# BruceGeLi/TCE_RL

Measured on NVIDIA B200. Metric: TCE policy-update episodes/sec, higher is better.
Workload: dtype f32

## Files before the change

### include/tce_b200.h

```cpp
#ifndef TCE_B200_H
#define TCE_B200_H

#include <stddef.h>
#include <stdint.h>

#ifdef __cplusplus
extern "C" {
#endif

typedef enum {
  TCE_OK = 0,
  TCE_ERR_INVALID_ARGUMENT = -1,
  TCE_ERR_UNSUPPORTED_SHAPE = -2,
  TCE_ERR_CUDA = -3,
  TCE_ERR_WORKSPACE = -4
} tce_status;

int tce_version(void);
const char *tce_strerror(int status);
const char *tce_last_cuda_error(void);

typedef struct {
  int32_t num_dof;
  int32_t num_basis;
  int32_t num_basis_outside;
  int32_t pre_compute_length_factor;
  int32_t auto_scale_basis;
  int32_t relative_goal;
  int32_t relative_goal_scaled;
  int32_t reserved;
  double tau, delay, dt, alpha, alpha_phase, basis_bandwidth_factor, weights_scale, goal_scale;
} tce_mp_cfg;

typedef struct tce_tables tce_tables_t;

int tce_prodmp_tables_create(const tce_mp_cfg *cfg, void *stream, tce_tables_t **out);
void tce_prodmp_tables_destroy(tce_tables_t *tables);
int tce_prodmp_tables_num_pc(const tce_tables_t *tables);
int tce_prodmp_tables_export(const tce_tables_t *tables, double *y1, double *y2, double *dy1,
                             double *dy2, double *pos_basis, double *vel_basis, double *scale);

int tce_prodmp_traj_fwd(const tce_tables_t *tables, const float *params, const float *times,
                        const float *init_time, const float *init_pos, const float *init_vel,
                        float *traj, int64_t B, int64_t T, void *stream);
int tce_prodmp_traj_fwd_uniform(const tce_tables_t *tables, const float *params, const float *times_row,
                                const float *init_time, const float *init_pos, const float *init_vel,
                                float *rows_ws, float *traj, int64_t B, int64_t T, void *stream);
int tce_prodmp_traj_bwd(const tce_tables_t *tables, const float *grad_traj, const float *times,
                        const float *init_time, float *grad_params, float *grad_init_pos,
                        float *grad_init_vel, int64_t B, int64_t T, void *stream);

int tce_mvn_rsample(const float *mean, const float *L, int64_t ldb_L, const float *eps, uint64_t seed,
                    uint64_t offset, float *out, int64_t B, int n, void *stream);
int tce_chol_fwd(const float *A, float *L, int32_t *info, int64_t B, int n, void *stream);
int tce_chol_bwd(const float *L, const float *grad_L, float *grad_A, int64_t B, int n, void *stream);
int tce_policy_head_fwd(const float *vec, int64_t ldb_vec, float min_std, float *L, int64_t B, int n,
                        void *stream);
int tce_policy_head_bwd(const float *vec, int64_t ldb_vec, const float *grad_L, float *grad_vec,
                        int64_t B, int n, void *stream);
int tce_policy_head_diag_fwd(const float *vec, int64_t ldb_vec, float min_std, float *L, int64_t B, int n,
                             void *stream);
int tce_policy_head_diag_bwd(const float *vec, int64_t ldb_vec, const float *grad_L, float *grad_vec,
                             int64_t B, int n, void *stream);
int tce_gauss_stats(const float *mean, const float *L, int64_t ldb_L, const float *mean_o,
                    const float *L_o, int64_t ldb_Lo, double *out, int64_t B, int n, void *stream);
int tce_gauss_stats_bwd(const float *mean, const float *L, int64_t ldb_L, const float *mean_o,
                        const float *L_o, int64_t ldb_Lo, const double *grad_out, float *grad_mean,
                        float *grad_L, int64_t B, int n, void *stream);

int tce_gauss_maha(const float *mean, const float *mean_o, const float *L_o, int64_t ldb_Lo,
                   const double *grad_out, double *maha, float *grad_mean, int64_t B, int n, void *stream);
int tce_gauss_maha_bwd_full(const float *mean, const float *mean_o, const float *L_o, int64_t ldb_Lo,
                            const double *grad_out, float *grad_mean, float *grad_L, int64_t B, int n,
                            void *stream);
int tce_tri_inverse(const float *L, int64_t ldb, double *Linv, int64_t B, int n, void *stream);
int tce_gauss_maha_shared(const float *mean, const float *mean_o, const double *Linv, const double *grad_out,
                          double *maha, float *grad_mean, int64_t B, int n, void *stream);

int tce_proj_mean_fwd(const float *mean, const float *mean_o, const double *mean_part, double eps,
                      float *proj_mean, int64_t B, int n, void *stream);
int tce_proj_mean_bwd(const float *mean, const float *mean_o, const double *mean_part, double eps,
                      const float *grad_out, float *grad_mean, double *grad_mean_part, int64_t B, int n,
                      void *stream);
int tce_proj_entropy_fwd(const float *L, const double *beta, int64_t ldb_beta, int equality, float *out,
                         double *entropy, int64_t B, int n, void *stream);
int tce_proj_entropy_bwd(const float *L, const double *beta, int64_t ldb_beta, int equality,
                         const float *grad_out, float *grad_L, int64_t B, int n, void *stream);
int tce_proj_kl_diag_fwd(const float *s, int64_t ldb_s, int64_t inc_s, const float *s_old, int64_t ldb_so,
                         int64_t inc_so, double eps_cov, const double *beta, int64_t ldb_beta, int equality,
                         float *out, int64_t ldb_o, int64_t inc_o, double *state, int32_t *info, int64_t B, int n,
                         void *stream);
int tce_proj_kl_diag_bwd(const float *s, int64_t ldb_s, int64_t inc_s, const float *s_old, int64_t ldb_so,
                         int64_t inc_so, const double *state, const float *grad_out, int64_t ldb_g, int64_t inc_g,
                         float *grad_s, int64_t ldb_gs, int64_t inc_gs, int64_t B, int n, void *stream);
size_t tce_proj_kl_save_doubles(int64_t B, int n);
int tce_proj_kl_cov_fwd(const float *L, const float *L_o, double eps_cov, float *proj_L, double *save,
                        int32_t *info, int warm_start, int64_t B, int n, void *stream);
int tce_proj_kl_cov_bwd(const float *L, const float *proj_L, const float *grad_out, const double *save,
                        float *grad_L, int64_t B, int n, void *stream);
int tce_proj_kl_entropy_fwd(const float *L, const float *L_o, double eps_cov, const double *beta,
                            int64_t ldb_beta, int equality, float *proj_L, float *out_L, double *save,
                            int32_t *info, int warm_start, int64_t B, int n, void *stream);
int tce_proj_kl_entropy_bwd(const float *L, const float *proj_L, const float *grad_out, const double *save,
                            float *grad_L, int64_t B, int n, void *stream);
int tce_proj_kl_entropy_bwd_inv(const float *L, const float *proj_L, const float *grad_out, const double *save,
                                const double *out_inv, float *grad_L, int64_t B, int n, void *stream);
int tce_proj_kl_entropy_bwd_tr(const float *L, const float *proj_L, const float *grad_out, const double *save,
                               double tr_coeff, float *grad_L, int64_t B, int n, void *stream);
int tce_proj_kl_bwd_sigma(const float *L, const double *grad_sigma, const double *save, int fused_entropy,
                          double tr_coeff, float *grad_L, int64_t B, int n, void *stream);
int tce_proj_kl_entropy_fwd_sigma_vec(const float *vec, int64_t ldb_vec, float min_std, float *L_built,
                                      const float *L_o, double eps_cov, const double *beta, int64_t ldb_beta,
                                      int equality, float *proj_L, float *out_L, double *save, int32_t *info,
                                      int warm_start, int64_t B, int n, void *stream);
int tce_proj_kl_bwd_sigma_k_vec(const float *L, const float *vec, int64_t ldb_vec, const double *grad_sigma,
                                const double *save, int fused_entropy, double tr_coeff, float *grad_vec, int64_t B,
                                int n, void *stream);
int tce_proj_kl_bwd_prep(double *save, int64_t B, int n, void *stream);
int tce_proj_kl_bwd_sigma_k(const float *L, const double *grad_sigma, const double *save, int fused_entropy,
                            double tr_coeff, float *grad_L, int64_t B, int n, void *stream);
int tce_proj_kl_entropy_fwd_sigma(const float *L, const float *L_o, double eps_cov, const double *beta,
                                  int64_t ldb_beta, int equality, float *proj_L, float *out_L, double *save,
                                  int32_t *info, int warm_start, int64_t B, int n, void *stream);
int tce_proj_kl_entropy_fwd_chol(const double *save, float *proj_L, float *out_L, double *out_inv, int32_t *info,
                                 int64_t B, int n, void *stream);
int tce_proj_frob_cov_fwd(const float *L, const float *L_o, int64_t ldb_Lo, double eps_cov, float *proj_L,
                          double *save_sc, int32_t *info, int64_t B, int n, void *stream);
int tce_proj_frob_cov_bwd(const float *L, const float *L_o, int64_t ldb_Lo, double eps_cov,
                          const float *proj_L, const float *grad_out, const double *save_sc, float *grad_L,
                          int64_t B, int n, void *stream);
int tce_proj_w2_cov_fwd(const float *L, const float *L_o, int64_t ldb_Lo, double eps_cov, int scale_prec,
                        float *proj_L, double *save_sc, int64_t B, int n, void *stream);
int tce_proj_w2_cov_bwd(const float *L, const float *L_o, int64_t ldb_Lo, double eps_cov, int scale_prec,
                        const float *grad_out, float *grad_L, int64_t B, int n, void *stream);
int tce_cov_distance(int kind, const float *L, const float *L_o, int64_t ldb_Lo, int scale_prec,
                     const double *grad_val, double *val, float *grad_L, int64_t B, int n, void *stream);

size_t tce_seglik_work_bytes(const tce_tables_t *tables, int64_t B, int64_t P);
int tce_seglik_gram(const tce_tables_t *tables, const float *smp_traj, const float *mean, const float *L,
                    int64_t ldb_L, const float *times, const float *init_time, const float *init_pos,
                    const float *init_vel, const int64_t *pred_pairs, void *work, double *diag_max,
                    int64_t B, int64_t T, int64_t P, void *stream);
int tce_seglik_chol(const tce_tables_t *tables, const void *work, void *adj, const double *diag_max, double reg_rel,
                    const float *grad_logp, const float *logp_old, const float *advantage,
                    double grad_scale, double *loss_acc, float *logp, int32_t *info, int64_t B,
                    int64_t P, void *stream);
int tce_seglik_bwd(const tce_tables_t *tables, const void *work, const float *L, int64_t ldb_L,
                   const float *times, const float *init_time, const int64_t *pred_pairs,
                   const float *upstream, float *grad_mean, float *grad_L, int64_t B, int64_t T, int64_t P,
                   void *stream);
int tce_seglik_diag_max(const tce_tables_t *tables, const float *s, int64_t ldb_s, int64_t inc_s,
                        const float *times, const float *init_time, const int64_t *pred_pairs, double *diag_max,
                        int64_t B, int64_t T, int64_t P, void *stream);
int tce_seglik_diag_fwd(const tce_tables_t *tables, const float *smp_traj, const float *mean, const float *s,
                        int64_t ldb_s, int64_t inc_s, const float *times, const float *init_time,
                        const float *init_pos, const float *init_vel, const int64_t *pred_pairs,
                        const double *diag_max, double reg_rel, float *logp, int32_t *info, int64_t B, int64_t T,
                        int64_t P, void *stream);
int tce_seglik_diag_bwd(const tce_tables_t *tables, const float *smp_traj, const float *mean, const float *s,
                        int64_t ldb_s, int64_t inc_s, const float *times, const float *init_time,
                        const float *init_pos, const float *init_vel, const int64_t *pred_pairs,
                        const double *diag_max, double reg_rel, const float *grad_logp, float *grad_mean,
                        float *grad_s, int64_t ldb_gs, int64_t inc_gs, int64_t B, int64_t T, int64_t P,
                        void *stream);

int tce_seglik_fused_config(const tce_tables_t *tables, int64_t B, int64_t P, int chained, int32_t *episodes_per_iter,
                            int32_t *grid, int64_t *part_floats, int64_t *pre_doubles_per_episode);
int tce_seglik_prepass(const tce_tables_t *tables, const float *smp_traj, const float *mean, const float *L,
                       int64_t ldb_L, const double *Sigma0, const double *sigma_scale, const float *times,
                       const float *init_time, const float *init_pos, const float *init_vel,
                       const int64_t *pred_pairs, double *pre, double *diag_max, int chained, int64_t B, int64_t T,
                       int64_t P, void *stream);
int tce_seglik_fused(const tce_tables_t *tables, const double *pre, const float *L, int64_t ldb_L,
                     const double *Sigma0, const double *sigma_scale, const int64_t *pred_pairs,
                     const double *diag_max, double reg_rel, int grad_mode, const float *grad_logp,
                     const float *logp_old, const float *advantage, double grad_scale, double *loss_acc, float *logp,
                     int32_t *info, float *grad_mean, float *grad_L, float *dsigma_part, int chained, int64_t B,
                     int64_t P, void *stream);
int tce_seglik_dsigma_reduce(const tce_tables_t *tables, float *dsigma_part, int nparts, const float *L,
                             const float *upstream, float *grad_L, double *grad_sigma, void *stream);
size_t tce_seglik_uniform_ws_doubles(const tce_tables_t *tables, int64_t P);
int tce_seglik_uniform_parts(const tce_tables_t *tables, int64_t B, int64_t P, int32_t *nparts,
                             int64_t *apart_doubles);
int tce_seglik_uniform_prep(const tce_tables_t *tables, const float *L, const double *Sigma0,
                            const double *sigma_scale, const float *times, const float *init_time,
                            const int64_t *pred_pairs, double *ws, double *diag_max, double reg_rel, int what,
                            int64_t P, void *stream);
int tce_seglik_uniform_main(const tce_tables_t *tables, const double *ws, const float *smp_traj, const float *mean,
                            const float *init_pos, const float *init_vel, const int64_t *pred_pairs, int grad_mode,
                            const float *grad_logp, const float *logp_old, const float *advantage,
                            double grad_scale, double *loss_acc, float *logp, int32_t *info, float *grad_mean,
                            double *apart, int64_t B, int64_t T, int64_t P, void *stream);
int tce_seglik_uniform_finish(const tce_tables_t *tables, double *ws, const double *apart, int nparts,
                              const float *L, const float *upstream, float *grad_L, double *grad_sigma, int64_t P,
                              void *stream);

int tce_gae(const float *rewards, const float *values, const uint8_t *dones, const uint8_t *tl_dones,
            float gamma, float lam, int use_gae, float *adv, float *ret, int64_t B, int64_t T,
            void *stream);
int tce_segment_advantage_raw(int mode, const float *rewards, const float *values, const float *advantages,
                              const int64_t *pred_pairs, float gamma, float *seg, double *stats, int64_t B,
                              int64_t T, int64_t P, void *stream);
int tce_sum_stats(const float *x, double *stats, int64_t N, void *stream);
int tce_normalize_by_stats(float *x, const double *stats, int64_t N, void *stream);

int tce_grad_sumsq(const float *grad_flat, int64_t n, double *state, void *stream);
int tce_adam_step(int count, float *const *params, const int64_t *sizes, const float *grad_flat, float *m,
                  float *v, const double *state, double max_norm, double lr, double beta1, double beta2,
                  double eps, double weight_decay, void *stream);

int tce_p2p_allreduce_sumsq(int world, int rank, const void *const *peer_bufs, void *const *peer_pads, int64_t n,
                            float *avg_out, void *local2, double *state3, void *stream);
int tce_p2p_allreduce_sumsq_range(int world, int rank, const void *const *peer_bufs, void *const *peer_pads,
                                  int64_t offset, int64_t n, int phase, int bump_step, float *avg_out, void *local2,
                                  double *state3, void *stream);

size_t tce_p2p_push_xchg_bytes(int world, int64_t n_total);
int tce_p2p_push_allreduce_sumsq(int world, int rank, void *const *peer_xchg, const float *grad, int64_t n_total,
                                 int64_t offset, int64_t n, int phase, int bump_step, float *avg_out, void *local2,
                                 double *state3, void *stream);

int tce_epoch_mean_fwd(const float *mean, const float *mean_old, const double *Linv_old, double eps_mean,
                       float *proj_mean, double *maha_old, float *u_old, double *acc, int64_t B, int n,
                       void *stream);
int tce_epoch_tr_mean(const float *mean, const float *mean_old, const double *maha_old, const float *u_old,
                      const double *Linv_new, const double *kl_scalars, double eps_mean, double tr_coeff,
                      float *tr_grad, double *acc, int64_t B, int n, void *stream);
int tce_epoch_mean_combine(const float *g_proj_mean, const float *mean, const float *mean_old, const double *maha_old,
                           const float *u_old, const float *tr_grad, double eps_mean, float *grad_mean, int64_t B,
                           int n, void *stream);
int tce_epoch_metrics(const double *acc, const double *lik_stats, const double *kl_scalars, const double *adam_stats,
                      int64_t B, double tr_coeff, int with_cov, double ent_coef, double *out19, void *stream);

int tce_debug_kl_phase_cycles(long long *out32);
int tce_debug_seglik_phase_cycles(long long *out32);
int tce_bench_fma(int fp64, int iters, void *scratch, double *flops, void *stream);

#ifdef __cplusplus
}
#endif
#endif
```

### tce_rl_b200/_lib.py

```python
from __future__ import annotations

import ctypes as C
import os

HERE = os.path.dirname(os.path.abspath(__file__))
LIB_PATH = os.path.join(HERE, "libtce_b200.so")


class TceError(RuntimeError):
    pass


class MpCfg(C.Structure):
    _fields_ = [("num_dof", C.c_int32), ("num_basis", C.c_int32), ("num_basis_outside", C.c_int32),
                ("pre_compute_length_factor", C.c_int32), ("auto_scale_basis", C.c_int32),
                ("relative_goal", C.c_int32), ("relative_goal_scaled", C.c_int32), ("reserved", C.c_int32),
                ("tau", C.c_double), ("delay", C.c_double), ("dt", C.c_double), ("alpha", C.c_double),
                ("alpha_phase", C.c_double), ("basis_bandwidth_factor", C.c_double),
                ("weights_scale", C.c_double), ("goal_scale", C.c_double)]


_P, _I64, _I32, _U64, _F, _D = C.c_void_p, C.c_int64, C.c_int, C.c_uint64, C.c_float, C.c_double

SIGNATURES = {
    "tce_version": (C.c_int, []),
    "tce_strerror": (C.c_char_p, [C.c_int]),
    "tce_last_cuda_error": (C.c_char_p, []),
    "tce_prodmp_tables_create": (C.c_int, [C.POINTER(MpCfg), _P, C.POINTER(_P)]),
    "tce_prodmp_tables_destroy": (None, [_P]),
    "tce_prodmp_tables_num_pc": (C.c_int, [_P]),
    "tce_prodmp_tables_export": (C.c_int, [_P] * 8),
    "tce_prodmp_traj_fwd": (C.c_int, [_P] * 7 + [_I64, _I64, _P]),
    "tce_prodmp_traj_fwd_uniform": (C.c_int, [_P] * 8 + [_I64, _I64, _P]),
    "tce_prodmp_traj_bwd": (C.c_int, [_P] * 7 + [_I64, _I64, _P]),
    "tce_mvn_rsample": (C.c_int, [_P, _P, _I64, _P, _U64, _U64, _P, _I64, _I32, _P]),
    "tce_chol_fwd": (C.c_int, [_P, _P, _P, _I64, _I32, _P]),
    "tce_chol_bwd": (C.c_int, [_P, _P, _P, _I64, _I32, _P]),
    "tce_policy_head_fwd": (C.c_int, [_P, _I64, _F, _P, _I64, _I32, _P]),
    "tce_policy_head_bwd": (C.c_int, [_P, _I64, _P, _P, _I64, _I32, _P]),
    "tce_policy_head_diag_fwd": (C.c_int, [_P, _I64, _F, _P, _I64, _I32, _P]),
    "tce_policy_head_diag_bwd": (C.c_int, [_P, _I64, _P, _P, _I64, _I32, _P]),
    "tce_proj_kl_diag_fwd": (C.c_int, [_P, _I64, _I64, _P, _I64, _I64, _D, _P, _I64, _I32, _P, _I64, _I64, _P, _P, _I64,
                                       _I32, _P]),
    "tce_proj_kl_diag_bwd": (C.c_int, [_P, _I64, _I64, _P, _I64, _I64, _P, _P, _I64, _I64, _P, _I64, _I64, _I64, _I32,
                                       _P]),
    "tce_seglik_diag_max": (C.c_int, [_P, _P, _I64, _I64, _P, _P, _P, _P, _I64, _I64, _I64, _P]),
    "tce_seglik_diag_fwd": (C.c_int, [_P, _P, _P, _P, _I64, _I64, _P, _P, _P, _P, _P, _P, _D, _P, _P, _I64, _I64, _I64,
                                      _P]),
    "tce_seglik_diag_bwd": (C.c_int, [_P, _P, _P, _P, _I64, _I64, _P, _P, _P, _P, _P, _P, _D, _P, _P, _P, _I64, _I64,
                                      _I64, _I64, _I64, _P]),
    "tce_gauss_stats": (C.c_int, [_P, _P, _I64, _P, _P, _I64, _P, _I64, _I32, _P]),
    "tce_gauss_stats_bwd": (C.c_int, [_P, _P, _I64, _P, _P, _I64, _P, _P, _P, _I64, _I32, _P]),
    "tce_gauss_maha": (C.c_int, [_P, _P, _P, _I64, _P, _P, _P, _I64, _I32, _P]),
    "tce_gauss_maha_bwd_full": (C.c_int, [_P, _P, _P, _I64, _P, _P, _P, _I64, _I32, _P]),
    "tce_tri_inverse": (C.c_int, [_P, _I64, _P, _I64, _I32, _P]),
    "tce_gauss_maha_shared": (C.c_int, [_P, _P, _P, _P, _P, _P, _I64, _I32, _P]),
    "tce_proj_mean_fwd": (C.c_int, [_P, _P, _P, _D, _P, _I64, _I32, _P]),
    "tce_proj_mean_bwd": (C.c_int, [_P, _P, _P, _D, _P, _P, _P, _I64, _I32, _P]),
    "tce_proj_entropy_fwd": (C.c_int, [_P, _P, _I64, _I32, _P, _P, _I64, _I32, _P]),
    "tce_proj_entropy_bwd": (C.c_int, [_P, _P, _I64, _I32, _P, _P, _I64, _I32, _P]),
    "tce_proj_kl_save_doubles": (C.c_size_t, [_I64, _I32]),
    "tce_proj_kl_cov_fwd": (C.c_int, [_P, _P, _D, _P, _P, _P, _I32, _I64, _I32, _P]),
    "tce_proj_kl_cov_bwd": (C.c_int, [_P, _P, _P, _P, _P, _I64, _I32, _P]),
    "tce_proj_kl_entropy_fwd": (C.c_int, [_P, _P, _D, _P, _I64, _I32, _P, _P, _P, _P, _I32, _I64, _I32, _P]),
    "tce_proj_kl_entropy_bwd": (C.c_int, [_P, _P, _P, _P, _P, _I64, _I32, _P]),
    "tce_proj_kl_entropy_bwd_tr": (C.c_int, [_P, _P, _P, _P, _D, _P, _I64, _I32, _P]),
    "tce_proj_kl_bwd_sigma": (C.c_int, [_P, _P, _P, _I32, _D, _P, _I64, _I32, _P]),
    "tce_proj_kl_bwd_sigma_k": (C.c_int, [_P, _P, _P, _I32, _D, _P, _I64, _I32, _P]),
    "tce_proj_kl_bwd_prep": (C.c_int, [_P, _I64, _I32, _P]),
    "tce_proj_kl_entropy_fwd_sigma_vec": (C.c_int, [_P, _I64, _F, _P, _P, _D, _P, _I64, _I32, _P, _P, _P, _P, _I32, _I64,
                                                    _I32, _P]),
    "tce_proj_kl_bwd_sigma_k_vec": (C.c_int, [_P, _P, _I64, _P, _P, _I32, _D, _P, _I64, _I32, _P]),
    "tce_proj_kl_entropy_bwd_inv": (C.c_int, [_P, _P, _P, _P, _P, _P, _I64, _I32, _P]),
    "tce_proj_kl_entropy_fwd_sigma": (C.c_int, [_P, _P, _D, _P, _I64, _I32, _P, _P, _P, _P, _I32, _I64, _I32, _P]),
    "tce_proj_kl_entropy_fwd_chol": (C.c_int, [_P, _P, _P, _P, _P, _I64, _I32, _P]),
    "tce_grad_sumsq": (C.c_int, [_P, _I64, _P, _P]),
    "tce_adam_step": (C.c_int, [_I32, _P, _P, _P, _P, _P, _P, _D, _D, _D, _D, _D, _D, _P]),
    "tce_proj_frob_cov_fwd": (C.c_int, [_P, _P, _I64, _D, _P, _P, _P, _I64, _I32, _P]),
    "tce_proj_frob_cov_bwd": (C.c_int, [_P, _P, _I64, _D, _P, _P, _P, _P, _I64, _I32, _P]),
    "tce_proj_w2_cov_fwd": (C.c_int, [_P, _P, _I64, _D, _I32, _P, _P, _I64, _I32, _P]),
    "tce_proj_w2_cov_bwd": (C.c_int, [_P, _P, _I64, _D, _I32, _P, _P, _I64, _I32, _P]),
    "tce_cov_distance": (C.c_int, [_I32, _P, _P, _I64, _I32, _P, _P, _P, _I64, _I32, _P]),
    "tce_seglik_work_bytes": (C.c_size_t, [_P, _I64, _I64]),
    "tce_seglik_gram": (C.c_int, [_P, _P, _P, _P, _I64, _P, _P, _P, _P, _P, _P, _P, _I64, _I64, _I64, _P]),
    "tce_seglik_chol": (C.c_int, [_P, _P, _P, _P, _D, _P, _P, _P, _D, _P, _P, _P, _I64, _I64, _P]),
    "tce_seglik_bwd": (C.c_int, [_P, _P, _P, _I64, _P, _P, _P, _P, _P, _P, _I64, _I64, _I64, _P]),
    "tce_seglik_fused_config": (C.c_int, [_P, _I64, _I64, _I32, C.POINTER(C.c_int32), C.POINTER(C.c_int32),
                                          C.POINTER(C.c_int64), C.POINTER(C.c_int64)]),
    "tce_seglik_prepass": (C.c_int, [_P] * 4 + [_I64] + [_P] * 9 + [_I32, _I64, _I64, _I64, _P]),
    "tce_seglik_fused": (C.c_int, [_P, _P, _P, _I64, _P, _P, _P, _P, _D, _I32, _P, _P, _P, _D, _P, _P, _P, _P, _P, _P,
                                   _I32, _I64, _I64, _P]),
    "tce_seglik_dsigma_reduce": (C.c_int, [_P, _P, _I32, _P, _P, _P, _P, _P]),
    "tce_seglik_uniform_ws_doubles": (C.c_size_t, [_P, _I64]),
    "tce_seglik_uniform_parts": (C.c_int, [_P, _I64, _I64, C.POINTER(C.c_int32), C.POINTER(C.c_int64)]),
    "tce_seglik_uniform_prep": (C.c_int, [_P, _P, _P, _P, _P, _P, _P, _P, _P, _D, _I32, _I64, _P]),
    "tce_seglik_uniform_main": (C.c_int, [_P, _P, _P, _P, _P, _P, _P, _I32, _P, _P, _P, _D, _P, _P, _P, _P, _P, _I64,
                                          _I64, _I64, _P]),
    "tce_seglik_uniform_finish": (C.c_int, [_P, _P, _P, _I32, _P, _P, _P, _P, _I64, _P]),
    "tce_p2p_allreduce_sumsq": (C.c_int, [_I32, _I32, _P, _P, _I64, _P, _P, _P, _P]),
    "tce_p2p_allreduce_sumsq_range": (C.c_int, [_I32, _I32, _P, _P, _I64, _I64, _I32, _I32, _P, _P, _P, _P]),
    "tce_p2p_push_xchg_bytes": (C.c_size_t, [_I32, _I64]),
    "tce_p2p_push_allreduce_sumsq": (C.c_int, [_I32, _I32, _P, _P, _I64, _I64, _I64, _I32, _I32, _P, _P, _P, _P]),
    "tce_epoch_mean_fwd": (C.c_int, [_P, _P, _P, _D, _P, _P, _P, _P, _I64, _I32, _P]),
    "tce_epoch_tr_mean": (C.c_int, [_P, _P, _P, _P, _P, _P, _D, _D, _P, _P, _I64, _I32, _P]),
    "tce_epoch_mean_combine": (C.c_int, [_P, _P, _P, _P, _P, _P, _D, _P, _I64, _I32, _P]),
    "tce_epoch_metrics": (C.c_int, [_P, _P, _P, _P, _I64, _D, _I32, _D, _P, _P]),
    "tce_gae": (C.c_int, [_P, _P, _P, _P, _F, _F, _I32, _P, _P, _I64, _I64, _P]),
    "tce_segment_advantage_raw": (C.c_int, [_I32, _P, _P, _P, _P, _F, _P, _P, _I64, _I64, _I64, _P]),
    "tce_sum_stats": (C.c_int, [_P, _P, _I64, _P]),
    "tce_normalize_by_stats": (C.c_int, [_P, _P, _I64, _P]),
    "tce_debug_kl_phase_cycles": (C.c_int, [_P]),
    "tce_debug_seglik_phase_cycles": (C.c_int, [_P]),
    "tce_bench_fma": (C.c_int, [_I32, _I32, _P, C.POINTER(C.c_double), _P]),
}

_lib = None


def load() -> C.CDLL:
    global _lib
    if _lib is None:
        if not os.path.exists(LIB_PATH):
            raise TceError(f"{LIB_PATH} is missing: run `python -m tce_rl_b200._build` "
                           "(or __graft_entry__.build()); there is no CPU fallback")
        lib = C.CDLL(LIB_PATH)
        for name, (res, args) in SIGNATURES.items():
            fn = getattr(lib, name)
            fn.restype, fn.argtypes = res, args
        _lib = lib
    return _lib


def check(status: int, what: str = "") -> None:
    if status != 0:
        lib = load()
        msg = lib.tce_strerror(status).decode()
        if status == -3:
            msg += " -- " + lib.tce_last_cuda_error().decode()
        raise TceError(f"{what}: {msg} (status {status})")


LAUNCHES = 0
_NO_KERNEL = {"tce_seglik_fused_config", "tce_seglik_uniform_parts", "tce_prodmp_tables_export", "tce_prodmp_tables_create", "tce_debug_kl_phase_cycles", "tce_debug_seglik_phase_cycles"}


TIMING = None


def call(name: str, *args) -> None:
    global LAUNCHES
    if TIMING is not None and name not in _NO_KERNEL:
        import torch
        st = torch.cuda.ExternalStream(args[-1]) if args[-1] else torch.cuda.default_stream()
        a, b = torch.cuda.Event(enable_timing=True), torch.cuda.Event(enable_timing=True)
        a.record(st)
        check(getattr(load(), name)(*args), name)
        b.record(st)
        TIMING.append((name, a, b))
        LAUNCHES += 1
        return
    check(getattr(load(), name)(*args), name)
    if name not in _NO_KERNEL:
        LAUNCHES += 1
```

### tce_rl_b200/csrc/tce_seglik_fused.cu

```cuda
#include <math.h>

#include "tce_common.cuh"

namespace {

constexpr int FT = 256;
constexpr double LN_2PI = 1.8378770664093453;

__host__ __device__ constexpr int tri(int n) { return n * (n + 1) / 2; }
__device__ __forceinline__ int tri_idx(int r, int c) { return r * (r + 1) / 2 + c; }
__device__ __forceinline__ void tri_decode(int t, int &I, int &J) {
  int i = (int)((sqrtf(8.0f * (float)t + 1.0f) - 1.0f) * 0.5f);
  while (i * (i + 1) / 2 > t) --i;
  while ((i + 1) * (i + 2) / 2 <= t) ++i;
  I = i;
  J = t - i * (i + 1) / 2;
}

struct Links { int pf, ps, nxt, prv; };
__device__ __forceinline__ Links links(int chained, int q, int P) {
  Links l;
  if (chained) { l.pf = q < P ? q : -1; l.ps = q >= 1 ? q - 1 : -1; l.nxt = q + 1; l.prv = q - 1; }
  else if (q & 1) { l.pf = -1; l.ps = q >> 1; l.nxt = q; l.prv = q - 1; }
  else { l.pf = q >> 1; l.ps = -1; l.nxt = q + 1; l.prv = q; }
  return l;
}
__device__ __forceinline__ long long point_time_index(const int64_t *__restrict__ pairs, int chained, int q, int P) {
  if (!chained) return pairs[q];
  return q < P ? pairs[2 * q] : pairs[2 * P - 1];
}
__device__ __forceinline__ int point_of(int chained, int p, int k) { return chained ? p + k : 2 * p + k; }

__device__ int block_chained(const int64_t *__restrict__ pairs, int P) {
  int ok = 1;
  for (int pp = threadIdx.x; pp + 1 < P; pp += blockDim.x) ok &= (pairs[2 * pp + 1] == pairs[2 * pp + 2]);
  return __syncthreads_and(ok) != 0;
}

template <int K1>
__device__ __forceinline__ void init_row_entry(const TabDev &tb, double t_init, int j, double *init_row) {
  int i0; double w;
  time_to_index(tb, t_init, i0, w);
  if (j < K1) {
    init_row[5 + j] = lerp_t(tb.pos[(size_t)i0 * K1 + j], tb.pos[(size_t)(i0 + 1) * K1 + j], w);
    init_row[5 + K1 + j] = lerp_t(tb.vel[(size_t)i0 * K1 + j], tb.vel[(size_t)(i0 + 1) * K1 + j], w);
  } else {
    const double a = lerp_t(tb.y1[i0], tb.y1[i0 + 1], w), b = lerp_t(tb.y2[i0], tb.y2[i0 + 1], w);
    const double c = lerp_t(tb.dy1[i0], tb.dy1[i0 + 1], w), d = lerp_t(tb.dy2[i0], tb.dy2[i0 + 1], w);
    init_row[0] = a; init_row[1] = b; init_row[2] = c; init_row[3] = d;
    init_row[4] = 1.0 / (a * d - b * c);
  }
}
template <int K1>
__device__ __forceinline__ void basis_entry(const TabDev &tb, const double *init_row, double t, int j, double *h_row,
                                            double *xi_row) {
  int i0; double w;
  time_to_index(tb, t, i0, w);
  const double y1 = lerp_t(tb.y1[i0], tb.y1[i0 + 1], w), y2 = lerp_t(tb.y2[i0], tb.y2[i0 + 1], w);
  const double idet = init_row[4];
  const double xi1 = (init_row[3] * y1 - init_row[2] * y2) * idet, xi2 = (init_row[0] * y2 - init_row[1] * y1) * idet;
  if (j < K1) {
    const double pj = lerp_t(tb.pos[(size_t)i0 * K1 + j], tb.pos[(size_t)(i0 + 1) * K1 + j], w);
    h_row[j] = (pj - xi1 * init_row[5 + j] - xi2 * init_row[5 + K1 + j]) * tb.scale[j];
  } else {
    xi_row[0] = xi1;
    xi_row[1] = xi2;
  }
}

template <int N>
__device__ __forceinline__ double seg_factor(double (&c)[tri(N)], double (&z)[N], double reg, int &bad) {
#define CE(r, q) c[(r) * ((r) + 1) / 2 + (q)]
  bad = 0;
  double half_logdet = 0.0, maha = 0.0;
#pragma unroll
  for (int j = 0; j < N; ++j) {
    double dj = CE(j, j) + reg;
#pragma unroll
    for (int k = 0; k < j; ++k) dj = fma(-CE(j, k), CE(j, k), dj);
    if (!(dj > 0.0) && bad == 0) bad = j + 1;
    double inv = (double)rsqrtf((float)dj);
    inv = inv * fma(-0.5 * dj, inv * inv, 1.5);
    inv = inv * fma(-0.5 * dj, inv * inv, 1.5);
    CE(j, j) = inv;
    half_logdet += 0.5 * log(dj);
#pragma unroll
    for (int i = j + 1; i < N; ++i) {
      double v = CE(i, j);
#pragma unroll
      for (int k = 0; k < j; ++k) v = fma(-CE(i, k), CE(j, k), v);
      CE(i, j) = v * inv;
    }
    double zj = z[j];
#pragma unroll
    for (int k = 0; k < j; ++k) zj = fma(-CE(j, k), z[k], zj);
    zj *= inv;
    z[j] = zj;
    maha = fma(zj, zj, maha);
  }
  return -0.5 * ((double)N * LN_2PI + maha) - half_logdet;
}
template <int N>
__device__ __forceinline__ void seg_adjoint(double (&c)[tri(N)], double (&z)[N], double g) {
#pragma unroll
  for (int i = N - 1; i >= 0; --i) {
    double v = z[i];
#pragma unroll
    for (int k = i + 1; k < N; ++k) v = fma(-CE(k, i), z[k], v);
    z[i] = v * CE(i, i);
  }
#pragma unroll
  for (int j = 0; j < N; ++j) {
#pragma unroll
    for (int i = j + 1; i < N; ++i) {
      double v = 0.0;
#pragma unroll
      for (int k = j; k < i; ++k) v = fma(CE(i, k), CE(k, j), v);
      CE(i, j) = -v * CE(i, i);
    }
  }
#pragma unroll
  for (int i = 0; i < N; ++i) {
#pragma unroll
    for (int j = 0; j <= i; ++j) {
      double v = 0.0;
#pragma unroll
      for (int k = i; k < N; ++k) v = fma(CE(k, i), CE(k, j), v);
      CE(i, j) = 0.5 * g * (z[i] * z[j] - v);
    }
  }
#pragma unroll
  for (int i = 0; i < N; ++i) z[i] *= g;
#undef CE
}

struct SegIO {
  const float *grad_logp, *logp_old, *advantage;
  float *logp;
  int32_t *info;
  double grad_scale, reg;
  int grad_mode;
};
template <int N>
__device__ __noinline__ void segment_thread(double *Ccol, double *Rcol, int S, long long gid, const SegIO &io,
                                            double &loss_part, double &ratio_part) {
  constexpr int NT = tri(N);
  double c[NT];
#define CE(r, q) c[(r) * ((r) + 1) / 2 + (q)]
#define ZS(i) Rcol[(size_t)(i) * S]
#pragma unroll
  for (int t = 0; t < NT; ++t) c[t] = Ccol[(size_t)t * S];
  int bad = 0;
  double half_logdet = 0.0, maha = 0.0;
#pragma unroll
  for (int j = 0; j < N; ++j) {
    double dj = CE(j, j) + io.reg;
#pragma unroll
    for (int k = 0; k < j; ++k) dj = fma(-CE(j, k), CE(j, k), dj);
    if (!(dj > 0.0) && bad == 0) bad = j + 1;
    double inv = (double)rsqrtf((float)dj);
    inv = inv * fma(-0.5 * dj, inv * inv, 1.5);
    inv = inv * fma(-0.5 * dj, inv * inv, 1.5);
    CE(j, j) = inv;
    half_logdet += 0.5 * log(dj);
#pragma unroll
    for (int i = j + 1; i < N; ++i) {
      double v = CE(i, j);
#pragma unroll
      for (int k = 0; k < j; ++k) v = fma(-CE(i, k), CE(j, k), v);
      CE(i, j) = v * inv;
    }
    double zj = ZS(j);
#pragma unroll
    for (int k = 0; k < j; ++k) zj = fma(-CE(j, k), ZS(k), zj);
    zj *= inv;
    ZS(j) = zj;
    maha = fma(zj, zj, maha);
  }
  const double lp = -0.5 * ((double)N * LN_2PI + maha) - half_logdet;
  if (io.logp) io.logp[gid] = (float)lp;
  if (io.info) io.info[gid] = bad;
  if (io.grad_mode == 0) return;
  double g;
  if (io.grad_mode == 2) {
    const double ratio = exp(lp - (double)io.logp_old[gid]);
    g = -ratio * (double)io.advantage[gid] * io.grad_scale;
    loss_part += g;
    ratio_part += ratio * io.grad_scale;
  } else {
    g = (double)io.grad_logp[gid];
  }
#pragma unroll
  for (int i = N - 1; i >= 0; --i) {
    double v = ZS(i);
#pragma unroll
    for (int k = i + 1; k < N; ++k) v = fma(-CE(k, i), ZS(k), v);
    ZS(i) = v * CE(i, i);
  }
#pragma unroll
  for (int j = 0; j < N; ++j) {
#pragma unroll
    for (int i = j + 1; i < N; ++i) {
      double v = 0.0;
#pragma unroll
      for (int k = j; k < i; ++k) v = fma(CE(i, k), CE(k, j), v);
      CE(i, j) = -v * CE(i, i);
    }
  }
  const double hg = 0.5 * g;
#pragma unroll
  for (int i = 0; i < N; ++i) {
    const double ai = ZS(i);
#pragma unroll
    for (int j = 0; j <= i; ++j) {
      double v = 0.0;
#pragma unroll
      for (int k = i; k < N; ++k) v = fma(CE(k, i), CE(k, j), v);
      Ccol[(size_t)(i * (i + 1) / 2 + j) * S] = hg * (ai * ZS(j) - v);
    }
  }
#pragma unroll
  for (int i = 0; i < N; ++i) ZS(i) = g * ZS(i);
#undef CE
#undef ZS
}

template <int K1>
__device__ __noinline__ void dsigma_block_store(bool own, const double *G, int S, const double *hm_e, int bd, int bdd,
                                                int chained, int nq, int P, float *dst, int ld, float *dst_t) {
  double acc[K1 * K1];
  if (own) {
#pragma unroll
    for (int t = 0; t < K1 * K1; ++t) acc[t] = 0.0;
    const int r0 = 2 * bd, q0 = 2 * bdd;
    const double *g00 = G + (size_t)tri_idx(r0, q0) * S, *g10 = G + (size_t)tri_idx(r0 + 1, q0) * S;
    const double *g11 = G + (size_t)tri_idx(r0 + 1, q0 + 1) * S;
    const double *g01 = (bd != bdd) ? G + (size_t)tri_idx(r0, q0 + 1) * S : g10;
    for (int q = 0; q < nq; ++q) {
      const Links lk = links(chained, q, P);
      const double *hq = hm_e + q * K1;
      double cs = 0.0, cn = 0.0, cp = 0.0;
      if (lk.pf >= 0) { cs += g00[lk.pf]; cn = g10[lk.pf]; }
      if (lk.ps >= 0) { cs += g11[lk.ps]; cp = g01[lk.ps]; }
      const double *hn = hm_e + (lk.pf >= 0 ? lk.nxt : q) * K1, *hp = hm_e + (lk.ps >= 0 ? lk.prv : q) * K1;
      double h[K1], w[K1];
#pragma unroll
      for (int j = 0; j < K1; ++j) h[j] = hq[j];
#pragma unroll
      for (int i = 0; i < K1; ++i) w[i] = fma(cs, h[i], fma(cn, hn[i], cp * hp[i]));
#pragma unroll
      for (int i = 0; i < K1; ++i)
#pragma unroll
        for (int j = 0; j < K1; ++j) acc[i * K1 + j] = fma(w[i], h[j], acc[i * K1 + j]);
    }
  }
  __syncthreads();
  if (own) {
    if (ld == 0) {
#pragma unroll
      for (int t = 0; t < K1 * K1; ++t) dst[t] = (float)acc[t];
    } else {
#pragma unroll
      for (int i = 0; i < K1; ++i)
#pragma unroll
        for (int j = 0; j < K1; ++j) {
          const float v = (float)acc[i * K1 + j];
          dst[i * ld + j] = v;
          if (dst_t) dst_t[j * ld + i] = v;
        }
    }
  }
}

__host__ __device__ inline size_t pre_doubles(int nq, int K1, int N, int P) { return (size_t)nq * K1 + (size_t)N * P; }

template <int D, int K1>
struct FusedLayout {
  static constexpr int Dp = D * K1, N = 2 * D, NT = tri(N), NB = tri(D);
  static constexpr int KP = (K1 + 1) & ~1;
  static constexpr int NR4 = (Dp + 3) & ~3, LD = NR4 + 1;
  static constexpr int IR = (5 + 2 * K1 + 1) & ~1;
  static constexpr int LCNT = (NR4 * NR4 + FT - 1) / FT;
  size_t sblk, dsacc, cs, rs, hm, total;
  int E, S, SP, nq;
  __host__ __device__ FusedLayout(int E_, int P, int chained) {
    E = E_; S = E * P; SP = S | 1; nq = chained ? P + 1 : 2 * P;
    size_t o = 0;
    auto take = [&](size_t bytes) { size_t at = o; o += (bytes + 15) & ~(size_t)15; return at; };
    const size_t sb = sizeof(double) * NB * K1 * KP, ls = sizeof(float) * NR4 * LD;
    sblk = take(sb > ls ? sb : ls);
    dsacc = take(sizeof(float) * NB * K1 * K1);
    const size_t c1 = sizeof(double) * NT * SP, c2 = sizeof(float) * (size_t)E * NR4 * LD;
    const size_t c3 = sizeof(float) * (size_t)E * NB * K1 * K1, c12 = c1 > c2 ? c1 : c2;
    cs = take(c12 > c3 ? c12 : c3);
    rs = take(sizeof(double) * N * SP);
    hm = take(sizeof(double) * (size_t)E * nq * K1);
    total = o;
  }
};

template <int K1, int KP>
__device__ __forceinline__ double *sblk_at(double *Sblk, int blk) { return Sblk + (size_t)blk * K1 * KP; }

template <int K1, int KP>
__device__ __forceinline__ void sblk_store(double *Sblk, int i, int j, double v) {
  const int d = i / K1, dd = j / K1, ii = i - d * K1, jj = j - dd * K1;
  double *blk = sblk_at<K1, KP>(Sblk, tri_idx(d, dd));
  blk[ii * KP + jj] = v;
  if (d == dd) blk[jj * KP + ii] = v;
}

__device__ __forceinline__ void stage_lower(const float *__restrict__ L, float *Ls, int n, int NR, int LD) {
  for (int e0 = threadIdx.x; e0 < NR * NR; e0 += 4 * FT) {
    float v[4];
#pragma unroll
    for (int u = 0; u < 4; ++u) {
      const int e = e0 + u * FT, i = e / NR, c = e - i * NR;
      v[u] = (e < NR * NR && i < n && c <= i) ? L[(size_t)i * n + c] : 0.0f;
    }
#pragma unroll
    for (int u = 0; u < 4; ++u) {
      const int e = e0 + u * FT, i = e / NR, c = e - i * NR;
      if (e < NR * NR) Ls[i * LD + c] = v[u];
    }
  }
}

template <int D, int K1>
__device__ __forceinline__ void sigma_from_factor(const float *Ls, double *Sblk) {
  using FL = FusedLayout<D, K1>;
  constexpr int NT4 = FL::NR4 / 4, LD = FL::LD, Dp = FL::Dp;
  static_assert(tri(NT4) <= FT, "one tile per thread");
  float c[4][4];
  int I = 0, J = 0;
  const bool act = threadIdx.x < tri(NT4);
  if (act) {
    tri_decode(threadIdx.x, I, J);
    const float *a = Ls + (4 * I) * LD, *bq = Ls + (4 * J) * LD;
#pragma unroll
    for (int x = 0; x < 4; ++x)
#pragma unroll
      for (int y = 0; y < 4; ++y) c[x][y] = 0.f;
    const int kmax = 4 * J + 3;
    for (int k = 0; k <= kmax; ++k) {
      float av[4], bv[4];
#pragma unroll
      for (int x = 0; x < 4; ++x) { av[x] = a[x * LD + k]; bv[x] = bq[x * LD + k]; }
#pragma unroll
      for (int x = 0; x < 4; ++x)
#pragma unroll
        for (int y = 0; y < 4; ++y) c[x][y] = fmaf(av[x], bv[y], c[x][y]);
    }
  }
  __syncthreads();
  if (act) {
#pragma unroll
    for (int x = 0; x < 4; ++x)
#pragma unroll
      for (int y = 0; y < 4; ++y) {
        const int i = 4 * I + x, j = 4 * J + y;
        if (i < Dp && j <= i) sblk_store<K1, FL::KP>(Sblk, i, j, (double)c[x][y]);
      }
  }
  __syncthreads();
}

template <int D, int K1>
__device__ __forceinline__ double gram_item(const double *__restrict__ Sb, const double *__restrict__ hm_e, int q,
                                            const Links &lk, int d, int dd, double *CS, int S, int slot0) {
  constexpr int KP = FusedLayout<D, K1>::KP;
  double h[K1], v[K1];
  const double *hq = hm_e + q * K1;
#pragma unroll
  for (int j = 0; j < K1; ++j) h[j] = hq[j];
#pragma unroll
  for (int i = 0; i < K1; ++i) {
    const double *row = Sb + i * KP;
    double a0 = 0.0, a1 = 0.0;
#pragma unroll
    for (int j = 0; j + 1 < K1; j += 2) {
      const double2 s = *reinterpret_cast<const double2 *>(row + j);
      a0 = fma(s.x, h[j], a0);
      a1 = fma(s.y, h[j + 1], a1);
    }
    if (K1 & 1) a0 = fma(row[K1 - 1], h[K1 - 1], a0);
    v[i] = a0 + a1;
  }
  double kuu = 0.0;
#pragma unroll
  for (int i = 0; i < K1; ++i) kuu = fma(h[i], v[i], kuu);
  const int r0 = 2 * d, q0 = 2 * dd;
  if (lk.pf >= 0) {
    const double *hn = hm_e + lk.nxt * K1;
    double kup = 0.0;
#pragma unroll
    for (int i = 0; i < K1; ++i) kup = fma(hn[i], v[i], kup);
    CS[(size_t)tri_idx(r0, q0) * S + slot0 + lk.pf] = kuu;
    CS[(size_t)tri_idx(r0 + 1, q0) * S + slot0 + lk.pf] = kup;
  }
  if (lk.ps >= 0) {
    CS[(size_t)tri_idx(r0 + 1, q0 + 1) * S + slot0 + lk.ps] = kuu;
    if (d != dd) {
      const double *hp = hm_e + lk.prv * K1;
      double kum = 0.0;
#pragma unroll
      for (int i = 0; i < K1; ++i) kum = fma(hp[i], v[i], kum);
      CS[(size_t)tri_idx(r0, q0 + 1) * S + slot0 + lk.ps] = kum;
    }
  }
  return kuu;
}

template <int NR4, int CNT>
__device__ __forceinline__ void prefetch_lower(const float *__restrict__ L, int n, float (&v)[CNT]) {
#pragma unroll
  for (int u = 0; u < CNT; ++u) {
    const int e = threadIdx.x + u * FT, i = e / NR4, c = e - i * NR4;
    v[u] = (e < NR4 * NR4 && i < n && c <= i) ? L[(size_t)i * n + c] : 0.0f;
  }
}
template <int NR4, int CNT>
__device__ __forceinline__ void commit_lower(const float (&v)[CNT], float *Ls, int LD) {
#pragma unroll
  for (int u = 0; u < CNT; ++u) {
    const int e = threadIdx.x + u * FT, i = e / NR4, c = e - i * NR4;
    if (e < NR4 * NR4) Ls[i * LD + c] = v[u];
  }
}

constexpr int PT = 128;
template <int D, int K1, bool SIGMA_IN>
__global__ void __launch_bounds__(PT)
seglik_prepass_kernel(TabDev tb, const float *__restrict__ smp_traj, const float *__restrict__ mean,
                      const float *__restrict__ L, long long ldb_L, const double *__restrict__ Sigma0,
                      const double *__restrict__ sigma_scale, const float *__restrict__ times,
                      const float *__restrict__ init_time, const float *__restrict__ init_pos,
                      const float *__restrict__ init_vel, const int64_t *__restrict__ pairs,
                      double *__restrict__ pre, double *__restrict__ diag_max, long long B, int T, int P,
                      int chained) {
  using FL = FusedLayout<D, K1>;
  constexpr int Dp = FL::Dp, N = FL::N, IR = FL::IR;
  extern __shared__ __align__(16) unsigned char smem_raw[];
  double *Sd = reinterpret_cast<double *>(smem_raw);
  double *hm = Sd + D * K1 * K1;
  double *xi = hm + (size_t)2 * P * K1;
  double *init_row = xi + (size_t)4 * P;
  float *Lsm = reinterpret_cast<float *>(init_row + IR);
  __shared__ double s_max[PT / 32];
  if (chained && !block_chained(pairs, P)) return;
  const int nq = chained ? P + 1 : 2 * P;
  const size_t pstride = pre_doubles(nq, K1, N, P);
  const bool shared_cov = SIGMA_IN || ldb_L == 0;
  const double tau = tb.tau;
  double my_max = 0.0;
  auto load_diag_blocks = [&](long long b) {
    if (SIGMA_IN) {
      const double sc = sigma_scale ? *sigma_scale : 1.0;
      for (int e = threadIdx.x; e < D * K1 * K1; e += PT) {
        const int d = e / (K1 * K1), r = e - d * K1 * K1, i = r / K1, j = r - i * K1;
        Sd[e] = sc * Sigma0[(size_t)(d * K1 + i) * Dp + d * K1 + j];
      }
    } else {
      const float *Lb = L + b * ldb_L;
      for (int e0 = threadIdx.x; e0 < Dp * Dp; e0 += 8 * PT) {
        float v[8];
#pragma unroll
        for (int u = 0; u < 8; ++u) v[u] = (e0 + u * PT < Dp * Dp) ? Lb[e0 + u * PT] : 0.f;
#pragma unroll
        for (int u = 0; u < 8; ++u) {
          const int e = e0 + u * PT;
          if (e < Dp * Dp) Lsm[(e / Dp) * (Dp + 1) + (e % Dp)] = v[u];
        }
      }
      __syncthreads();
      for (int e = threadIdx.x; e < D * K1 * K1; e += PT) {
        const int d = e / (K1 * K1), r = e - d * K1 * K1, i = r / K1, j = r - i * K1;
        const float *a = Lsm + (d * K1 + i) * (Dp + 1), *bq = Lsm + (d * K1 + j) * (Dp + 1);
        const int kmax = d * K1 + (i < j ? i : j);
        float a0 = 0.f, a1 = 0.f, a2 = 0.f, a3 = 0.f;
        int k = 0;
        for (; k + 3 <= kmax; k += 4) {
          a0 = fmaf(a[k], bq[k], a0); a1 = fmaf(a[k + 1], bq[k + 1], a1);
          a2 = fmaf(a[k + 2], bq[k + 2], a2); a3 = fmaf(a[k + 3], bq[k + 3], a3);
        }
        for (; k <= kmax; ++k) a0 = fmaf(a[k], bq[k], a0);
        Sd[e] = (double)((a0 + a1) + (a2 + a3));
      }
    }
  };
  if (shared_cov) load_diag_blocks(0);
  for (long long b = blockIdx.x; b < B; b += gridDim.x) {
    __syncthreads();
    if (!shared_cov) load_diag_blocks(b);
    if (threadIdx.x <= K1) init_row_entry<K1>(tb, (double)init_time[b], threadIdx.x, init_row);
    __syncthreads();
    for (int it = threadIdx.x; it < nq * (K1 + 1); it += PT) {
      const int q = it / (K1 + 1), j = it - q * (K1 + 1);
      basis_entry<K1>(tb, init_row, (double)times[b * T + point_time_index(pairs, chained, q, P)], j, hm + q * K1,
                      xi + 2 * q);
    }
    __syncthreads();
    double *pb = pre + (size_t)b * pstride;
    for (int it = threadIdx.x; it < nq * K1; it += PT) pb[it] = hm[it];
    double *rb = pb + (size_t)nq * K1;
    for (int it = threadIdx.x; it < P * N; it += PT) {
      const int d = it / (2 * P), pk = it - d * 2 * P, p = pk >> 1, k = pk & 1;
      const int q = point_of(chained, p, k);
      const double *hq = hm + q * K1;
      const double y0 = (double)init_pos[b * D + d], v0 = (double)init_vel[b * D + d] * tau;
      double mu = xi[2 * q] * y0 + xi[2 * q + 1] * v0;
      const float *th = mean + b * Dp + d * K1;
#pragma unroll
      for (int j = 0; j < K1; ++j) mu = fma(hq[j], (double)th[j], mu);
      if (tb.relative_goal) {
        const double shift = tb.relative_goal_scaled ? y0 : y0 / tb.scale[K1 - 1];
        mu = fma(hq[K1 - 1], shift, mu);
      }
      const double x = (double)smp_traj[(b * T + pairs[2 * p + k]) * (2 * D) + d];
      rb[(size_t)(2 * d + k) * P + p] = x - mu;
    }
    for (int it = threadIdx.x; it < D * nq; it += PT) {
      const int d = it / nq, q = it - d * nq;
      const double *S = Sd + d * K1 * K1, *h = hm + q * K1;
      double acc = 0.0;
#pragma unroll
      for (int i = 0; i < K1; ++i) {
        double v = 0.0;
#pragma unroll
        for (int j = 0; j < K1; ++j) v = fma(S[i * K1 + j], h[j], v);
        acc = fma(h[i], v, acc);
      }
      my_max = fmax(my_max, acc);
    }
  }
  my_max = warp_max(my_max);
  if ((threadIdx.x & 31) == 0) s_max[threadIdx.x >> 5] = my_max;
  __syncthreads();
  if (threadIdx.x == 0) {
    double m = 0.0;
    for (int w = 0; w < PT / 32; ++w) m = fmax(m, s_max[w]);
    atomic_max_pos_double(diag_max, m);
  }
}

template <int D, int K1, bool SIGMA_IN>
__global__ void __launch_bounds__(FT, 1)
seglik_fused_kernel(const double *__restrict__ pre, const float *__restrict__ L, long long ldb_L,
                    const double *__restrict__ Sigma0, const double *__restrict__ sigma_scale,
                    const int64_t *__restrict__ pairs, const double *__restrict__ diag_max, double reg_rel,
                    int grad_mode, const float *__restrict__ grad_logp, const float *__restrict__ logp_old,
                    const float *__restrict__ advantage, double grad_scale, double *__restrict__ loss_acc,
                    float *__restrict__ logp, int32_t *__restrict__ info, float *__restrict__ grad_mean,
                    float *__restrict__ grad_L, float *__restrict__ dsigma_part, long long B, int P, int E,
                    int chained) {
  using FL = FusedLayout<D, K1>;
  constexpr int Dp = FL::Dp, N = FL::N, NT = FL::NT, NB = FL::NB, KP = FL::KP, NR4 = FL::NR4, LD = FL::LD;
  constexpr int LCNT = FL::LCNT;
  extern __shared__ __align__(16) unsigned char smem_raw[];
  if (chained && !block_chained(pairs, P)) {
    if (blockIdx.x == 0 && threadIdx.x == 0 && info) info[0] = -7;
    return;
  }
  const FL lay(E, P, chained);
  const int S = lay.SP, nq = lay.nq;
  double *Sblk = reinterpret_cast<double *>(smem_raw + lay.sblk);
  float *Ls = reinterpret_cast<float *>(smem_raw + lay.sblk);
  float *dsacc = reinterpret_cast<float *>(smem_raw + lay.dsacc);
  double *CS = reinterpret_cast<double *>(smem_raw + lay.cs);
  float *dSb = reinterpret_cast<float *>(smem_raw + lay.cs);
  double *RS = reinterpret_cast<double *>(smem_raw + lay.rs);
  double *hm = reinterpret_cast<double *>(smem_raw + lay.hm);
  __shared__ double s_red[2 * (FT / 32)];

  const bool shared_cov = SIGMA_IN || ldb_L == 0;
  const bool want_grad = grad_mode != 0;
  const int warp = threadIdx.x >> 5, lane = threadIdx.x & 31;
  const double reg = reg_rel * (*diag_max);
  const size_t pstride = pre_doubles(nq, K1, N, P);
  double loss_part = 0.0, ratio_part = 0.0;
  if (blockIdx.x == 0 && threadIdx.x == 0 && dsigma_part && want_grad)
    *reinterpret_cast<unsigned int *>(dsigma_part + ((size_t)gridDim.x + 1) * NB * K1 * K1) = 0u;

  if (shared_cov) {
    if (SIGMA_IN) {
      const double sc = sigma_scale ? *sigma_scale : 1.0;
      for (int e0 = threadIdx.x; e0 < Dp * Dp; e0 += 4 * FT) {
        double v[4];
#pragma unroll
        for (int u = 0; u < 4; ++u) v[u] = (e0 + u * FT < Dp * Dp) ? Sigma0[e0 + u * FT] : 0.0;
#pragma unroll
        for (int u = 0; u < 4; ++u) {
          const int e = e0 + u * FT, i = e / Dp, j = e - i * Dp;
          if (e < Dp * Dp && j <= i) sblk_store<K1, KP>(Sblk, i, j, sc * v[u]);
        }
      }
      __syncthreads();
    } else {
      float lr[LCNT];
      prefetch_lower<NR4, LCNT>(L, Dp, lr);
      commit_lower<NR4, LCNT>(lr, Ls, LD);
      __syncthreads();
      sigma_from_factor<D, K1>(Ls, Sblk);
    }
    if (want_grad && dsigma_part)
      for (int e = threadIdx.x; e < NB * K1 * K1; e += FT) dsacc[e] = 0.f;
  }

  const long long n_groups = (B + E - 1) / E;
  for (long long grp = blockIdx.x; grp < n_groups; grp += gridDim.x) {
    const long long b0 = grp * E;
    const int Ec = (int)((B - b0) < E ? (B - b0) : E);
    __syncthreads();
    {
      const double *pg = pre + (size_t)b0 * pstride;
      const int total = Ec * (int)pstride, hme = nq * K1;
      for (int it0 = threadIdx.x; it0 < total; it0 += 6 * FT) {
        double v[6];
#pragma unroll
        for (int u = 0; u < 6; ++u) v[u] = (it0 + u * FT < total) ? pg[it0 + u * FT] : 0.0;
#pragma unroll
        for (int u = 0; u < 6; ++u) {
          const int it = it0 + u * FT;
          if (it < total) {
            const int e = it / (int)pstride, r = it - e * (int)pstride;
            if (r < hme) hm[(size_t)e * hme + r] = v[u];
            else { const int rr = r - hme, i = rr / P, p = rr - i * P; RS[(size_t)i * S + e * P + p] = v[u]; }
          }
        }
      }
    }
    __syncthreads();
    if (shared_cov) {
      const int items = Ec * nq, chunks = (items + 31) >> 5;
      for (int wt = warp; wt < NB * chunks; wt += FT / 32) {
        const int blk = wt / chunks, item = (wt - blk * chunks) * 32 + lane;
        if (item < items) {
          int d, dd;
          tri_decode(blk, d, dd);
          const int e = item / nq, q = item - e * nq;
          gram_item<D, K1>(sblk_at<K1, KP>(Sblk, blk), hm + (size_t)e * nq * K1, q, links(chained, q, P), d, dd, CS, S,
                           e * P);
        }
      }
    } else {
      float lr[LCNT];
      prefetch_lower<NR4, LCNT>(L + b0 * ldb_L, Dp, lr);
      for (int e = 0; e < Ec; ++e) {
        __syncthreads();
        commit_lower<NR4, LCNT>(lr, Ls, LD);
        if (e + 1 < Ec) prefetch_lower<NR4, LCNT>(L + (b0 + e + 1) * ldb_L, Dp, lr);
        __syncthreads();
        sigma_from_factor<D, K1>(Ls, Sblk);
        const int chunks = (nq + 31) >> 5;
        for (int wt = warp; wt < NB * chunks; wt += FT / 32) {
          const int blk = wt / chunks, q = (wt - blk * chunks) * 32 + lane;
          if (q < nq) {
            int d, dd;
            tri_decode(blk, d, dd);
            gram_item<D, K1>(sblk_at<K1, KP>(Sblk, blk), hm + (size_t)e * nq * K1, q, links(chained, q, P), d, dd, CS,
                             S, e * P);
          }
        }
      }
    }
    __syncthreads();
    if ((int)threadIdx.x < Ec * P) {
      const int slot = threadIdx.x, e = slot / P, p = slot - e * P;
      SegIO io{grad_logp, logp_old, advantage, logp, info, grad_scale, reg, grad_mode};
      segment_thread<N>(CS + slot, RS + slot, S, (b0 + e) * P + p, io, loss_part, ratio_part);
    }
    if (!want_grad) continue;
    __syncthreads();
    if (grad_mean) {
      for (int it = threadIdx.x; it < Ec * Dp; it += FT) {
        const int e = it / Dp, o = it - e * Dp, d = o / K1, j = o - d * K1;
        const double *hm_e = hm + (size_t)e * nq * K1;
        const double *a0 = RS + (size_t)(2 * d) * S + e * P, *a1 = RS + (size_t)(2 * d + 1) * S + e * P;
        double acc0 = 0.0, acc1 = 0.0;
        for (int p = 0; p < P; ++p) {
          acc0 = fma(hm_e[point_of(chained, p, 0) * K1 + j], a0[p], acc0);
          acc1 = fma(hm_e[point_of(chained, p, 1) * K1 + j], a1[p], acc1);
        }
        grad_mean[(b0 + e) * Dp + o] = (float)(acc0 + acc1);
      }
    }
    if (!grad_L && !dsigma_part) continue;
    const bool own = (int)threadIdx.x < Ec * NB;
    int be = 0, bblk = 0, bd = 0, bdd = 0;
    if (own) {
      be = threadIdx.x / NB; bblk = threadIdx.x - be * NB;
      tri_decode(bblk, bd, bdd);
    }
    if (shared_cov) {
      dsigma_block_store<K1>(own, CS + be * P, S, hm + (size_t)be * nq * K1, bd, bdd, chained, nq, P,
                             dSb + ((size_t)be * NB + bblk) * (K1 * K1), 0, nullptr);
      __syncthreads();
      for (int e2 = threadIdx.x; e2 < NB * K1 * K1; e2 += FT) {
        float s = dsacc[e2];
        for (int e = 0; e < Ec; ++e) s += dSb[(size_t)e * NB * K1 * K1 + e2];
        dsacc[e2] = s;
      }
    } else {
      float *M0 = dSb + (size_t)be * NR4 * LD;
      dsigma_block_store<K1>(own, CS + be * P, S, hm + (size_t)be * nq * K1, bd, bdd, chained, nq, P,
                             M0 + (bd * K1) * LD + bdd * K1, LD, bd != bdd ? M0 + (bdd * K1) * LD + bd * K1 : nullptr);
      if (NR4 > Dp) {
        for (int it = threadIdx.x; it < Ec * (NR4 - Dp) * NR4; it += FT) {
          const int e = it / ((NR4 - Dp) * NR4), r = it - e * (NR4 - Dp) * NR4, a = Dp + r / NR4, c = r - (r / NR4) * NR4;
          float *M = dSb + (size_t)e * NR4 * LD;
          M[a * LD + c] = 0.f;
          M[c * LD + a] = 0.f;
        }
      }
      float lr[LCNT];
      prefetch_lower<NR4, LCNT>(L + b0 * ldb_L, Dp, lr);
      for (int e = 0; e < Ec; ++e) {
        __syncthreads();
        commit_lower<NR4, LCNT>(lr, Ls, LD);
        if (e + 1 < Ec) prefetch_lower<NR4, LCNT>(L + (b0 + e + 1) * ldb_L, Dp, lr);
        __syncthreads();
        const float *M = dSb + (size_t)e * NR4 * LD;
        float *gL = grad_L + (size_t)(b0 + e) * Dp * Dp;
        constexpr int NT4 = NR4 / 4;
        if (threadIdx.x < tri(NT4)) {
          int I, J;
          tri_decode(threadIdx.x, I, J);
          const float *mrow = M + (4 * I) * LD;
          float c4[4][4];
#pragma unroll
          for (int x = 0; x < 4; ++x)
#pragma unroll
            for (int y = 0; y < 4; ++y) c4[x][y] = 0.f;
          for (int k = NR4 - 1; k >= 4 * J; --k) {
            float mv[4], lv[4];
#pragma unroll
            for (int x = 0; x < 4; ++x) { mv[x] = mrow[x * LD + k]; lv[x] = Ls[k * LD + 4 * J + x]; }
#pragma unroll
            for (int x = 0; x < 4; ++x)
#pragma unroll
              for (int y = 0; y < 4; ++y) c4[x][y] = fmaf(mv[x], lv[y], c4[x][y]);
          }
#pragma unroll
          for (int x = 0; x < 4; ++x)
#pragma unroll
            for (int y = 0; y < 4; ++y) {
              const int i = 4 * I + x, j = 4 * J + y;
              if (i < Dp && j < Dp) gL[(size_t)i * Dp + j] = j <= i ? 2.f * c4[x][y] : 0.f;
            }
        } else {
          for (int t = threadIdx.x - tri(NT4); t < NT4 * NT4; t += FT - tri(NT4)) {
            const int I = t / NT4, J = t - I * NT4;
            if (J > I)
              for (int x = 0; x < 4; ++x)
                for (int y = 0; y < 4; ++y) {
                  const int i = 4 * I + x, j = 4 * J + y;
                  if (i < Dp && j < Dp) gL[(size_t)i * Dp + j] = 0.f;
                }
          }
        }
      }
    }
  }
  __syncthreads();
  if (shared_cov && want_grad && dsigma_part) {
    float *out = dsigma_part + (size_t)blockIdx.x * NB * K1 * K1;
    for (int e = threadIdx.x; e < NB * K1 * K1; e += FT) out[e] = dsacc[e];
  }
  if (grad_mode == 2 && loss_acc) {
    loss_part = warp_sum(loss_part);
    ratio_part = warp_sum(ratio_part);
    if (lane == 0) { s_red[2 * warp] = loss_part; s_red[2 * warp + 1] = ratio_part; }
    __syncthreads();
    if (threadIdx.x == 0) {
      double a = 0.0, r = 0.0;
      for (int w = 0; w < FT / 32; ++w) { a += s_red[2 * w]; r += s_red[2 * w + 1]; }
      if (r != 0.0) { atomicAdd(loss_acc, a); atomicAdd(loss_acc + 1, r); }
    }
  }
}

template <int D, int K1>
__device__ __forceinline__ void dl_from_dsigma(const float *M, const float *Ls, float *__restrict__ grad_L) {
  using FL = FusedLayout<D, K1>;
  constexpr int Dp = FL::Dp, NR4 = FL::NR4, LD = FL::LD, NT2 = NR4 / 2;
  for (int t = threadIdx.x; t < tri(NT2); t += blockDim.x) {
    int I, J;
    tri_decode(t, I, J);
    const float *m0 = M + (2 * I) * LD, *m1 = m0 + LD;
    float c00 = 0.f, c01 = 0.f, c10 = 0.f, c11 = 0.f;
    for (int k = 2 * J; k < NR4; ++k) {
      const float a0 = m0[k], a1 = m1[k], l0 = Ls[k * LD + 2 * J], l1 = Ls[k * LD + 2 * J + 1];
      c00 = fmaf(a0, l0, c00); c01 = fmaf(a0, l1, c01);
      c10 = fmaf(a1, l0, c10); c11 = fmaf(a1, l1, c11);
    }
    const int i0 = 2 * I, j0 = 2 * J;
    if (i0 < Dp && j0 < Dp) grad_L[(size_t)i0 * Dp + j0] = 2.f * c00;
    if (i0 < Dp && j0 + 1 < Dp) grad_L[(size_t)i0 * Dp + j0 + 1] = j0 + 1 <= i0 ? 2.f * c01 : 0.f;
    if (i0 + 1 < Dp && j0 < Dp) grad_L[(size_t)(i0 + 1) * Dp + j0] = 2.f * c10;
    if (i0 + 1 < Dp && j0 + 1 < Dp) grad_L[(size_t)(i0 + 1) * Dp + j0 + 1] = 2.f * c11;
  }
  for (int e = threadIdx.x; e < Dp * Dp; e += blockDim.x) {
    const int i = e / Dp, j = e - i * Dp;
    if (j / 2 > i / 2) grad_L[e] = 0.f;
  }
}

template <int D, int K1>
__device__ __forceinline__ void unpack_blocks(const float *blocks, float scale, float *M) {
  using FL = FusedLayout<D, K1>;
  constexpr int NB = FL::NB, LD = FL::LD, NE = NB * K1 * K1;
  for (int e = threadIdx.x; e < NE; e += blockDim.x) {
    const float v = scale * __ldcg(blocks + e);
    const int blk = e / (K1 * K1), r = e - blk * K1 * K1, i = r / K1, j = r - i * K1;
    int d, dd;
    tri_decode(blk, d, dd);
    M[(d * K1 + i) * LD + dd * K1 + j] = v;
    if (d != dd) M[(dd * K1 + j) * LD + d * K1 + i] = v;
  }
}

constexpr int RT = 256;
template <int D, int K1>
__global__ void __launch_bounds__(RT)
dsigma_reduce_kernel(float *part, int nparts, const float *__restrict__ L, const float *__restrict__ upstream,
                     float *__restrict__ grad_L, double *__restrict__ grad_sigma) {
  using FL = FusedLayout<D, K1>;
  constexpr int Dp = FL::Dp, NB = FL::NB, NR4 = FL::NR4, LD = FL::LD, NE = NB * K1 * K1;
  extern __shared__ __align__(16) unsigned char smem_raw[];
  float *M = reinterpret_cast<float *>(smem_raw);
  float *Ls = M + NR4 * LD;
  __shared__ float s_part[8][33];
  __shared__ int s_last;
  float *dsum = part + (size_t)nparts * NE;
  unsigned int *ticket = reinterpret_cast<unsigned int *>(dsum + NE);
  const int el = threadIdx.x & 31, sl = threadIdx.x >> 5, e = blockIdx.x * 32 + el;
  float a[4] = {0.f, 0.f, 0.f, 0.f};
  if (e < NE) {
    int k = sl;
    for (; k + 24 < nparts; k += 32) {
#pragma unroll
      for (int u = 0; u < 4; ++u) a[u] += part[(size_t)(k + 8 * u) * NE + e];
    }
    for (; k < nparts; k += 8) a[0] += part[(size_t)k * NE + e];
  }
  s_part[sl][el] = (a[0] + a[1]) + (a[2] + a[3]);
  __syncthreads();
  if (threadIdx.x < 32 && e < NE) {
    float t = 0.f;
#pragma unroll
    for (int u = 0; u < 8; ++u) t += s_part[u][el];
    dsum[e] = t;
  }
  __threadfence();
  __syncthreads();
  if (threadIdx.x == 0) s_last = (atomicAdd(ticket, 1u) == gridDim.x - 1);
  __syncthreads();
  if (!s_last) return;
  __threadfence();
  const float up = upstream ? *upstream : 1.0f;
  for (int t = threadIdx.x; t < NR4 * LD; t += RT) M[t] = 0.f;
  for (int e0 = threadIdx.x; e0 < NR4 * NR4; e0 += RT) {
    const int i = e0 / NR4, c = e0 - i * NR4;
    Ls[i * LD + c] = (L && i < Dp && c <= i) ? L[(size_t)i * Dp + c] : 0.f;
  }
  __syncthreads();
  unpack_blocks<D, K1>(dsum, up, M);
  __syncthreads();
  if (grad_sigma)
    for (int t = threadIdx.x; t < Dp * Dp; t += RT) grad_sigma[t] = (double)M[(t / Dp) * LD + (t % Dp)];
  if (grad_L) dl_from_dsigma<D, K1>(M, Ls, grad_L);
}

template <int D, int K1>
struct UniLayout {
  static constexpr int N = 2 * D, NT = tri(N);
  size_t hm, xi, xinv, cinv, gbuf, hld, flags, total;
  __host__ __device__ UniLayout(int P) {
    size_t o = 0;
    auto take = [&](size_t n) { size_t at = o; o += (n + 1) & ~(size_t)1; return at; };
    hm = take((size_t)2 * P * K1); xi = take((size_t)4 * P); xinv = take((size_t)P * NT);
    cinv = take((size_t)P * NT); gbuf = take((size_t)P * NT); hld = take(P); flags = take(4); total = o;
  }
};

constexpr int UT = 1024;
template <int D, int K1, bool SIGMA_IN>
__global__ void __launch_bounds__(UT)
uniform_prep_kernel(TabDev tb, const float *__restrict__ L, const double *__restrict__ Sigma0,
                    const double *__restrict__ sigma_scale, const float *__restrict__ times,
                    const float *__restrict__ init_time, const int64_t *__restrict__ pairs, double *ws,
                    double *diag_max, double reg_rel, int P, int what) {
  using FL = FusedLayout<D, K1>;
  using UL = UniLayout<D, K1>;
  constexpr int Dp = FL::Dp, N = FL::N, NT = FL::NT, NB = FL::NB, KP = FL::KP, NR4 = FL::NR4, LD = FL::LD, IR = FL::IR;
  extern __shared__ __align__(16) unsigned char smem_raw[];
  const UL ul(P);
  double *Sblk = reinterpret_cast<double *>(smem_raw);
  float *Ls = reinterpret_cast<float *>(smem_raw);
  const size_t sb = sizeof(double) * NB * K1 * KP, ls = sizeof(float) * NR4 * LD;
  double *irow = reinterpret_cast<double *>(smem_raw + (((sb > ls ? sb : ls) + 15) & ~(size_t)15));
  double *hm = irow + IR;
  __shared__ double s_max[UT / 32];
  const int warp = threadIdx.x >> 5, lane = threadIdx.x & 31;
  const int chained = block_chained(pairs, P);
  const int nq = chained ? P + 1 : 2 * P;
  double *g_c = ws + ul.xinv;
  if (what & 1) {
    if (threadIdx.x <= K1) init_row_entry<K1>(tb, (double)init_time[0], threadIdx.x, irow);
    if (SIGMA_IN) {
      const double sc = sigma_scale ? *sigma_scale : 1.0;
      for (int e0 = threadIdx.x; e0 < Dp * Dp; e0 += 4 * UT) {
        double v[4];
#pragma unroll
        for (int u = 0; u < 4; ++u) v[u] = (e0 + u * UT < Dp * Dp) ? Sigma0[e0 + u * UT] : 0.0;
#pragma unroll
        for (int u = 0; u < 4; ++u) {
          const int e = e0 + u * UT, i = e / Dp, j = e - i * Dp;
          if (e < Dp * Dp && j <= i) sblk_store<K1, KP>(Sblk, i, j, sc * v[u]);
        }
      }
      __syncthreads();
    } else {
      for (int e0 = threadIdx.x; e0 < NR4 * NR4; e0 += 4 * UT) {
        float v[4];
#pragma unroll
        for (int u = 0; u < 4; ++u) {
          const int e = e0 + u * UT, i = e / NR4, c = e - i * NR4;
          v[u] = (e < NR4 * NR4 && i < Dp && c <= i) ? L[(size_t)i * Dp + c] : 0.f;
        }
#pragma unroll
        for (int u = 0; u < 4; ++u) {
          const int e = e0 + u * UT, i = e / NR4, c = e - i * NR4;
          if (e < NR4 * NR4) Ls[i * LD + c] = v[u];
        }
      }
      __syncthreads();
      float vals[(Dp * (Dp + 1) / 2 + UT - 1) / UT];
      int cnt = 0;
      for (int t = threadIdx.x; t < tri(Dp); t += UT, ++cnt) {
        int i, j;
        tri_decode(t, i, j);
        const float *a = Ls + i * LD, *bq = Ls + j * LD;
        float a0 = 0.f, a1 = 0.f;
        int k = 0;
        for (; k + 1 <= j; k += 2) { a0 = fmaf(a[k], bq[k], a0); a1 = fmaf(a[k + 1], bq[k + 1], a1); }
        if (k <= j) a0 = fmaf(a[k], bq[k], a0);
        vals[cnt] = a0 + a1;
      }
      __syncthreads();
      cnt = 0;
      for (int t = threadIdx.x; t < tri(Dp); t += UT, ++cnt) {
        int i, j;
        tri_decode(t, i, j);
        sblk_store<K1, KP>(Sblk, i, j, (double)vals[cnt]);
      }
      __syncthreads();
    }
    for (int it = threadIdx.x; it < nq * (K1 + 1); it += UT) {
      const int q = it / (K1 + 1), j = it - q * (K1 + 1);
      double xr[2];
      basis_entry<K1>(tb, irow, (double)times[point_time_index(pairs, chained, q, P)], j, hm + (size_t)q * K1, xr);
      if (j < K1) ws[ul.hm + (size_t)q * K1 + j] = hm[(size_t)q * K1 + j];
      else { ws[ul.xi + 2 * q] = xr[0]; ws[ul.xi + 2 * q + 1] = xr[1]; }
    }
    __syncthreads();
    double my_max = 0.0;
    for (int it = threadIdx.x; it < NB * nq; it += UT) {
      const int blk = it / nq, q = it - blk * nq;
      int d, dd;
      tri_decode(blk, d, dd);
      const Links lk = links(chained, q, P);
      double h[K1], v[K1];
      const double *Sb = sblk_at<K1, KP>(Sblk, blk), *hq = hm + (size_t)q * K1;
#pragma unroll
      for (int j = 0; j < K1; ++j) h[j] = hq[j];
#pragma unroll
      for (int i = 0; i < K1; ++i) {
        double a0 = 0.0, a1 = 0.0;
#pragma unroll
        for (int j = 0; j + 1 < K1; j += 2) { a0 = fma(Sb[i * KP + j], h[j], a0); a1 = fma(Sb[i * KP + j + 1], h[j + 1], a1); }
        if (K1 & 1) a0 = fma(Sb[i * KP + K1 - 1], h[K1 - 1], a0);
        v[i] = a0 + a1;
      }
      double kuu = 0.0;
#pragma unroll
      for (int i = 0; i < K1; ++i) kuu = fma(h[i], v[i], kuu);
      const int r0 = 2 * d, q0 = 2 * dd;
      if (lk.pf >= 0) {
        const double *hn = hm + (size_t)lk.nxt * K1;
        double kup = 0.0;
#pragma unroll
        for (int i = 0; i < K1; ++i) kup = fma(hn[i], v[i], kup);
        g_c[(size_t)lk.pf * NT + tri_idx(r0, q0)] = kuu;
        g_c[(size_t)lk.pf * NT + tri_idx(r0 + 1, q0)] = kup;
      }
      if (lk.ps >= 0) {
        g_c[(size_t)lk.ps * NT + tri_idx(r0 + 1, q0 + 1)] = kuu;
        if (d != dd) {
          const double *hp = hm + (size_t)lk.prv * K1;
          double kum = 0.0;
#pragma unroll
          for (int i = 0; i < K1; ++i) kum = fma(hp[i], v[i], kum);
          g_c[(size_t)lk.ps * NT + tri_idx(r0, q0 + 1)] = kum;
        }
      }
      if (d == dd) my_max = fmax(my_max, kuu);
    }
    my_max = warp_max(my_max);
    if (lane == 0) s_max[warp] = my_max;
    __syncthreads();
    if (threadIdx.x == 0) {
      double m = 0.0;
      for (int w = 0; w < UT / 32; ++w) m = fmax(m, s_max[w]);
      atomic_max_pos_double(diag_max, m);
      ws[ul.flags] = (double)chained;
      ws[ul.flags + 1] = (double)nq;
      *reinterpret_cast<unsigned int *>(ws + ul.flags + 2) = 0u;
    }
  }
}

template <int D, int K1>
__global__ void __launch_bounds__(32)
uniform_factor_kernel(double *ws, const double *__restrict__ diag_max, double reg_rel, int P) {
  using UL = UniLayout<D, K1>;
  constexpr int N = 2 * D, NT = tri(N);
  static_assert(N <= 32, "lane = row");
  const UL ul(P);
  __shared__ double A[NT], X[NT], dinv[N];
  const int p = blockIdx.x, lane = threadIdx.x;
  const double reg = reg_rel * (*diag_max);
  double *g_x = ws + ul.xinv + (size_t)p * NT;
  for (int t = lane; t < NT; t += 32) A[t] = g_x[t];
  __syncwarp();
  double hld = 0.0;
  const int i = lane;
  for (int j = 0; j < N; ++j) {
    double s = 0.0;
    if (i >= j && i < N) {
      s = A[tri_idx(i, j)] + (i == j ? reg : 0.0);
      const double *ri = A + tri_idx(i, 0), *rj = A + tri_idx(j, 0);
      double s1 = 0.0;
      int k = 0;
      for (; k + 1 < j; k += 2) { s = fma(-ri[k], rj[k], s); s1 = fma(-ri[k + 1], rj[k + 1], s1); }
      if (k < j) s = fma(-ri[k], rj[k], s);
      s += s1;
    }
    const double d = __shfl_sync(0xffffffffu, s, j);
    double inv = (double)rsqrtf((float)d);
    inv = inv * fma(-0.5 * d, inv * inv, 1.5);
    inv = inv * fma(-0.5 * d, inv * inv, 1.5);
    hld += 0.5 * log(d);
    __syncwarp();
    if (i == j) { A[tri_idx(j, j)] = d * inv; dinv[j] = inv; }
    else if (i > j && i < N) A[tri_idx(i, j)] = s * inv;
    __syncwarp();
  }
  if (lane < N) {
    const int j = lane;
    double x[N];
#pragma unroll
    for (int r = 0; r < N; ++r) {
      double v = (r == j) ? 1.0 : 0.0;
#pragma unroll
      for (int k = 0; k < r; ++k) v = fma(-A[r * (r + 1) / 2 + k], (k >= j) ? x[k] : 0.0, v);
      x[r] = (r >= j) ? v * dinv[r] : 0.0;
    }
#pragma unroll
    for (int r = 0; r < N; ++r)
      if (r >= j) X[tri_idx(r, j)] = x[r];
  }
  __syncwarp();
  for (int t = lane; t < NT; t += 32) {
    int r, c;
    tri_decode(t, r, c);
    double v = 0.0;
    for (int k = r; k < N; ++k) v = fma(X[tri_idx(k, r)], X[tri_idx(k, c)], v);
    ws[ul.cinv + (size_t)p * NT + t] = v;
    g_x[t] = X[t];
  }
  if (lane == 0) ws[ul.hld + p] = hld;
}

constexpr int UM_THREADS = 256;
template <int D, int K1, int EP>
struct UniMainSmem {
  static constexpr int UM_EP = EP;
  static constexpr int Dp = D * K1, N = 2 * D, NT = tri(N), AL = UM_EP + 1, MS = Dp | 1;
  size_t X, h, xi, hld, al, g, mean, r, y0, pidx, total;
  int RS;
  __host__ __device__ UniMainSmem(int P) {
    size_t o = 0;
    auto take = [&](size_t bytes) { size_t at = o; o += (bytes + 15) & ~(size_t)15; return at; };
    RS = (2 * P * D) | 1;
    X = take(sizeof(double) * P * NT); h = take(sizeof(double) * 2 * P * K1); xi = take(sizeof(double) * 4 * P);
    hld = take(sizeof(double) * P); al = take(sizeof(double) * (size_t)P * N * AL);
    g = take(sizeof(double) * (size_t)P * AL); r = take(sizeof(double) * (size_t)UM_EP * RS);
    mean = take(sizeof(float) * UM_EP * MS); y0 = take(sizeof(float) * 2 * UM_EP * D);
    pidx = take(sizeof(int) * 2 * P);
    total = o;
  }
};
template <int D, int K1, int UM_EP>
__global__ void __launch_bounds__(UM_THREADS, 1)
uniform_main_kernel(TabDev tb, const double *__restrict__ ws, const float *__restrict__ smp_traj,
                    const float *__restrict__ mean, const float *__restrict__ init_pos,
                    const float *__restrict__ init_vel, const int64_t *__restrict__ pairs, int grad_mode,
                    const float *__restrict__ grad_logp, const float *__restrict__ logp_old,
                    const float *__restrict__ advantage, double grad_scale, double *__restrict__ loss_acc,
                    float *__restrict__ logp, int32_t *__restrict__ info, float *__restrict__ grad_mean,
                    double *__restrict__ apart, long long B, int T, int P) {
  using UL = UniLayout<D, K1>;
  using SM = UniMainSmem<D, K1, UM_EP>;
  constexpr int Dp = D * K1, N = 2 * D, NT = tri(N), AL = SM::AL, MS = SM::MS;
  const UL ul(P);
  const SM sm(P);
  extern __shared__ __align__(16) unsigned char smem_raw[];
  double *sX = reinterpret_cast<double *>(smem_raw + sm.X);
  double *sh = reinterpret_cast<double *>(smem_raw + sm.h);
  double *sxi = reinterpret_cast<double *>(smem_raw + sm.xi);
  double *shld = reinterpret_cast<double *>(smem_raw + sm.hld);
  double *sal = reinterpret_cast<double *>(smem_raw + sm.al);
  double *sg = reinterpret_cast<double *>(smem_raw + sm.g);
  double *sr = reinterpret_cast<double *>(smem_raw + sm.r);
  float *smean = reinterpret_cast<float *>(smem_raw + sm.mean);
  float *sy0 = reinterpret_cast<float *>(smem_raw + sm.y0);
  int *spidx = reinterpret_cast<int *>(smem_raw + sm.pidx);
  __shared__ double s_red[2 * (UM_THREADS / 32)];
  const int chained = (int)ws[ul.flags], nq = (int)ws[ul.flags + 1];
  const int warp = threadIdx.x >> 5, lane = threadIdx.x & 31, nwarps = UM_THREADS / 32;
  const int RS = sm.RS;
  const bool want_grad = grad_mode != 0;
  const double tau = tb.tau;
  for (int t = threadIdx.x; t < P * NT; t += UM_THREADS) sX[t] = ws[ul.xinv + t];
  for (int t = threadIdx.x; t < nq * K1; t += UM_THREADS) sh[t] = ws[ul.hm + t];
  for (int t = threadIdx.x; t < 2 * nq; t += UM_THREADS) sxi[t] = ws[ul.xi + t];
  for (int t = threadIdx.x; t < P; t += UM_THREADS) shld[t] = ws[ul.hld + t];
  for (int t = threadIdx.x; t < nq; t += UM_THREADS) spidx[t] = (int)point_time_index(pairs, chained, t, P);
  constexpr int MAXACC = 12;
  const int NE = P * (NT + 1);
  double racc[MAXACC];
#pragma unroll
  for (int u = 0; u < MAXACC; ++u) racc[u] = 0.0;
  double loss_part = 0.0, ratio_part = 0.0;
  const long long n_chunks = (B + UM_EP - 1) / UM_EP;
  for (long long ch = blockIdx.x; ch < n_chunks; ch += gridDim.x) {
    const long long bbase = ch * UM_EP;
    const int nb = (int)((B - bbase) < UM_EP ? (B - bbase) : UM_EP);
    __syncthreads();
    for (int t = threadIdx.x; t < nb * Dp; t += UM_THREADS) smean[(t / Dp) * MS + (t % Dp)] = mean[bbase * Dp + t];
    for (int t = threadIdx.x; t < nb * D; t += UM_THREADS) {
      sy0[t] = init_pos[bbase * D + t];
      sy0[UM_EP * D + t] = init_vel[bbase * D + t];
    }
    for (int t0 = threadIdx.x; t0 < nb * nq * D; t0 += 8 * UM_THREADS) {
      float v[8];
#pragma unroll
      for (int u = 0; u < 8; ++u) {
        const int t = t0 + u * UM_THREADS;
        if (t < nb * nq * D) {
          const int l = t / (nq * D), r = t - l * nq * D, q = r / D, d = r - q * D;
          v[u] = smp_traj[((bbase + l) * T + spidx[q]) * (2 * D) + d];
        }
      }
#pragma unroll
      for (int u = 0; u < 8; ++u) {
        const int t = t0 + u * UM_THREADS;
        if (t < nb * nq * D) { const int l = t / (nq * D); sr[(size_t)l * RS + (t - l * nq * D)] = (double)v[u]; }
      }
    }
    __syncthreads();
    for (int t = threadIdx.x; t < nb * nq * D; t += UM_THREADS) {
      const int l = t / (nq * D), r = t - l * nq * D, q = r / D, d = r - q * D;
      const double y0 = (double)sy0[l * D + d], v0 = (double)sy0[UM_EP * D + l * D + d] * tau;
      const double *hq = sh + (size_t)q * K1;
      const float *th = smean + l * MS + d * K1;
      double mu = sxi[2 * q] * y0 + sxi[2 * q + 1] * v0;
#pragma unroll
      for (int j = 0; j < K1; ++j) mu = fma(hq[j], (double)th[j], mu);
      if (tb.relative_goal) {
        const double shift = tb.relative_goal_scaled ? y0 : y0 / tb.scale[K1 - 1];
        mu = fma(hq[K1 - 1], shift, mu);
      }
      sr[(size_t)l * RS + r] -= mu;
    }
    __syncthreads();
    constexpr int PPW = 32 / UM_EP;
    const int el = lane % UM_EP;
    const long long b = bbase + el;
    for (int p = warp * PPW + lane / UM_EP; p < P; p += nwarps * PPW) {
      double g = 0.0, al[N];
#pragma unroll
      for (int i = 0; i < N; ++i) al[i] = 0.0;
      if (el < nb) {
        const double *X = sX + (size_t)p * NT;
        const double *r0 = sr + (size_t)el * RS + point_of(chained, p, 0) * D;
        const double *r1 = sr + (size_t)el * RS + point_of(chained, p, 1) * D;
        double r[N], z[N];
#pragma unroll
        for (int d = 0; d < D; ++d) { r[2 * d] = r0[d]; r[2 * d + 1] = r1[d]; }
        double maha = 0.0;
#pragma unroll
        for (int i = 0; i < N; ++i) {
          double v = 0.0;
#pragma unroll
          for (int j = 0; j <= i; ++j) v = fma(X[i * (i + 1) / 2 + j], r[j], v);
          z[i] = v;
          maha = fma(v, v, maha);
        }
        const double lp = -0.5 * ((double)N * LN_2PI + maha) - shld[p];
        const long long gid = b * P + p;
        if (logp) logp[gid] = (float)lp;
        if (info) info[gid] = 0;
        if (want_grad) {
          if (grad_mode == 2) {
            const double ratio = exp(lp - (double)logp_old[gid]);
            g = -ratio * (double)advantage[gid] * grad_scale;
            loss_part += g;
            ratio_part += ratio * grad_scale;
          } else {
            g = (double)grad_logp[gid];
          }
#pragma unroll
          for (int j = 0; j < N; ++j) {
            double v = 0.0;
#pragma unroll
            for (int i = j; i < N; ++i) v = fma(X[i * (i + 1) / 2 + j], z[i], v);
            al[j] = v;
          }
        }
      }
      if (want_grad) {
#pragma unroll
        for (int j = 0; j < N; ++j) sal[((size_t)p * N + j) * AL + el] = al[j];
        sg[(size_t)p * AL + el] = g;
      }
    }
    if (!want_grad) continue;
    __syncthreads();
    if (grad_mean) {
      for (int it = threadIdx.x; it < UM_EP * Dp; it += UM_THREADS) {
        const int o = it / UM_EP, l = it - o * UM_EP, d = o / K1, j = o - d * K1;
        if (l >= nb) continue;
        double acc0 = 0.0, acc1 = 0.0;
        for (int p = 0; p < P; ++p) {
          const double gg = sg[(size_t)p * AL + l];
          acc0 = fma(gg * sh[(size_t)point_of(chained, p, 0) * K1 + j], sal[((size_t)p * N + 2 * d) * AL + l], acc0);
          acc1 = fma(gg * sh[(size_t)point_of(chained, p, 1) * K1 + j], sal[((size_t)p * N + 2 * d + 1) * AL + l], acc1);
        }
        grad_mean[(bbase + l) * Dp + o] = (float)(acc0 + acc1);
      }
    }
    if (apart) {
      constexpr int nb_even = UM_EP;
#pragma unroll
      for (int u = 0; u < MAXACC; ++u) {
        const int e = threadIdx.x + u * UM_THREADS;
        if (e < NE) {
          const int p = e / (NT + 1), t = e - p * (NT + 1);
          const double *gp = sg + (size_t)p * AL;
          double a0 = 0.0, a1 = 0.0;
          if (t < NT) {
            int i, j;
            tri_decode(t, i, j);
            const double *ai = sal + ((size_t)p * N + i) * AL, *aj = sal + ((size_t)p * N + j) * AL;
#pragma unroll 4
            for (int l = 0; l < nb_even; l += 2) {
              a0 = fma(gp[l] * ai[l], aj[l], a0);
              a1 = fma(gp[l + 1] * ai[l + 1], aj[l + 1], a1);
            }
          } else {
            for (int l = 0; l < nb_even; ++l) a0 += gp[l];
          }
          racc[u] += a0 + a1;
        }
      }
    }
  }
  if (want_grad && apart) {
#pragma unroll
    for (int u = 0; u < MAXACC; ++u) {
      const int e = threadIdx.x + u * UM_THREADS;
      if (e < NE) apart[(size_t)blockIdx.x * NE + e] = racc[u];
    }
  }
  if (grad_mode == 2 && loss_acc) {
    loss_part = warp_sum(loss_part);
    ratio_part = warp_sum(ratio_part);
    if (lane == 0) { s_red[2 * warp] = loss_part; s_red[2 * warp + 1] = ratio_part; }
    __syncthreads();
    if (threadIdx.x == 0) {
      double a = 0.0, rr = 0.0;
      for (int w = 0; w < nwarps; ++w) { a += s_red[2 * w]; rr += s_red[2 * w + 1]; }
      if (rr != 0.0) { atomicAdd(loss_acc, a); atomicAdd(loss_acc + 1, rr); }
    }
  }
}

template <int D, int K1>
__global__ void __launch_bounds__(UT)
uniform_finish_kernel(double *ws, const double *__restrict__ apart, int nparts, const float *__restrict__ L,
                      const float *__restrict__ upstream, float *__restrict__ grad_L, double *__restrict__ grad_sigma,
                      int P) {
  using FL = FusedLayout<D, K1>;
  using UL = UniLayout<D, K1>;
  constexpr int Dp = FL::Dp, NT = FL::NT, NB = FL::NB, NR4 = FL::NR4, LD = FL::LD;
  static_assert(NT + 1 <= 128, "128 entry slots");
  const UL ul(P);
  extern __shared__ __align__(16) unsigned char smem_raw[];
  float *M = reinterpret_cast<float *>(smem_raw);
  float *Ls = M + NR4 * LD;
  double *G = reinterpret_cast<double *>(Ls + NR4 * LD + (NR4 * LD & 1));
  double *hm = G + (size_t)P * NT;
  __shared__ double s_part[8][129];
  __shared__ int s_last;
  const int NE = P * (NT + 1);
  const int p = blockIdx.x, t = threadIdx.x & 127, sl = threadIdx.x >> 7;
  unsigned int *ticket = reinterpret_cast<unsigned int *>(ws + ul.flags + 2);
  float lreg[(NR4 * NR4 + UT - 1) / UT];
#pragma unroll
  for (int u = 0; u < (NR4 * NR4 + UT - 1) / UT; ++u) {
    const int e = threadIdx.x + u * UT, i = e / NR4, c = e - i * NR4;
    lreg[u] = (L && e < NR4 * NR4 && i < Dp && c <= i) ? L[(size_t)i * Dp + c] : 0.f;
  }
  double a[4] = {0.0, 0.0, 0.0, 0.0};
  if (t <= NT) {
    const double *src = apart + (size_t)p * (NT + 1) + t;
    int k = sl;
    for (; k + 24 < nparts; k += 32) {
#pragma unroll
      for (int u = 0; u < 4; ++u) a[u] += src[(size_t)(k + 8 * u) * NE];
    }
    for (; k < nparts; k += 8) a[0] += src[(size_t)k * NE];
  }
  s_part[sl][t] = (a[0] + a[1]) + (a[2] + a[3]);
  __syncthreads();
  if (threadIdx.x <= NT) {
    double v = 0.0;
#pragma unroll
    for (int u = 0; u < 8; ++u) v += s_part[u][threadIdx.x];
    s_part[0][threadIdx.x] = v;
  }
  __syncthreads();
  if (threadIdx.x < NT)
    ws[ul.gbuf + (size_t)p * NT + threadIdx.x] =
        0.5 * (s_part[0][threadIdx.x] - s_part[0][NT] * ws[ul.cinv + (size_t)p * NT + threadIdx.x]);
  __threadfence();
  __syncthreads();
  if (threadIdx.x == 0) s_last = (atomicAdd(ticket, 1u) == gridDim.x - 1);
  __syncthreads();
  if (!s_last) return;
  __threadfence();
  const int chained = (int)ws[ul.flags], nq = (int)ws[ul.flags + 1];
  const float up = upstream ? *upstream : 1.0f;
  for (int e = threadIdx.x; e < P * NT; e += UT) G[e] = __ldcg(ws + ul.gbuf + e);
  for (int e = threadIdx.x; e < nq * K1; e += UT) hm[e] = ws[ul.hm + e];
  for (int e = threadIdx.x; e < NR4 * LD; e += UT) M[e] = 0.f;
#pragma unroll
  for (int u = 0; u < (NR4 * NR4 + UT - 1) / UT; ++u) {
    const int e = threadIdx.x + u * UT, i = e / NR4, c = e - i * NR4;
    if (e < NR4 * NR4) Ls[i * LD + c] = lreg[u];
  }
  __syncthreads();
  for (int task = threadIdx.x; task < NB * K1; task += UT) {
    const int blk = task / K1, i = task - blk * K1;
    int d, dd;
    tri_decode(blk, d, dd);
    const int r0 = 2 * d, q0 = 2 * dd;
    const int e00 = tri_idx(r0, q0), e10 = tri_idx(r0 + 1, q0), e11 = tri_idx(r0 + 1, q0 + 1);
    const int e01 = (d != dd) ? tri_idx(r0, q0 + 1) : e10;
    double acc[K1];
#pragma unroll
    for (int j = 0; j < K1; ++j) acc[j] = 0.0;
    for (int q = 0; q < nq; ++q) {
      const Links lk = links(chained, q, P);
      double w = 0.0;
      const double hqi = hm[(size_t)q * K1 + i];
      if (lk.pf >= 0) {
        const double *Gp = G + (size_t)lk.pf * NT;
        w += Gp[e00] * hqi + Gp[e10] * hm[(size_t)lk.nxt * K1 + i];
      }
      if (lk.ps >= 0) {
        const double *Gp = G + (size_t)lk.ps * NT;
        w += Gp[e11] * hqi + Gp[e01] * hm[(size_t)lk.prv * K1 + i];
      }
#pragma unroll
      for (int j = 0; j < K1; ++j) acc[j] = fma(w, hm[(size_t)q * K1 + j], acc[j]);
    }
#pragma unroll
    for (int j = 0; j < K1; ++j) {
      const float v = up * (float)acc[j];
      M[(d * K1 + i) * LD + dd * K1 + j] = v;
      if (d != dd) M[(dd * K1 + j) * LD + d * K1 + i] = v;
    }
  }
  __syncthreads();
  if (grad_sigma)
    for (int e = threadIdx.x; e < Dp * Dp; e += UT) grad_sigma[e] = (double)M[(e / Dp) * LD + (e % Dp)];
  if (grad_L) dl_from_dsigma<D, K1>(M, Ls, grad_L);
}

}

#define TCE_FOR_SHAPES(X) X(7, 9) X(4, 9) X(7, 4) X(3, 4) X(2, 3)

namespace {
constexpr size_t SMEM_LIMIT = 227 * 1024;

template <int D, int K1>
int fused_pick_E(int P, int chained) {
  int E = FT / P;
  if (E > FT / tri(D)) E = FT / tri(D);
  while (E > 1 && FusedLayout<D, K1>(E, P, chained).total > SMEM_LIMIT) --E;
  if (E < 1 || FusedLayout<D, K1>(E, P, chained).total > SMEM_LIMIT) return 0;
  return E;
}

int sm_count() {
  static int n = 0;
  if (!n) {
    int dev = 0;
    cudaGetDevice(&dev);
    cudaDeviceGetAttribute(&n, cudaDevAttrMultiProcessorCount, dev);
    if (n <= 0) n = 148;
  }
  return n;
}
}

extern "C" int tce_seglik_fused_config(const tce_tables_t *t, int64_t B, int64_t P, int chained, int32_t *E_out,
                                       int32_t *grid_out, int64_t *part_floats, int64_t *pre_doubles_per_episode) {
  if (!t || B < 0 || P < 1) return TCE_ERR_INVALID_ARGUMENT;
#define X(Dv, Kv)                                                                              \
  if (t->D == Dv && t->K1 == Kv) {                                                             \
    if (P > FT) return TCE_ERR_UNSUPPORTED_SHAPE;                                              \
    const int E = fused_pick_E<Dv, Kv>((int)P, chained);                                       \
    if (!E) return TCE_ERR_UNSUPPORTED_SHAPE;                                                  \
    const int64_t groups = (B + E - 1) / E;                                                    \
    int grid = (int)(groups < sm_count() ? groups : sm_count());                               \
    if (grid < 1) grid = 1;                                                                    \
    if (E_out) *E_out = E;                                                                     \
    if (grid_out) *grid_out = grid;                                                            \
                               \
    if (part_floats) *part_floats = ((int64_t)grid + 1) * tri(Dv) * Kv * Kv + 4;               \
    if (pre_doubles_per_episode)                                                               \
      *pre_doubles_per_episode = (int64_t)pre_doubles(chained ? (int)P + 1 : 2 * (int)P, Kv, 2 * Dv, (int)P); \
    return TCE_OK;                                                                             \
  }
  TCE_FOR_SHAPES(X)
#undef X
  return TCE_ERR_UNSUPPORTED_SHAPE;
}

template <bool SIGMA_IN>
static int prepass_launch(const tce_tables_t *t, const float *smp_traj, const float *mean, const float *L,
                          int64_t ldb_L, const double *Sigma0, const double *sigma_scale, const float *times,
                          const float *init_time, const float *init_pos, const float *init_vel,
                          const int64_t *pred_pairs, double *pre, double *diag_max, int chained, int64_t B, int64_t T,
                          int64_t P, void *stream) {
  if (B == 0) return TCE_OK;
  if (!t || !smp_traj || !mean || (SIGMA_IN ? !Sigma0 : !L) || !times || !init_time || !init_pos || !init_vel ||
      !pred_pairs || !pre || !diag_max || B < 0 || T < 1 || P < 1)
    return TCE_ERR_INVALID_ARGUMENT;
  cudaStream_t st = (cudaStream_t)stream;
#define X(Dv, Kv)                                                                                                  \
  if (t->D == Dv && t->K1 == Kv) {                                                                                 \
    using FL = FusedLayout<Dv, Kv>;                                                                                \
    const size_t smem = sizeof(double) * ((size_t)Dv * Kv * Kv + 2 * P * Kv + 4 * P + FL::IR) + 32 +               \
                        (SIGMA_IN ? 0 : sizeof(float) * FL::Dp * (FL::Dp + 1));                                    \
    if (smem > SMEM_LIMIT) return TCE_ERR_UNSUPPORTED_SHAPE;                                                       \
    auto kern = seglik_prepass_kernel<Dv, Kv, SIGMA_IN>;                                                           \
    TCE_CUDA(cudaFuncSetAttribute(kern, cudaFuncAttributeMaxDynamicSharedMemorySize, (int)smem), "prepass smem");  \
    int64_t grid = B;                                                                                              \
    const int64_t cap = (int64_t)sm_count() * 16;                                                                  \
    if (grid > cap) grid = cap;                                                                                    \
    kern<<<(unsigned)grid, PT, smem, st>>>(tab_dev(t), smp_traj, mean, L, ldb_L, Sigma0, sigma_scale, times,       \
                                           init_time, init_pos, init_vel, pred_pairs, pre, diag_max, (long long)B, \
                                           (int)T, (int)P, chained);                                               \
    TCE_CHECK_LAUNCH("seglik_prepass_kernel");                                                                     \
    return TCE_OK;                                                                                                 \
  }
  TCE_FOR_SHAPES(X)
#undef X
  return TCE_ERR_UNSUPPORTED_SHAPE;
}

extern "C" int tce_seglik_prepass(const tce_tables_t *t, const float *smp_traj, const float *mean, const float *L,
                                  int64_t ldb_L, const double *Sigma0, const double *sigma_scale, const float *times,
                                  const float *init_time, const float *init_pos, const float *init_vel,
                                  const int64_t *pred_pairs, double *pre, double *diag_max, int chained, int64_t B,
                                  int64_t T, int64_t P, void *stream) {
  if (Sigma0)
    return prepass_launch<true>(t, smp_traj, mean, nullptr, 0, Sigma0, sigma_scale, times, init_time, init_pos,
                                init_vel, pred_pairs, pre, diag_max, chained, B, T, P, stream);
  return prepass_launch<false>(t, smp_traj, mean, L, ldb_L, nullptr, nullptr, times, init_time, init_pos, init_vel,
                               pred_pairs, pre, diag_max, chained, B, T, P, stream);
}

template <bool SIGMA_IN>
static int fused_launch(const tce_tables_t *t, const double *pre, const float *L, int64_t ldb_L, const double *Sigma0,
                        const double *sigma_scale, const int64_t *pred_pairs, const double *diag_max, double reg_rel,
                        int grad_mode, const float *grad_logp, const float *logp_old, const float *advantage,
                        double grad_scale, double *loss_acc, float *logp, int32_t *info, float *grad_mean,
                        float *grad_L, float *dsigma_part, int chained, int64_t B, int64_t P, void *stream) {
  if (B == 0) return TCE_OK;
  if (!t || !pre || (SIGMA_IN ? !Sigma0 : !L) || !pred_pairs || !diag_max || B < 0 || P < 1 || grad_mode < 0 ||
      grad_mode > 2)
    return TCE_ERR_INVALID_ARGUMENT;
  if (grad_mode == 1 && !grad_logp) return TCE_ERR_INVALID_ARGUMENT;
  if (grad_mode == 2 && (!logp_old || !advantage)) return TCE_ERR_INVALID_ARGUMENT;
  const bool shared_cov = SIGMA_IN || ldb_L == 0;
  if (grad_mode && !shared_cov && dsigma_part) return TCE_ERR_INVALID_ARGUMENT;
  if (grad_mode && shared_cov && grad_L) return TCE_ERR_INVALID_ARGUMENT;
  cudaStream_t st = (cudaStream_t)stream;
  int32_t E = 0, grid = 0;
  int rc = tce_seglik_fused_config(t, B, P, chained, &E, &grid, nullptr, nullptr);
  if (rc != TCE_OK) return rc;
#define X(Dv, Kv)                                                                                                  \
  if (t->D == Dv && t->K1 == Kv) {                                                                                 \
    const size_t smem = FusedLayout<Dv, Kv>(E, (int)P, chained).total;                                             \
    auto kern = seglik_fused_kernel<Dv, Kv, SIGMA_IN>;                                                             \
    TCE_CUDA(cudaFuncSetAttribute(kern, cudaFuncAttributeMaxDynamicSharedMemorySize, (int)smem), "fused smem");    \
    kern<<<(unsigned)grid, FT, smem, st>>>(pre, L, ldb_L, Sigma0, sigma_scale, pred_pairs, diag_max, reg_rel,      \
                                           grad_mode, grad_logp, logp_old, advantage, grad_scale, loss_acc, logp,  \
                                           info, grad_mean, grad_L, dsigma_part, (long long)B, (int)P, (int)E,     \
                                           chained);                                                               \
    TCE_CHECK_LAUNCH("seglik_fused_kernel");                                                                       \
    return TCE_OK;                                                                                                 \
  }
  TCE_FOR_SHAPES(X)
#undef X
  return TCE_ERR_UNSUPPORTED_SHAPE;
}

extern "C" int tce_seglik_fused(const tce_tables_t *t, const double *pre, const float *L, int64_t ldb_L,
                                const double *Sigma0, const double *sigma_scale, const int64_t *pred_pairs,
                                const double *diag_max, double reg_rel, int grad_mode, const float *grad_logp,
                                const float *logp_old, const float *advantage, double grad_scale, double *loss_acc,
                                float *logp, int32_t *info, float *grad_mean, float *grad_L, float *dsigma_part,
                                int chained, int64_t B, int64_t P, void *stream) {
  if (Sigma0)
    return fused_launch<true>(t, pre, nullptr, 0, Sigma0, sigma_scale, pred_pairs, diag_max, reg_rel, grad_mode,
                              grad_logp, logp_old, advantage, grad_scale, loss_acc, logp, info, grad_mean, grad_L,
                              dsigma_part, chained, B, P, stream);
  return fused_launch<false>(t, pre, L, ldb_L, nullptr, nullptr, pred_pairs, diag_max, reg_rel, grad_mode, grad_logp,
                             logp_old, advantage, grad_scale, loss_acc, logp, info, grad_mean, grad_L, dsigma_part,
                             chained, B, P, stream);
}

extern "C" int tce_seglik_dsigma_reduce(const tce_tables_t *t, float *dsigma_part, int nparts, const float *L,
                                        const float *upstream, float *grad_L, double *grad_sigma, void *stream) {
  if (!t || !dsigma_part || nparts < 1 || (!grad_L && !grad_sigma) || (grad_L && !L)) return TCE_ERR_INVALID_ARGUMENT;
#define X(Dv, Kv)                                                                                               \
  if (t->D == Dv && t->K1 == Kv) {                                                                              \
    using FL = FusedLayout<Dv, Kv>;                                                                             \
    const size_t smem = sizeof(float) * 2 * FL::NR4 * FL::LD + 16;                                              \
    auto kern = dsigma_reduce_kernel<Dv, Kv>;                                                                   \
    TCE_CUDA(cudaFuncSetAttribute(kern, cudaFuncAttributeMaxDynamicSharedMemorySize, (int)smem), "reduce smem"); \
    const int NE = FL::NB * Kv * Kv;                                                                            \
    kern<<<(NE + 31) / 32, RT, smem, (cudaStream_t)stream>>>(dsigma_part, nparts, L, upstream, grad_L, grad_sigma); \
    TCE_CHECK_LAUNCH("dsigma_reduce_kernel");                                                                   \
    return TCE_OK;                                                                                              \
  }
  TCE_FOR_SHAPES(X)
#undef X
  return TCE_ERR_UNSUPPORTED_SHAPE;
}

extern "C" size_t tce_seglik_uniform_ws_doubles(const tce_tables_t *t, int64_t P) {
  if (!t || P < 1) return 0;
#define X(Dv, Kv) if (t->D == Dv && t->K1 == Kv) return UniLayout<Dv, Kv>((int)P).total;
  TCE_FOR_SHAPES(X)
#undef X
  return 0;
}

static int uniform_ep(int64_t B) { return B <= 8 * (int64_t)sm_count() ? 8 : 32; }
static int uniform_grid(int64_t B) {
  const int ep = uniform_ep(B);
  const int64_t chunks = (B + ep - 1) / ep;
  const int64_t cap = (int64_t)sm_count();
  return (int)(chunks < cap ? (chunks < 1 ? 1 : chunks) : cap);
}

extern "C" int tce_seglik_uniform_parts(const tce_tables_t *t, int64_t B, int64_t P, int32_t *nparts,
                                        int64_t *apart_doubles) {
  if (!t || P < 1 || B < 0) return TCE_ERR_INVALID_ARGUMENT;
  const int g = uniform_grid(B);
  const int64_t N = 2 * (int64_t)t->D, NT = N * (N + 1) / 2;
  if (P * (NT + 1) > 12 * UM_THREADS) return TCE_ERR_UNSUPPORTED_SHAPE;
  if (nparts) *nparts = g;
  if (apart_doubles) *apart_doubles = (int64_t)g * P * (NT + 1);
  return TCE_OK;
}

extern "C" int tce_seglik_uniform_prep(const tce_tables_t *t, const float *L, const double *Sigma0,
                                       const double *sigma_scale, const float *times, const float *init_time,
                                       const int64_t *pred_pairs, double *ws, double *diag_max, double reg_rel,
                                       int what, int64_t P, void *stream) {
  if (!t || (!L && !Sigma0) || !times || !init_time || !pred_pairs || !ws || !diag_max || P < 1 || !(what & 3))
    return TCE_ERR_INVALID_ARGUMENT;
  cudaStream_t st = (cudaStream_t)stream;
#define X(Dv, Kv)                                                                                                   \
  if (t->D == Dv && t->K1 == Kv) {                                                                                  \
    using FL = FusedLayout<Dv, Kv>;                                                                                 \
    const size_t sb = sizeof(double) * FL::NB * Kv * FL::KP, ls = sizeof(float) * FL::NR4 * FL::LD;                 \
    const size_t smem = (((sb > ls ? sb : ls) + 15) & ~(size_t)15) + sizeof(double) * (FL::IR + 2 * P * Kv) + 16;   \
    if (smem > SMEM_LIMIT) return TCE_ERR_UNSUPPORTED_SHAPE;                                                        \
    if ((what & 1) && Sigma0) {                                                                                     \
      auto kern = uniform_prep_kernel<Dv, Kv, true>;                                                                \
      TCE_CUDA(cudaFuncSetAttribute(kern, cudaFuncAttributeMaxDynamicSharedMemorySize, (int)smem), "uprep smem");   \
      kern<<<1, UT, smem, st>>>(tab_dev(t), nullptr, Sigma0, sigma_scale, times, init_time, pred_pairs, ws,         \
                                diag_max, reg_rel, (int)P, what);                                                   \
    } else if (what & 1) {                                                                                          \
      auto kern = uniform_prep_kernel<Dv, Kv, false>;                                                               \
      TCE_CUDA(cudaFuncSetAttribute(kern, cudaFuncAttributeMaxDynamicSharedMemorySize, (int)smem), "uprep smem");   \
      kern<<<1, UT, smem, st>>>(tab_dev(t), L, nullptr, nullptr, times, init_time, pred_pairs, ws, diag_max,        \
                                reg_rel, (int)P, what);                                                             \
    }                                                                                                               \
    if (what & 1) TCE_CHECK_LAUNCH("uniform_prep_kernel");                                                          \
    if (what & 2) uniform_factor_kernel<Dv, Kv><<<(unsigned)P, 32, 0, st>>>(ws, diag_max, reg_rel, (int)P);         \
    TCE_CHECK_LAUNCH("uniform_factor_kernel");                                                                      \
    return TCE_OK;                                                                                                  \
  }
  TCE_FOR_SHAPES(X)
#undef X
  return TCE_ERR_UNSUPPORTED_SHAPE;
}

extern "C" int tce_seglik_uniform_main(const tce_tables_t *t, const double *ws, const float *smp_traj,
                                       const float *mean, const float *init_pos, const float *init_vel,
                                       const int64_t *pred_pairs, int grad_mode, const float *grad_logp,
                                       const float *logp_old, const float *advantage, double grad_scale,
                                       double *loss_acc, float *logp, int32_t *info, float *grad_mean, double *apart,
                                       int64_t B, int64_t T, int64_t P, void *stream) {
  if (B == 0) return TCE_OK;
  if (!t || !ws || !smp_traj || !mean || !init_pos || !init_vel || !pred_pairs || B < 0 || T < 1 || P < 1 ||
      grad_mode < 0 || grad_mode > 2)
    return TCE_ERR_INVALID_ARGUMENT;
  if (grad_mode == 1 && !grad_logp) return TCE_ERR_INVALID_ARGUMENT;
  if (grad_mode == 2 && (!logp_old || !advantage)) return TCE_ERR_INVALID_ARGUMENT;
  const unsigned grid = (unsigned)uniform_grid(B);
#define X(Dv, Kv)                                                                                                  \
  if (t->D == Dv && t->K1 == Kv) {                                                                                 \
    constexpr int N = 2 * Dv, NT = N * (N + 1) / 2;                                                                \
    if (P * (NT + 1) > 12 * UM_THREADS) return TCE_ERR_UNSUPPORTED_SHAPE;                                          \
    if (uniform_ep(B) == 8) {                                                                                      \
      const size_t smem = UniMainSmem<Dv, Kv, 8>((int)P).total;                                                    \
      if (smem > SMEM_LIMIT) return TCE_ERR_UNSUPPORTED_SHAPE;                                                     \
      auto kern = uniform_main_kernel<Dv, Kv, 8>;                                                                  \
      TCE_CUDA(cudaFuncSetAttribute(kern, cudaFuncAttributeMaxDynamicSharedMemorySize, (int)smem), "umain smem");  \
      kern<<<grid, UM_THREADS, smem, (cudaStream_t)stream>>>(                                                      \
          tab_dev(t), ws, smp_traj, mean, init_pos, init_vel, pred_pairs, grad_mode, grad_logp, logp_old,          \
          advantage, grad_scale, loss_acc, logp, info, grad_mean, apart, (long long)B, (int)T, (int)P);            \
    } else {                                                                                                       \
      const size_t smem = UniMainSmem<Dv, Kv, 32>((int)P).total;                                                   \
      if (smem > SMEM_LIMIT) return TCE_ERR_UNSUPPORTED_SHAPE;                                                     \
      auto kern = uniform_main_kernel<Dv, Kv, 32>;                                                                 \
      TCE_CUDA(cudaFuncSetAttribute(kern, cudaFuncAttributeMaxDynamicSharedMemorySize, (int)smem), "umain smem");  \
      kern<<<grid, UM_THREADS, smem, (cudaStream_t)stream>>>(                                                      \
          tab_dev(t), ws, smp_traj, mean, init_pos, init_vel, pred_pairs, grad_mode, grad_logp, logp_old,          \
          advantage, grad_scale, loss_acc, logp, info, grad_mean, apart, (long long)B, (int)T, (int)P);            \
    }                                                                                                              \
    TCE_CHECK_LAUNCH("uniform_main_kernel");                                                                       \
    return TCE_OK;                                                                                                 \
  }
  TCE_FOR_SHAPES(X)
#undef X
  return TCE_ERR_UNSUPPORTED_SHAPE;
}

extern "C" int tce_seglik_uniform_finish(const tce_tables_t *t, double *ws, const double *apart, int nparts,
                                         const float *L, const float *upstream, float *grad_L, double *grad_sigma,
                                         int64_t P, void *stream) {
  if (!t || !ws || !apart || nparts < 1 || (!grad_L && !grad_sigma) || (grad_L && !L) || P < 1)
    return TCE_ERR_INVALID_ARGUMENT;
#define X(Dv, Kv)                                                                                          \
  if (t->D == Dv && t->K1 == Kv) {                                                                         \
    using FL = FusedLayout<Dv, Kv>;                                                                        \
    const size_t smem = sizeof(float) * (2 * FL::NR4 * FL::LD + 2) +                                       \
                        sizeof(double) * ((size_t)P * FL::NT + 2 * P * Kv) + 16;                           \
    if (smem > SMEM_LIMIT) return TCE_ERR_UNSUPPORTED_SHAPE;                                               \
    auto kern = uniform_finish_kernel<Dv, Kv>;                                                             \
    TCE_CUDA(cudaFuncSetAttribute(kern, cudaFuncAttributeMaxDynamicSharedMemorySize, (int)smem), "ufin smem"); \
    kern<<<(unsigned)P, UT, smem, (cudaStream_t)stream>>>(ws, apart, nparts, L, upstream, grad_L, grad_sigma, \
                                                          (int)P);                                         \
    TCE_CHECK_LAUNCH("uniform_finish_kernel");                                                             \
    return TCE_OK;                                                                                         \
  }
  TCE_FOR_SHAPES(X)
#undef X
  return TCE_ERR_UNSUPPORTED_SHAPE;
}
```

### tce_rl_b200/ops_seglik.py

```python
from __future__ import annotations

import ctypes as C
import warnings
import weakref
from typing import Optional, Tuple

import torch

from . import _lib
from ._lib import TceError

Tensor = torch.Tensor

_REG_GROUP = None
_GLOBAL_UNIFORM = False


def set_regulariser_group(group) -> None:
    global _REG_GROUP, _GLOBAL_UNIFORM
    _REG_GROUP = group
    _GLOBAL_UNIFORM = False


def sync_uniform(init_time: Tensor, times: Tensor) -> bool:
    global _GLOBAL_UNIFORM
    _GLOBAL_UNIFORM = False
    if _REG_GROUP is None:
        return False
    import torch.distributed as dist
    group = None if _REG_GROUP is True else _REG_GROUP
    local = times.shape[0] > 0 and times_uniform(init_time, times)
    if times.shape[0] > 0:
        row, t0 = times[0].double(), init_time[0].double().reshape(1)
        sig = torch.cat([t0, row.sum().reshape(1), (row * torch.arange(1, row.numel() + 1, device=row.device)).sum()
                         .reshape(1), torch.full((1,), float(local), device=row.device, dtype=torch.float64)])
    else:
        sig = None
    big = 1e300
    lo = sig.clone() if sig is not None else torch.full((4,), big, device=times.device, dtype=torch.float64)
    hi = sig.clone() if sig is not None else torch.full((4,), -big, device=times.device, dtype=torch.float64)
    dist.all_reduce(lo, op=dist.ReduceOp.MIN, group=group)
    dist.all_reduce(hi, op=dist.ReduceOp.MAX, group=group)
    _GLOBAL_UNIFORM = bool(torch.equal(lo, hi) and lo[3].item() == 1.0)
    return _GLOBAL_UNIFORM


def _reduce_diag_max(diag_max: Tensor) -> None:
    if _REG_GROUP is not None:
        import torch.distributed as dist
        dist.all_reduce(diag_max, op=dist.ReduceOp.MAX, group=None if _REG_GROUP is True else _REG_GROUP)


def _stream() -> int:
    return torch.cuda.current_stream().cuda_stream


def _p(t: Optional[Tensor]) -> Optional[int]:
    return None if t is None else t.data_ptr()


def _chk(t: Tensor, dtype=torch.float32, name="tensor") -> Tensor:
    if not t.is_cuda:
        raise TceError(f"{name} must be a CUDA tensor (tce_rl_b200 has no CPU path)")
    if t.dtype != dtype:
        raise TceError(f"{name} must be {dtype}, got {t.dtype}")
    return t.contiguous()


class _IdCache:

    def __init__(self):
        self._d = {}

    def get(self, t: Tensor):
        ent = self._d.get(id(t))
        return ent[1] if ent is not None and ent[0]() is t else None

    def put(self, t: Tensor, value) -> None:
        key = id(t)
        self._d[key] = (weakref.ref(t, lambda _r, k=key, d=self._d: d.pop(k, None)), value)


_PAIR_FACTS = _IdCache()
_TIME_FACTS = _IdCache()


def pairs_chained(pred_pairs: Tensor) -> bool:
    key = _PAIR_FACTS.get(pred_pairs)
    if key is not None and key[0] == pred_pairs._version:
        return key[1]
    if pred_pairs.is_cuda and torch.cuda.is_current_stream_capturing():
        return False
    pp = pred_pairs.detach().cpu()
    res = bool(pp.shape[0] >= 1 and (pp.shape[0] == 1 or bool((pp[:-1, 1] == pp[1:, 0]).all())))
    _PAIR_FACTS.put(pred_pairs, (pred_pairs._version, res))
    return res


_WARNED_CAPTURE = False


def times_uniform(init_time: Tensor, times: Tensor) -> bool:
    sig = (times._version, init_time.data_ptr(), init_time._version)
    key = _TIME_FACTS.get(times)
    if key is not None and key[0] == sig:
        return key[1]
    if times.is_cuda and torch.cuda.is_current_stream_capturing():
        global _WARNED_CAPTURE
        if not _WARNED_CAPTURE:
            _WARNED_CAPTURE = True
            warnings.warn("tce_rl_b200: time grid of a dataset first seen during CUDA-graph capture -- the capture cannot "
                          "read the device, so the general-grid likelihood is recorded (slower than the common-grid "
                          "path); run one eager epoch on these tensors first or call ops_seglik.declare_uniform")
        return False
    res = bool(times.shape[0] >= 1 and bool(((times == times[:1]).all() & (init_time == init_time[:1]).all()).item()))
    _TIME_FACTS.put(times, (sig, res))
    return res


def declare_uniform(init_time: Tensor, times: Tensor, value: bool) -> None:
    _TIME_FACTS.put(times, ((times._version, init_time.data_ptr(), init_time._version), bool(value)))


def shared_factor(L: Tensor, batch: int) -> Optional[Tensor]:
    n = L.shape[-1]
    if L.dim() == 2:
        return L.reshape(1, n, n)
    if L.dim() != 3:
        return None
    if L.shape[0] == 1:
        return L if L.is_contiguous() else L.contiguous()
    if L.stride(0) == 0 and L.stride(1) == n and L.stride(2) == 1:
        first = getattr(L, "_tce_first", None)
        if first is not None:
            return first
        base = L._base
        if base is not None and base.numel() == n * n and base.shape[-2:] == (n, n) and base.is_contiguous() \
                and base.data_ptr() == L.data_ptr():
            return base.reshape(1, n, n)
        return L[:1]
    return None


def fused_config(tables: int, B: int, P: int, chained: bool) -> dict:
    lib = _lib.load()
    E, grid, part, pre = C.c_int32(), C.c_int32(), C.c_int64(), C.c_int64()
    _lib.check(lib.tce_seglik_fused_config(tables, max(B, 1), P, int(chained), C.byref(E), C.byref(grid),
                                           C.byref(part), C.byref(pre)), "tce_seglik_fused_config")
    nparts, apart = C.c_int32(), C.c_int64()
    rc = lib.tce_seglik_uniform_parts(tables, max(B, 1), P, C.byref(nparts), C.byref(apart))
    return {"E": E.value, "grid": grid.value, "part_floats": part.value, "pre_doubles": pre.value,
            "ws_doubles": lib.tce_seglik_uniform_ws_doubles(tables, P),
            "uni_parts": nparts.value if rc == 0 else 0, "apart_doubles": apart.value if rc == 0 else 0}


@torch.library.custom_op("tce::seglik", mutates_args=())
def seglik(smp_traj: Tensor, mean: Tensor, L: Optional[Tensor], sigma: Optional[Tensor],
           sigma_scale: Optional[Tensor], times: Tensor, init_time: Tensor, init_pos: Tensor, init_vel: Tensor,
           pred_pairs: Tensor, tables: int, reg_rel: float, grad_mode: int, grad_logp: Optional[Tensor],
           logp_old: Optional[Tensor], advantage: Optional[Tensor], chained: bool, uniform: bool,
           want_grad_L: bool, want_grad_sigma: bool = False) -> Tuple[Tensor, Tensor, Tensor, Tensor, Tensor, Tensor]:
    smp_traj, mean, times = _chk(smp_traj, name="smp_traj"), _chk(mean, name="mean"), _chk(times, name="times")
    init_time, init_pos, init_vel = _chk(init_time), _chk(init_pos), _chk(init_vel)
    pairs = _chk(pred_pairs, torch.int64, "pred_pairs")
    B, T = times.shape
    P, Dp = pairs.shape[0], mean.shape[-1]
    dev = mean.device
    if L is None and sigma is None:
        raise TceError("either L or sigma is required")
    if L is not None:
        L = _chk(L, name="L")
        if L.dim() != 3 or L.shape[0] not in (1, B):
            raise TceError("L must be [B, n, n] or [1, n, n]")
    shared = sigma is not None or L.shape[0] == 1
    ldb = 0 if shared else Dp * Dp
    if sigma is not None:
        if sigma.dtype != torch.float64 or not sigma.is_cuda or not sigma.is_contiguous() or sigma.numel() != Dp * Dp:
            raise TceError("sigma must be a contiguous CUDA float64 [Dp, Dp] tensor")
    if uniform and not shared:
        raise TceError("the uniform path needs a shared covariance")
    logp = torch.empty(B, P, device=dev, dtype=torch.float32)
    info = torch.empty(B, P, device=dev, dtype=torch.int32)
    acc = torch.zeros(3, device=dev, dtype=torch.float64)
    diag_max, stats = acc[:1], acc[1:]
    want = grad_mode != 0
    g_mean = torch.empty(B, Dp, device=dev, dtype=torch.float32) if want else mean.new_empty(0)
    need_L = want and want_grad_L
    need_S = want and want_grad_sigma
    if need_S and not shared:
        raise TceError("grad_sigma exists for a shared covariance only")
    g_L = mean.new_empty(0)
    g_S = mean.new_empty(0, dtype=torch.float64)
    if B == 0:
        if need_L:
            g_L = torch.zeros(1 if shared else 0, Dp, Dp, device=dev, dtype=torch.float32)
        if need_S:
            g_S = torch.zeros(Dp, Dp, device=dev, dtype=torch.float64)
        return logp, info, acc, g_mean, g_L, g_S
    if need_L and shared and L is None:
        raise TceError("grad_L of a shared covariance needs its factor L")
    st = _stream()
    cfg = fused_config(tables, B, P, chained)
    scale = 1.0 / (B * P)
    if uniform and cfg["uni_parts"] == 0:
        uniform = False
    if uniform:
        ws = torch.empty(cfg["ws_doubles"], device=dev, dtype=torch.float64)
        Lp = None if sigma is not None else _p(L)
        if _REG_GROUP is None or (_GLOBAL_UNIFORM and shared):
            _lib.call("tce_seglik_uniform_prep", tables, Lp, _p(sigma), _p(sigma_scale), _p(times), _p(init_time),
                      _p(pairs), _p(ws), _p(diag_max), float(reg_rel), 3, P, st)
        else:
            _lib.call("tce_seglik_uniform_prep", tables, Lp, _p(sigma), _p(sigma_scale), _p(times), _p(init_time),
                      _p(pairs), _p(ws), _p(diag_max), float(reg_rel), 1, P, st)
            _reduce_diag_max(diag_max)
            _lib.call("tce_seglik_uniform_prep", tables, Lp, _p(sigma), _p(sigma_scale), _p(times), _p(init_time),
                      _p(pairs), _p(ws), _p(diag_max), float(reg_rel), 2, P, st)
        apart = torch.empty(cfg["apart_doubles"], device=dev, dtype=torch.float64) if (need_L or need_S) else None
        _lib.call("tce_seglik_uniform_main", tables, _p(ws), _p(smp_traj), _p(mean), _p(init_pos), _p(init_vel),
                  _p(pairs), int(grad_mode), _p(grad_logp), _p(logp_old), _p(advantage), scale, _p(stats), _p(logp),
                  _p(info), _p(g_mean) if want else None, _p(apart), B, T, P, st)
        if need_L or need_S:
            if need_L:
                g_L = torch.empty(1, Dp, Dp, device=dev, dtype=torch.float32)
            if need_S:
                g_S = torch.empty(Dp, Dp, device=dev, dtype=torch.float64)
            _lib.call("tce_seglik_uniform_finish", tables, _p(ws), _p(apart), cfg["uni_parts"],
                      _p(L) if need_L else None, None, _p(g_L) if need_L else None, _p(g_S) if need_S else None, P, st)
        return logp, info, acc, g_mean, g_L, g_S
    pre = torch.empty(B * cfg["pre_doubles"], device=dev, dtype=torch.float64)
    _lib.call("tce_seglik_prepass", tables, _p(smp_traj), _p(mean), None if sigma is not None else _p(L), ldb,
              _p(sigma), _p(sigma_scale), _p(times), _p(init_time), _p(init_pos), _p(init_vel), _p(pairs), _p(pre),
              _p(diag_max), int(chained), B, T, P, st)
    _reduce_diag_max(diag_max)
    part = None
    if need_L or need_S:
        if shared:
            part = torch.empty(cfg["part_floats"], device=dev, dtype=torch.float32)
        else:
            g_L = torch.empty(B, Dp, Dp, device=dev, dtype=torch.float32)
    _lib.call("tce_seglik_fused", tables, _p(pre), None if sigma is not None else _p(L), ldb, _p(sigma),
              _p(sigma_scale), _p(pairs), _p(diag_max), float(reg_rel), int(grad_mode), _p(grad_logp), _p(logp_old),
              _p(advantage), scale, _p(stats), _p(logp), _p(info), _p(g_mean) if want else None,
              _p(g_L) if (need_L and not shared) else None, _p(part), int(chained), B, P, st)
    if (need_L or need_S) and shared:
        if need_L:
            g_L = torch.empty(1, Dp, Dp, device=dev, dtype=torch.float32)
        if need_S:
            g_S = torch.empty(Dp, Dp, device=dev, dtype=torch.float64)
        _lib.call("tce_seglik_dsigma_reduce", tables, _p(part), cfg["grid"], _p(L) if need_L else None, None,
                  _p(g_L) if need_L else None, _p(g_S) if need_S else None, st)
    return logp, info, acc, g_mean, g_L, g_S


@seglik.register_fake
def _(smp_traj, mean, L, sigma, sigma_scale, times, init_time, init_pos, init_vel, pred_pairs, tables, reg_rel,
      grad_mode, grad_logp, logp_old, advantage, chained, uniform, want_grad_L, want_grad_sigma=False):
    B, P, Dp = times.shape[0], pred_pairs.shape[0], mean.shape[-1]
    shared = sigma is not None or L.shape[0] == 1
    want = grad_mode != 0
    return (mean.new_empty(B, P), mean.new_empty(B, P, dtype=torch.int32), mean.new_empty(3, dtype=torch.float64),
            mean.new_empty(B, Dp) if want else mean.new_empty(0),
            mean.new_empty(1 if shared else B, Dp, Dp) if (want and want_grad_L) else mean.new_empty(0),
            mean.new_empty(Dp, Dp, dtype=torch.float64) if (want and want_grad_sigma) else
            mean.new_empty(0, dtype=torch.float64))


def _resolve(L: Tensor, B: int, sigma):
    first = shared_factor(L, B)
    if first is not None:
        return first, True
    if sigma is not None:
        raise TceError("sigma describes ONE covariance: pass the shared factor with it")
    return L, False


class _SegLogProb(torch.autograd.Function):

    @staticmethod
    def forward(ctx, smp_traj, mean, L, times, init_time, init_pos, init_vel, pred_pairs, tables, reg_rel, chained,
                uniform, sigma, sigma_scale):
        logp, info, acc, _, _, _ = seglik(smp_traj, mean, L, sigma, sigma_scale, times, init_time, init_pos, init_vel,
                                          pred_pairs, tables, reg_rel, 0, None, None, None, chained, uniform, False)
        diag_max = acc[:1]
        ctx.save_for_backward(smp_traj, mean, L, times, init_time, init_pos, init_vel, pred_pairs)
        ctx.sig = (sigma, sigma_scale)
        ctx.args = (tables, reg_rel, chained, uniform)
        ctx.mark_non_differentiable(info, diag_max)
        ctx.set_materialize_grads(False)
        return logp, info, diag_max

    @staticmethod
    def backward(ctx, g_logp, g_info, g_diag):
        if g_logp is None:
            return (None,) * 14
        smp_traj, mean, L, times, init_time, init_pos, init_vel, pred_pairs = ctx.saved_tensors
        tables, reg_rel, chained, uniform = ctx.args
        need_S = ctx.sig[0] is not None and ctx.needs_input_grad[12]
        need_L = ctx.needs_input_grad[2] and not need_S
        _, _, _, g_mean, g_L, g_S = seglik(smp_traj, mean, L, ctx.sig[0], ctx.sig[1], times, init_time, init_pos,
                                           init_vel, pred_pairs, tables, reg_rel, 1, g_logp.contiguous(), None, None,
                                           chained, uniform, need_L, need_S)
        return (None, g_mean if ctx.needs_input_grad[1] else None, g_L if need_L else None) + (None,) * 9 + (
            g_S.view_as(ctx.sig[0]) if need_S else None, None)


_UNIT = {}


def unit_seed(device, dtype) -> Tensor:
    key = (str(device), dtype)
    if key not in _UNIT:
        _UNIT[key] = torch.ones((), device=device, dtype=dtype)
    return _UNIT[key]


class _SegSurrogate(torch.autograd.Function):

    @staticmethod
    def forward(ctx, smp_traj, mean, L, times, init_time, init_pos, init_vel, pred_pairs, logp_old, advantage, tables,
                reg_rel, chained, uniform, sigma, sigma_scale):
        need_S = sigma is not None and bool(ctx.needs_input_grad[14])
        need_L = bool(ctx.needs_input_grad[2]) and not need_S
        logp, info, acc, g_mean, g_L, g_S = seglik(smp_traj, mean, L, sigma, sigma_scale, times, init_time, init_pos,
                                                   init_vel, pred_pairs, tables, reg_rel, 2, None, logp_old, advantage,
                                                   chained, uniform, need_L, need_S)
        s32 = acc[1:].to(torch.float32)
        ctx.save_for_backward(g_mean, g_L, g_S.view_as(sigma) if need_S else g_S)
        ctx.need_L, ctx.need_S = need_L, need_S
        ctx.mark_non_differentiable(logp, info)
        ctx.set_materialize_grads(False)
        return s32[0], s32[1], logp, info

    @staticmethod
    def backward(ctx, g_loss, g_ratio, g_logp, g_info):
        if g_loss is None:
            return (None,) * 16
        g_mean, g_L, g_S = ctx.saved_tensors
        if g_loss is not unit_seed(g_loss.device, g_loss.dtype):
            g_mean = g_mean * g_loss
            g_L = g_L * g_loss if ctx.need_L else g_L
            g_S = g_S * g_loss if ctx.need_S else g_S
        return (None, g_mean if ctx.needs_input_grad[1] else None, g_L if ctx.need_L else None) + (None,) * 11 + (
            g_S if ctx.need_S else None, None)


def _facts(pred_pairs, init_time, times, shared, uniform):
    chained = pairs_chained(pred_pairs)
    if uniform is None:
        uniform = shared and times_uniform(init_time, times)
    return chained, bool(uniform and shared)


PER_EPISODE_STAGED = True


def seg_logprob(smp_traj, mean, L, times, init_time, init_pos, init_vel, pred_pairs, tables, reg_rel: float = 1e-4,
                return_info: bool = False, uniform: Optional[bool] = None, sigma=None):
    Lr, shared = _resolve(L, times.shape[0], sigma)
    if not shared and PER_EPISODE_STAGED and times.shape[0] > 0:
        from . import ops
        return ops.seg_logprob_staged(smp_traj, mean, L, times, init_time, init_pos, init_vel, pred_pairs, tables,
                                      reg_rel, return_info)
    chained, uni = _facts(pred_pairs, init_time, times, shared, uniform)
    logp, info, diag_max = _SegLogProb.apply(smp_traj, mean, Lr, times, init_time, init_pos, init_vel, pred_pairs,
                                             tables.handle, float(reg_rel), chained, uni,
                                             None if sigma is None else sigma[0], None if sigma is None else sigma[1])
    return (logp, info, diag_max) if return_info else logp


def diag_strides(L: Tensor, name: str = "L") -> Tuple[int, int]:
    if not L.is_cuda or L.dtype != torch.float32 or L.dim() != 3 or L.shape[-1] != L.shape[-2]:
        raise TceError(f"{name} must be a CUDA float32 [B, n, n] tensor")
    return (0 if L.shape[0] == 1 else L.stride(0)), L.stride(1) + L.stride(2)


def _dense_diag_grad(L: Tensor) -> Tuple[Tensor, int, int]:
    n = L.shape[-1]
    return torch.zeros(L.shape[0], n, n, device=L.device, dtype=torch.float32), n * n, n + 1


@torch.library.custom_op("tce::seglik_diag_fwd", mutates_args=())
def seglik_diag_fwd(smp_traj: Tensor, mean: Tensor, L: Tensor, times: Tensor, init_time: Tensor, init_pos: Tensor,
                    init_vel: Tensor, pred_pairs: Tensor, tables: int, reg_rel: float) -> Tuple[Tensor, Tensor, Tensor]:
    smp_traj, mean, times = _chk(smp_traj, name="smp_traj"), _chk(mean, name="mean"), _chk(times, name="times")
    init_time, init_pos, init_vel = _chk(init_time), _chk(init_pos), _chk(init_vel)
    pairs = _chk(pred_pairs, torch.int64, "pred_pairs")
    ldb, inc = diag_strides(L)
    B, T = times.shape
    P = pairs.shape[0]
    dev = mean.device
    diag_max = torch.zeros(1, device=dev, dtype=torch.float64)
    logp = torch.empty(B, P, device=dev, dtype=torch.float32)
    info = torch.empty(B, P, device=dev, dtype=torch.int32)
    if B == 0:
        return logp, diag_max, info
    st = _stream()
    _lib.call("tce_seglik_diag_max", tables, _p(L), ldb, inc, _p(times), _p(init_time), _p(pairs), _p(diag_max), B, T,
              P, st)
    _reduce_diag_max(diag_max)
    _lib.call("tce_seglik_diag_fwd", tables, _p(smp_traj), _p(mean), _p(L), ldb, inc, _p(times), _p(init_time),
              _p(init_pos), _p(init_vel), _p(pairs), _p(diag_max), float(reg_rel), _p(logp), _p(info), B, T, P, st)
    return logp, diag_max, info


@seglik_diag_fwd.register_fake
def _(smp_traj, mean, L, times, init_time, init_pos, init_vel, pred_pairs, tables, reg_rel):
    B, P = times.shape[0], pred_pairs.shape[0]
    return mean.new_empty(B, P), mean.new_empty(1, dtype=torch.float64), mean.new_empty(B, P, dtype=torch.int32)


@torch.library.custom_op("tce::seglik_diag_bwd", mutates_args=())
def seglik_diag_bwd(grad_logp: Tensor, smp_traj: Tensor, mean: Tensor, L: Tensor, times: Tensor, init_time: Tensor,
                    init_pos: Tensor, init_vel: Tensor, pred_pairs: Tensor, diag_max: Tensor, tables: int,
                    reg_rel: float) -> Tuple[Tensor, Tensor]:
    grad_logp = _chk(grad_logp, name="grad_logp")
    smp_traj, mean, times = _chk(smp_traj), _chk(mean), _chk(times)
    init_time, init_pos, init_vel = _chk(init_time), _chk(init_pos), _chk(init_vel)
    pairs = _chk(pred_pairs, torch.int64, "pred_pairs")
    ldb, inc = diag_strides(L)
    B, T = times.shape
    g_mean = torch.empty(B, mean.shape[-1], device=mean.device, dtype=torch.float32)
    g_L, ldb_g, inc_g = _dense_diag_grad(L)
    if B == 0:
        return g_mean, g_L
    _lib.call("tce_seglik_diag_bwd", tables, _p(smp_traj), _p(mean), _p(L), ldb, inc, _p(times), _p(init_time),
              _p(init_pos), _p(init_vel), _p(pairs), _p(diag_max), float(reg_rel), _p(grad_logp), _p(g_mean), _p(g_L),
              ldb_g, inc_g, B, T, pairs.shape[0], _stream())
    return g_mean, g_L


@seglik_diag_bwd.register_fake
def _(grad_logp, smp_traj, mean, L, times, init_time, init_pos, init_vel, pred_pairs, diag_max, tables, reg_rel):
    return mean.new_empty(mean.shape), L.new_empty(L.shape)


def _seglik_diag_setup(ctx, inputs, output):
    ctx.save_for_backward(*inputs[:8], output[1])
    ctx.tables, ctx.reg_rel = inputs[8], inputs[9]
    ctx.set_materialize_grads(False)


def _seglik_diag_backward(ctx, g_logp, g_diag, g_info):
    if g_logp is None:
        return (None,) * 10
    smp_traj, mean, L, times, init_time, init_pos, init_vel, pred_pairs, diag_max = ctx.saved_tensors
    g_mean, g_L = seglik_diag_bwd(g_logp.contiguous(), smp_traj, mean, L, times, init_time, init_pos, init_vel,
                                  pred_pairs, diag_max, ctx.tables, ctx.reg_rel)
    return (None, g_mean if ctx.needs_input_grad[1] else None, g_L if ctx.needs_input_grad[2] else None) + (None,) * 7


seglik_diag_fwd.register_autograd(_seglik_diag_backward, setup_context=_seglik_diag_setup)


def seg_logprob_diag(smp_traj, mean, L, times, init_time, init_pos, init_vel, pred_pairs, tables, reg_rel: float = 1e-4,
                     return_info: bool = False):
    logp, diag_max, info = seglik_diag_fwd(smp_traj, mean, L, times, init_time, init_pos, init_vel, pred_pairs,
                                           tables.handle, float(reg_rel))
    return (logp, info, diag_max) if return_info else logp


def seg_surrogate(smp_traj, mean, L, times, init_time, init_pos, init_vel, pred_pairs, logp_old, advantage, tables,
                  reg_rel: float = 1e-4, uniform: Optional[bool] = None, sigma=None):
    if sigma is None:
        sigma = getattr(L, "_tce_sigma", None)
        if sigma is not None:
            sigma = sigma[:2]
    Lr, shared = _resolve(L, times.shape[0], sigma)
    if not shared:
        sigma = None
        if PER_EPISODE_STAGED and times.shape[0] > 0:
            from . import ops
            return ops.seg_surrogate_staged(smp_traj, mean, L, times, init_time, init_pos, init_vel, pred_pairs,
                                            _chk(logp_old, name="logp_old"), _chk(advantage, name="advantage"),
                                            tables, reg_rel)
    chained, uni = _facts(pred_pairs, init_time, times, shared, uniform)
    loss, ratio, logp, _ = _SegSurrogate.apply(smp_traj, mean, Lr, times, init_time, init_pos, init_vel, pred_pairs,
                                               _chk(logp_old, name="logp_old"), _chk(advantage, name="advantage"),
                                               tables.handle, float(reg_rel), chained, uni,
                                               None if sigma is None else sigma[0],
                                               None if sigma is None else sigma[1])
    return loss, ratio.detach(), logp
```

Baseline: 5.055 million.

## Fuse uniform seglik prep, factor and finish kernels into fewer launches

The separate prep, per-pair factor and finish kernels of the uniform segment-likelihood path are merged. One factor kernel now has each block build its own covariance block and Cholesky factor in shared memory, replacing the global scratch buffer and the extra 32-thread launch. The finish reduction moves into the main kernel's tail using ticket counters, and the host-side zeros allocation becomes an in-kernel reset. This removes kernel launches and global round-trips per policy update, at the cost of redundant per-block basis and covariance setup and a last-block-done reduction pattern.

```diff
diff --git a/include/tce_b200.h b/include/tce_b200.h
--- a/include/tce_b200.h
+++ b/include/tce_b200.h
@@ -182,18 +182,16 @@
 size_t tce_seglik_uniform_ws_doubles(const tce_tables_t *tables, int64_t P);
 int tce_seglik_uniform_parts(const tce_tables_t *tables, int64_t B, int64_t P, int32_t *nparts,
                              int64_t *apart_doubles);
-int tce_seglik_uniform_prep(const tce_tables_t *tables, const float *L, const double *Sigma0,
-                            const double *sigma_scale, const float *times, const float *init_time,
-                            const int64_t *pred_pairs, double *ws, double *diag_max, double reg_rel, int what,
-                            int64_t P, void *stream);
-int tce_seglik_uniform_main(const tce_tables_t *tables, const double *ws, const float *smp_traj, const float *mean,
+int tce_seglik_uniform_factor(const tce_tables_t *tables, const float *L, const double *Sigma0,
+                              const double *sigma_scale, const float *times, const float *init_time,
+                              const int64_t *pred_pairs, double *ws, double *acc, double reg_rel, int what, int64_t P,
+                              void *stream);
+int tce_seglik_uniform_main(const tce_tables_t *tables, double *ws, const float *smp_traj, const float *mean,
                             const float *init_pos, const float *init_vel, const int64_t *pred_pairs, int grad_mode,
                             const float *grad_logp, const float *logp_old, const float *advantage,
                             double grad_scale, double *loss_acc, float *logp, int32_t *info, float *grad_mean,
-                            double *apart, int64_t B, int64_t T, int64_t P, void *stream);
-int tce_seglik_uniform_finish(const tce_tables_t *tables, double *ws, const double *apart, int nparts,
-                              const float *L, const float *upstream, float *grad_L, double *grad_sigma, int64_t P,
-                              void *stream);
+                            double *apart, const float *L, const float *upstream, float *grad_L, double *grad_sigma,
+                            int64_t B, int64_t T, int64_t P, void *stream);
 
 int tce_gae(const float *rewards, const float *values, const uint8_t *dones, const uint8_t *tl_dones,
             float gamma, float lam, int use_gae, float *adv, float *ret, int64_t B, int64_t T,
diff --git a/tce_rl_b200/_lib.py b/tce_rl_b200/_lib.py
--- a/tce_rl_b200/_lib.py
+++ b/tce_rl_b200/_lib.py
@@ -93,10 +93,9 @@
     "tce_seglik_dsigma_reduce": (C.c_int, [_P, _P, _I32, _P, _P, _P, _P, _P]),
     "tce_seglik_uniform_ws_doubles": (C.c_size_t, [_P, _I64]),
     "tce_seglik_uniform_parts": (C.c_int, [_P, _I64, _I64, C.POINTER(C.c_int32), C.POINTER(C.c_int64)]),
-    "tce_seglik_uniform_prep": (C.c_int, [_P, _P, _P, _P, _P, _P, _P, _P, _P, _D, _I32, _I64, _P]),
-    "tce_seglik_uniform_main": (C.c_int, [_P, _P, _P, _P, _P, _P, _P, _I32, _P, _P, _P, _D, _P, _P, _P, _P, _P, _I64,
-                                          _I64, _I64, _P]),
-    "tce_seglik_uniform_finish": (C.c_int, [_P, _P, _P, _I32, _P, _P, _P, _P, _I64, _P]),
+    "tce_seglik_uniform_factor": (C.c_int, [_P, _P, _P, _P, _P, _P, _P, _P, _P, _D, _I32, _I64, _P]),
+    "tce_seglik_uniform_main": (C.c_int, [_P, _P, _P, _P, _P, _P, _P, _I32, _P, _P, _P, _D, _P, _P, _P, _P, _P, _P,
+                                          _P, _P, _P, _I64, _I64, _I64, _P]),
     "tce_p2p_allreduce_sumsq": (C.c_int, [_I32, _I32, _P, _P, _I64, _P, _P, _P, _P]),
     "tce_p2p_allreduce_sumsq_range": (C.c_int, [_I32, _I32, _P, _P, _I64, _I64, _I32, _I32, _P, _P, _P, _P]),
     "tce_p2p_push_xchg_bytes": (C.c_size_t, [_I32, _I64]),
diff --git a/tce_rl_b200/csrc/tce_seglik_fused.cu b/tce_rl_b200/csrc/tce_seglik_fused.cu
--- a/tce_rl_b200/csrc/tce_seglik_fused.cu
+++ b/tce_rl_b200/csrc/tce_seglik_fused.cu
@@ -871,28 +871,52 @@
   if (grad_L) dl_from_dsigma<D, K1>(M, Ls, grad_L);
 }
 
+constexpr int UNI_GROUP = 8;
+constexpr int UNI_TICKETS = 64;
 template <int D, int K1>
 struct UniLayout {
   static constexpr int N = 2 * D, NT = tri(N);
-  size_t hm, xi, xinv, cinv, gbuf, hld, flags, total;
+  size_t hm, xi, xinv, cinv, hld, flags, tickets, total;
   __host__ __device__ UniLayout(int P) {
     size_t o = 0;
     auto take = [&](size_t n) { size_t at = o; o += (n + 1) & ~(size_t)1; return at; };
     hm = take((size_t)2 * P * K1); xi = take((size_t)4 * P); xinv = take((size_t)P * NT);
-    cinv = take((size_t)P * NT); gbuf = take((size_t)P * NT); hld = take(P); flags = take(4); total = o;
+    cinv = take((size_t)P * NT); hld = take(P); flags = take(2); tickets = take(UNI_TICKETS / 2); total = o;
   }
 };
 
-constexpr int UT = 1024;
+template <int K1, int KP>
+__device__ __forceinline__ void block_times_h(const double *Sb, const double *hq, double (&h)[K1], double (&v)[K1]) {
+#pragma unroll
+  for (int j = 0; j < K1; ++j) h[j] = hq[j];
+#pragma unroll
+  for (int i = 0; i < K1; ++i) {
+    double a0 = 0.0, a1 = 0.0;
+#pragma unroll
+    for (int j = 0; j + 1 < K1; j += 2) { a0 = fma(Sb[i * KP + j], h[j], a0); a1 = fma(Sb[i * KP + j + 1], h[j + 1], a1); }
+    if (K1 & 1) a0 = fma(Sb[i * KP + K1 - 1], h[K1 - 1], a0);
+    v[i] = a0 + a1;
+  }
+}
+template <int K1>
+__device__ __forceinline__ double dot_k(const double *a, const double (&v)[K1]) {
+  double s = 0.0;
+#pragma unroll
+  for (int i = 0; i < K1; ++i) s = fma(a[i], v[i], s);
+  return s;
+}
+
+constexpr int UF = 256;
 template <int D, int K1, bool SIGMA_IN>
-__global__ void __launch_bounds__(UT)
-uniform_prep_kernel(TabDev tb, const float *__restrict__ L, const double *__restrict__ Sigma0,
-                    const double *__restrict__ sigma_scale, const float *__restrict__ times,
-                    const float *__restrict__ init_time, const int64_t *__restrict__ pairs, double *ws,
-                    double *diag_max, double reg_rel, int P, int what) {
+__global__ void __launch_bounds__(UF)
+uniform_factor_kernel(TabDev tb, const float *__restrict__ L, const double *__restrict__ Sigma0,
+                      const double *__restrict__ sigma_scale, const float *__restrict__ times,
+                      const float *__restrict__ init_time, const int64_t *__restrict__ pairs, double *ws, double *acc,
+                      double reg_rel, int P, int what) {
   using FL = FusedLayout<D, K1>;
   using UL = UniLayout<D, K1>;
   constexpr int Dp = FL::Dp, N = FL::N, NT = FL::NT, NB = FL::NB, KP = FL::KP, NR4 = FL::NR4, LD = FL::LD, IR = FL::IR;
+  static_assert(N <= 32, "lane = row");
   extern __shared__ __align__(16) unsigned char smem_raw[];
   const UL ul(P);
   double *Sblk = reinterpret_cast<double *>(smem_raw);
@@ -900,194 +924,184 @@
   const size_t sb = sizeof(double) * NB * K1 * KP, ls = sizeof(float) * NR4 * LD;
   double *irow = reinterpret_cast<double *>(smem_raw + (((sb > ls ? sb : ls) + 15) & ~(size_t)15));
   double *hm = irow + IR;
-  __shared__ double s_max[UT / 32];
+  double *xis = hm + (size_t)2 * P * K1;
+  __shared__ double s_max[UF / 32], Cp[NT], Sf[NT], Xs[NT], dinv[N], s_hld;
   const int warp = threadIdx.x >> 5, lane = threadIdx.x & 31;
+  const int p = blockIdx.x;
   const int chained = block_chained(pairs, P);
   const int nq = chained ? P + 1 : 2 * P;
-  double *g_c = ws + ul.xinv;
+  if (threadIdx.x <= K1) init_row_entry<K1>(tb, (double)init_time[0], threadIdx.x, irow);
+  if (SIGMA_IN) {
+    const double sc = sigma_scale ? *sigma_scale : 1.0;
+    for (int e0 = threadIdx.x; e0 < Dp * Dp; e0 += 4 * UF) {
+      double v[4];
+#pragma unroll
+      for (int u = 0; u < 4; ++u) v[u] = (e0 + u * UF < Dp * Dp) ? Sigma0[e0 + u * UF] : 0.0;
+#pragma unroll
+      for (int u = 0; u < 4; ++u) {
+        const int e = e0 + u * UF, i = e / Dp, j = e - i * Dp;
+        if (e < Dp * Dp && j <= i) sblk_store<K1, KP>(Sblk, i, j, sc * v[u]);
+      }
+    }
+    __syncthreads();
+  } else {
+    for (int e0 = threadIdx.x; e0 < NR4 * NR4; e0 += 4 * UF) {
+      float v[4];
+#pragma unroll
+      for (int u = 0; u < 4; ++u) {
+        const int e = e0 + u * UF, i = e / NR4, c = e - i * NR4;
+        v[u] = (e < NR4 * NR4 && i < Dp && c <= i) ? L[(size_t)i * Dp + c] : 0.f;
+      }
+#pragma unroll
+      for (int u = 0; u < 4; ++u) {
+        const int e = e0 + u * UF, i = e / NR4, c = e - i * NR4;
+        if (e < NR4 * NR4) Ls[i * LD + c] = v[u];
+      }
+    }
+    __syncthreads();
+    float vals[(Dp * (Dp + 1) / 2 + UF - 1) / UF];
+    int cnt = 0;
+    for (int t = threadIdx.x; t < tri(Dp); t += UF, ++cnt) {
+      int i, j;
+      tri_decode(t, i, j);
+      const float *a = Ls + i * LD, *bq = Ls + j * LD;
+      float a0 = 0.f, a1 = 0.f;
+      int k = 0;
+      for (; k + 1 <= j; k += 2) { a0 = fmaf(a[k], bq[k], a0); a1 = fmaf(a[k + 1], bq[k + 1], a1); }
+      if (k <= j) a0 = fmaf(a[k], bq[k], a0);
+      vals[cnt] = a0 + a1;
+    }
+    __syncthreads();
+    cnt = 0;
+    for (int t = threadIdx.x; t < tri(Dp); t += UF, ++cnt) {
+      int i, j;
+      tri_decode(t, i, j);
+      sblk_store<K1, KP>(Sblk, i, j, (double)vals[cnt]);
+    }
+    __syncthreads();
+  }
+  for (int it = threadIdx.x; it < nq * (K1 + 1); it += UF) {
+    const int q = it / (K1 + 1), j = it - q * (K1 + 1);
+    basis_entry<K1>(tb, irow, (double)times[point_time_index(pairs, chained, q, P)], j, hm + (size_t)q * K1,
+                    xis + 2 * q);
+  }
+  __syncthreads();
+  if (p == 0 && (what & 2)) {
+    for (int t = threadIdx.x; t < nq * K1; t += UF) ws[ul.hm + t] = hm[t];
+    for (int t = threadIdx.x; t < 2 * nq; t += UF) ws[ul.xi + t] = xis[t];
+  }
+  double dmax;
   if (what & 1) {
-    if (threadIdx.x <= K1) init_row_entry<K1>(tb, (double)init_time[0], threadIdx.x, irow);
-    if (SIGMA_IN) {
-      const double sc = sigma_scale ? *sigma_scale : 1.0;
-      for (int e0 = threadIdx.x; e0 < Dp * Dp; e0 += 4 * UT) {
-        double v[4];
-#pragma unroll
-        for (int u = 0; u < 4; ++u) v[u] = (e0 + u * UT < Dp * Dp) ? Sigma0[e0 + u * UT] : 0.0;
-#pragma unroll
-        for (int u = 0; u < 4; ++u) {
-          const int e = e0 + u * UT, i = e / Dp, j = e - i * Dp;
-          if (e < Dp * Dp && j <= i) sblk_store<K1, KP>(Sblk, i, j, sc * v[u]);
-        }
-      }
-      __syncthreads();
-    } else {
-      for (int e0 = threadIdx.x; e0 < NR4 * NR4; e0 += 4 * UT) {
-        float v[4];
-#pragma unroll
-        for (int u = 0; u < 4; ++u) {
-          const int e = e0 + u * UT, i = e / NR4, c = e - i * NR4;
-          v[u] = (e < NR4 * NR4 && i < Dp && c <= i) ? L[(size_t)i * Dp + c] : 0.f;
-        }
-#pragma unroll
-        for (int u = 0; u < 4; ++u) {
-          const int e = e0 + u * UT, i = e / NR4, c = e - i * NR4;
-          if (e < NR4 * NR4) Ls[i * LD + c] = v[u];
-        }
-      }
-      __syncthreads();
-      float vals[(Dp * (Dp + 1) / 2 + UT - 1) / UT];
-      int cnt = 0;
-      for (int t = threadIdx.x; t < tri(Dp); t += UT, ++cnt) {
-        int i, j;
-        tri_decode(t, i, j);
-        const float *a = Ls + i * LD, *bq = Ls + j * LD;
-        float a0 = 0.f, a1 = 0.f;
-        int k = 0;
-        for (; k + 1 <= j; k += 2) { a0 = fmaf(a[k], bq[k], a0); a1 = fmaf(a[k + 1], bq[k + 1], a1); }
-        if (k <= j) a0 = fmaf(a[k], bq[k], a0);
-        vals[cnt] = a0 + a1;
-      }
-      __syncthreads();
-      cnt = 0;
-      for (int t = threadIdx.x; t < tri(Dp); t += UT, ++cnt) {
-        int i, j;
-        tri_decode(t, i, j);
-        sblk_store<K1, KP>(Sblk, i, j, (double)vals[cnt]);
-      }
-      __syncthreads();
-    }
-    for (int it = threadIdx.x; it < nq * (K1 + 1); it += UT) {
-      const int q = it / (K1 + 1), j = it - q * (K1 + 1);
-      double xr[2];
-      basis_entry<K1>(tb, irow, (double)times[point_time_index(pairs, chained, q, P)], j, hm + (size_t)q * K1, xr);
-      if (j < K1) ws[ul.hm + (size_t)q * K1 + j] = hm[(size_t)q * K1 + j];
-      else { ws[ul.xi + 2 * q] = xr[0]; ws[ul.xi + 2 * q + 1] = xr[1]; }
-    }
-    __syncthreads();
     double my_max = 0.0;
-    for (int it = threadIdx.x; it < NB * nq; it += UT) {
-      const int blk = it / nq, q = it - blk * nq;
-      int d, dd;
-      tri_decode(blk, d, dd);
-      const Links lk = links(chained, q, P);
+    for (int it = threadIdx.x; it < D * nq; it += UF) {
+      const int d = it / nq, q = it - d * nq;
       double h[K1], v[K1];
-      const double *Sb = sblk_at<K1, KP>(Sblk, blk), *hq = hm + (size_t)q * K1;
-#pragma unroll
-      for (int j = 0; j < K1; ++j) h[j] = hq[j];
-#pragma unroll
-      for (int i = 0; i < K1; ++i) {
-        double a0 = 0.0, a1 = 0.0;
-#pragma unroll
-        for (int j = 0; j + 1 < K1; j += 2) { a0 = fma(Sb[i * KP + j], h[j], a0); a1 = fma(Sb[i * KP + j + 1], h[j + 1], a1); }
-        if (K1 & 1) a0 = fma(Sb[i * KP + K1 - 1], h[K1 - 1], a0);
-        v[i] = a0 + a1;
-      }
-      double kuu = 0.0;
-#pragma unroll
-      for (int i = 0; i < K1; ++i) kuu = fma(h[i], v[i], kuu);
-      const int r0 = 2 * d, q0 = 2 * dd;
-      if (lk.pf >= 0) {
-        const double *hn = hm + (size_t)lk.nxt * K1;
-        double kup = 0.0;
-#pragma unroll
-        for (int i = 0; i < K1; ++i) kup = fma(hn[i], v[i], kup);
-        g_c[(size_t)lk.pf * NT + tri_idx(r0, q0)] = kuu;
-        g_c[(size_t)lk.pf * NT + tri_idx(r0 + 1, q0)] = kup;
-      }
-      if (lk.ps >= 0) {
-        g_c[(size_t)lk.ps * NT + tri_idx(r0 + 1, q0 + 1)] = kuu;
-        if (d != dd) {
-          const double *hp = hm + (size_t)lk.prv * K1;
-          double kum = 0.0;
-#pragma unroll
-          for (int i = 0; i < K1; ++i) kum = fma(hp[i], v[i], kum);
-          g_c[(size_t)lk.ps * NT + tri_idx(r0, q0 + 1)] = kum;
-        }
-      }
-      if (d == dd) my_max = fmax(my_max, kuu);
+      block_times_h<K1, KP>(sblk_at<K1, KP>(Sblk, tri_idx(d, d)), hm + (size_t)q * K1, h, v);
+      my_max = fmax(my_max, dot_k<K1>(h, v));
     }
     my_max = warp_max(my_max);
     if (lane == 0) s_max[warp] = my_max;
     __syncthreads();
-    if (threadIdx.x == 0) {
-      double m = 0.0;
-      for (int w = 0; w < UT / 32; ++w) m = fmax(m, s_max[w]);
-      atomic_max_pos_double(diag_max, m);
-      ws[ul.flags] = (double)chained;
-      ws[ul.flags + 1] = (double)nq;
-      *reinterpret_cast<unsigned int *>(ws + ul.flags + 2) = 0u;
-    }
-  }
-}
-
-template <int D, int K1>
-__global__ void __launch_bounds__(32)
-uniform_factor_kernel(double *ws, const double *__restrict__ diag_max, double reg_rel, int P) {
-  using UL = UniLayout<D, K1>;
-  constexpr int N = 2 * D, NT = tri(N);
-  static_assert(N <= 32, "lane = row");
-  const UL ul(P);
-  __shared__ double A[NT], X[NT], dinv[N];
-  const int p = blockIdx.x, lane = threadIdx.x;
-  const double reg = reg_rel * (*diag_max);
-  double *g_x = ws + ul.xinv + (size_t)p * NT;
-  for (int t = lane; t < NT; t += 32) A[t] = g_x[t];
-  __syncwarp();
-  double hld = 0.0;
-  const int i = lane;
-  for (int j = 0; j < N; ++j) {
-    double s = 0.0;
-    if (i >= j && i < N) {
-      s = A[tri_idx(i, j)] + (i == j ? reg : 0.0);
-      const double *ri = A + tri_idx(i, 0), *rj = A + tri_idx(j, 0);
-      double s1 = 0.0;
-      int k = 0;
-      for (; k + 1 < j; k += 2) { s = fma(-ri[k], rj[k], s); s1 = fma(-ri[k + 1], rj[k + 1], s1); }
-      if (k < j) s = fma(-ri[k], rj[k], s);
-      s += s1;
-    }
-    const double d = __shfl_sync(0xffffffffu, s, j);
-    double inv = (double)rsqrtf((float)d);
-    inv = inv * fma(-0.5 * d, inv * inv, 1.5);
-    inv = inv * fma(-0.5 * d, inv * inv, 1.5);
-    hld += 0.5 * log(d);
+    dmax = 0.0;
+    for (int w = 0; w < UF / 32; ++w) dmax = fmax(dmax, s_max[w]);
+    if (p == 0 && threadIdx.x == 0) acc[0] = dmax;
+    if (what == 1) return;
+  } else {
+    dmax = *acc;
+  }
+  if (p == 0 && threadIdx.x == 0) {
+    acc[1] = 0.0;
+    acc[2] = 0.0;
+    ws[ul.flags] = (double)chained;
+    ws[ul.flags + 1] = (double)nq;
+  }
+  if (p == 0 && threadIdx.x < UNI_TICKETS) reinterpret_cast<unsigned int *>(ws + ul.tickets)[threadIdx.x] = 0u;
+  if (threadIdx.x < 2 * NB) {
+    const int blk = threadIdx.x >> 1, k = threadIdx.x & 1, q = point_of(chained, p, k);
+    int d, dd;
+    tri_decode(blk, d, dd);
+    const int r0 = 2 * d, q0 = 2 * dd;
+    double h[K1], v[K1];
+    block_times_h<K1, KP>(sblk_at<K1, KP>(Sblk, blk), hm + (size_t)q * K1, h, v);
+    const double kuu = dot_k<K1>(h, v);
+    if (k == 0) {
+      Cp[tri_idx(r0, q0)] = kuu;
+      Cp[tri_idx(r0 + 1, q0)] = dot_k<K1>(hm + (size_t)point_of(chained, p, 1) * K1, v);
+    } else {
+      Cp[tri_idx(r0 + 1, q0 + 1)] = kuu;
+      if (d != dd) Cp[tri_idx(r0, q0 + 1)] = dot_k<K1>(hm + (size_t)point_of(chained, p, 0) * K1, v);
+    }
+  }
+  __syncthreads();
+  if (warp == 0) {
+    const double reg = reg_rel * dmax;
+    const int i = lane;
+    double a[N];
+#pragma unroll
+    for (int c = 0; c < N; ++c) {
+      const int r = i < c ? c : i, cc = i < c ? i : c;
+      a[c] = i < N ? Cp[tri_idx(r < N ? r : 0, cc < N ? cc : 0)] + (c == i ? reg : 0.0) : 0.0;
+    }
+    double mprod = 1.0, my_inv = 0.0;
+    int esum = 0;
+#pragma unroll
+    for (int j = 0; j < N; ++j) {
+      const double dj = __shfl_sync(0xffffffffu, a[j], j);
+      double inv = (double)rsqrtf((float)dj);
+      inv = inv * fma(-0.5 * dj, inv * inv, 1.5);
+      inv = inv * fma(-0.5 * dj, inv * inv, 1.5);
+      int e;
+      mprod *= frexp(dj, &e);
+      esum += e;
+      if (i == j) my_inv = inv;
+      const double l = a[j] * inv;
+      a[j] = l;
+#pragma unroll
+      for (int k = j + 1; k < N; ++k) a[k] = fma(-l, __shfl_sync(0xffffffffu, l, k), a[k]);
+    }
+    if (i < N) {
+#pragma unroll
+      for (int c = 0; c < N; ++c)
+        if (c < i) Sf[tri_idx(i, c)] = a[c];
+      dinv[i] = my_inv;
+    }
+    if (lane == 0) s_hld = 0.5 * (log(mprod) + (double)esum * 0.6931471805599453);
     __syncwarp();
-    if (i == j) { A[tri_idx(j, j)] = d * inv; dinv[j] = inv; }
-    else if (i > j && i < N) A[tri_idx(i, j)] = s * inv;
-    __syncwarp();
-  }
-  if (lane < N) {
-    const int j = lane;
-    double x[N];
-#pragma unroll
-    for (int r = 0; r < N; ++r) {
-      double v = (r == j) ? 1.0 : 0.0;
-#pragma unroll
-      for (int k = 0; k < r; ++k) v = fma(-A[r * (r + 1) / 2 + k], (k >= j) ? x[k] : 0.0, v);
-      x[r] = (r >= j) ? v * dinv[r] : 0.0;
-    }
-#pragma unroll
-    for (int r = 0; r < N; ++r)
-      if (r >= j) X[tri_idx(r, j)] = x[r];
-  }
-  __syncwarp();
-  for (int t = lane; t < NT; t += 32) {
+    if (lane < N) {
+      const int j = lane;
+      double x[N];
+#pragma unroll
+      for (int r = 0; r < N; ++r) {
+        double v = (r == j) ? 1.0 : 0.0;
+#pragma unroll
+        for (int k = 0; k < r; ++k) v = fma(-Sf[r * (r + 1) / 2 + k], (k >= j) ? x[k] : 0.0, v);
+        x[r] = (r >= j) ? v * dinv[r] : 0.0;
+      }
+#pragma unroll
+      for (int r = 0; r < N; ++r)
+        if (r >= j) Xs[tri_idx(r, j)] = x[r];
+    }
+  }
+  __syncthreads();
+  for (int t = threadIdx.x; t < NT; t += UF) {
     int r, c;
     tri_decode(t, r, c);
     double v = 0.0;
-    for (int k = r; k < N; ++k) v = fma(X[tri_idx(k, r)], X[tri_idx(k, c)], v);
+    for (int k = r; k < N; ++k) v = fma(Xs[tri_idx(k, r)], Xs[tri_idx(k, c)], v);
     ws[ul.cinv + (size_t)p * NT + t] = v;
-    g_x[t] = X[t];
-  }
-  if (lane == 0) ws[ul.hld + p] = hld;
+    ws[ul.xinv + (size_t)p * NT + t] = Xs[t];
+  }
+  if (threadIdx.x == 0) ws[ul.hld + p] = s_hld;
 }
 
 constexpr int UM_THREADS = 256;
+__host__ __device__ inline int uni_record(int P, int NT) { return (P * (NT + 1) + 2 + 1) & ~1; }
 template <int D, int K1, int EP>
 struct UniMainSmem {
   static constexpr int UM_EP = EP;
   static constexpr int Dp = D * K1, N = 2 * D, NT = tri(N), AL = UM_EP + 1, MS = Dp | 1;
-  size_t X, h, xi, hld, al, g, mean, r, y0, pidx, total;
+  static constexpr int NR4 = FusedLayout<D, K1>::NR4, LD = FusedLayout<D, K1>::LD;
+  size_t X, h, xi, hld, al, g, mean, r, y0, pidx, tg, tm, tl, total;
   int RS;
   __host__ __device__ UniMainSmem(int P) {
     size_t o = 0;
@@ -1098,18 +1112,163 @@
     g = take(sizeof(double) * (size_t)P * AL); r = take(sizeof(double) * (size_t)UM_EP * RS);
     mean = take(sizeof(float) * UM_EP * MS); y0 = take(sizeof(float) * 2 * UM_EP * D);
     pidx = take(sizeof(int) * 2 * P);
-    total = o;
+    const size_t main_end = o;
+    o = al;
+    tg = take(sizeof(double) * uni_record(P, NT)); tm = take(sizeof(float) * NR4 * LD);
+    tl = take(sizeof(float) * NR4 * LD);
+    total = o > main_end ? o : main_end;
   }
 };
+
+template <int U2>
+__device__ __forceinline__ void sum_records(const double2 *src, int cnt, int n2, double2 *dst) {
+  double2 s[U2];
+#pragma unroll
+  for (int u = 0; u < U2; ++u) s[u] = make_double2(0.0, 0.0);
+  for (int k0 = 0; k0 < cnt; k0 += 4) {
+    double2 v[U2][4];
+#pragma unroll
+    for (int u = 0; u < U2; ++u) {
+      const int e = threadIdx.x + u * UM_THREADS;
+#pragma unroll
+      for (int j = 0; j < 4; ++j)
+        v[u][j] = (e < n2 && k0 + j < cnt) ? src[(size_t)(k0 + j) * n2 + e] : make_double2(0.0, 0.0);
+    }
+#pragma unroll
+    for (int u = 0; u < U2; ++u)
+#pragma unroll
+      for (int j = 0; j < 4; ++j)
+        if (k0 + j < cnt) { s[u].x += v[u][j].x; s[u].y += v[u][j].y; }
+  }
+#pragma unroll
+  for (int u = 0; u < U2; ++u) {
+    const int e = threadIdx.x + u * UM_THREADS;
+    if (e < n2) dst[e] = s[u];
+  }
+}
+
+template <int D, int K1, int UM_EP>
+__device__ __noinline__ void uniform_tail(double *apart, double *ws, const float *__restrict__ L,
+                                          const float *__restrict__ upstream, float *__restrict__ grad_L,
+                                          double *__restrict__ grad_sigma, double *__restrict__ loss_acc, int P) {
+  using FL = FusedLayout<D, K1>;
+  constexpr int Dp = FL::Dp, NT = FL::NT, NB = FL::NB, NR4 = FL::NR4, LD = FL::LD;
+  constexpr int U2 = (12 * UM_THREADS + 3) / 2 / UM_THREADS + 1;
+  using UL = UniLayout<D, K1>;
+  using SM = UniMainSmem<D, K1, UM_EP>;
+  extern __shared__ __align__(16) unsigned char smem_raw[];
+  const UL ul(P);
+  const SM sm(P);
+  double *Gs = reinterpret_cast<double *>(smem_raw + sm.tg);
+  float *M = reinterpret_cast<float *>(smem_raw + sm.tm);
+  float *Ls = reinterpret_cast<float *>(smem_raw + sm.tl);
+  const double *hm = reinterpret_cast<const double *>(smem_raw + sm.h);
+  const double *cinv = ws + ul.cinv;
+  unsigned int *tickets = reinterpret_cast<unsigned int *>(ws + ul.tickets);
+  const int chained = (int)ws[ul.flags], nq = (int)ws[ul.flags + 1];
+  const int NE = P * (NT + 1), NRec = uni_record(P, NT);
+  __shared__ int s_last;
+  const int nparts = gridDim.x, ngroups = (nparts + UNI_GROUP - 1) / UNI_GROUP, n2 = NRec / 2;
+  const int grp = blockIdx.x / UNI_GROUP, c0 = grp * UNI_GROUP;
+  const int gsz = nparts - c0 < UNI_GROUP ? nparts - c0 : UNI_GROUP;
+  double *gsum = apart + (size_t)nparts * NRec;
+  __threadfence();
+  __syncthreads();
+  if (threadIdx.x == 0) s_last = atomicAdd(tickets + 1 + grp, 1u) == (unsigned int)(gsz - 1);
+  __syncthreads();
+  if (!s_last) return;
+  __threadfence();
+  sum_records<U2>(reinterpret_cast<const double2 *>(apart + (size_t)c0 * NRec), gsz, n2,
+                  reinterpret_cast<double2 *>(gsum + (size_t)grp * NRec));
+  __threadfence();
+  __syncthreads();
+  if (threadIdx.x == 0) s_last = atomicAdd(tickets, 1u) == (unsigned int)(ngroups - 1);
+  __syncthreads();
+  if (!s_last) return;
+  __threadfence();
+  constexpr int LC = (NR4 * NR4 + UM_THREADS - 1) / UM_THREADS;
+  float lreg[LC];
+#pragma unroll
+  for (int u = 0; u < LC; ++u) {
+    const int e = threadIdx.x + u * UM_THREADS, i = e / NR4, c = e - i * NR4;
+    lreg[u] = (grad_L && e < NR4 * NR4 && i < Dp && c <= i) ? L[(size_t)i * Dp + c] : 0.f;
+  }
+  sum_records<U2>(reinterpret_cast<const double2 *>(gsum), ngroups, n2, reinterpret_cast<double2 *>(Gs));
+  for (int e = threadIdx.x; e < NR4 * LD; e += UM_THREADS) M[e] = 0.f;
+#pragma unroll
+  for (int u = 0; u < LC; ++u) {
+    const int e = threadIdx.x + u * UM_THREADS, i = e / NR4, c = e - i * NR4;
+    if (e < NR4 * NR4) Ls[i * LD + c] = lreg[u];
+  }
+  __syncthreads();
+  if (threadIdx.x == 0 && loss_acc) { loss_acc[0] = Gs[NE]; loss_acc[1] = Gs[NE + 1]; }
+  if (!grad_L && !grad_sigma) return;
+  constexpr int GC = (12 * UM_THREADS) / (NT + 1) * NT / UM_THREADS + 1;
+  double ci[GC];
+#pragma unroll
+  for (int u = 0; u < GC; ++u) {
+    const int e = threadIdx.x + u * UM_THREADS;
+    ci[u] = e < P * NT ? cinv[e] : 0.0;
+  }
+#pragma unroll
+  for (int u = 0; u < GC; ++u) {
+    const int e = threadIdx.x + u * UM_THREADS;
+    if (e < P * NT) {
+      const int p = e / NT, t = e - p * NT;
+      double *row = Gs + (size_t)p * (NT + 1);
+      row[t] = 0.5 * (row[t] - row[NT] * ci[u]);
+    }
+  }
+  __syncthreads();
+  const float up = upstream ? *upstream : 1.0f;
+  for (int task = threadIdx.x; task < NB * K1; task += UM_THREADS) {
+    const int blk = task / K1, i = task - blk * K1;
+    int d, dd;
+    tri_decode(blk, d, dd);
+    const int r0 = 2 * d, q0 = 2 * dd;
+    const int e00 = tri_idx(r0, q0), e10 = tri_idx(r0 + 1, q0), e11 = tri_idx(r0 + 1, q0 + 1);
+    const int e01 = (d != dd) ? tri_idx(r0, q0 + 1) : e10;
+    double acc[K1];
+#pragma unroll
+    for (int j = 0; j < K1; ++j) acc[j] = 0.0;
+    for (int q = 0; q < nq; ++q) {
+      const Links lk = links(chained, q, P);
+      double w = 0.0;
+      const double hqi = hm[(size_t)q * K1 + i];
+      if (lk.pf >= 0) {
+        const double *Gp = Gs + (size_t)lk.pf * (NT + 1);
+        w += Gp[e00] * hqi + Gp[e10] * hm[(size_t)lk.nxt * K1 + i];
+      }
+      if (lk.ps >= 0) {
+        const double *Gp = Gs + (size_t)lk.ps * (NT + 1);
+        w += Gp[e11] * hqi + Gp[e01] * hm[(size_t)lk.prv * K1 + i];
+      }
+#pragma unroll
+      for (int j = 0; j < K1; ++j) acc[j] = fma(w, hm[(size_t)q * K1 + j], acc[j]);
+    }
+#pragma unroll
+    for (int j = 0; j < K1; ++j) {
+      const float v = up * (float)acc[j];
+      M[(d * K1 + i) * LD + dd * K1 + j] = v;
+      if (d != dd) M[(dd * K1 + j) * LD + d * K1 + i] = v;
+    }
+  }
+  __syncthreads();
+  if (grad_sigma)
+    for (int e = threadIdx.x; e < Dp * Dp; e += UM_THREADS) grad_sigma[e] = (double)M[(e / Dp) * LD + (e % Dp)];
+  if (grad_L) dl_from_dsigma<D, K1>(M, Ls, grad_L);
+}
+
 template <int D, int K1, int UM_EP>
 __global__ void __launch_bounds__(UM_THREADS, 1)
-uniform_main_kernel(TabDev tb, const double *__restrict__ ws, const float *__restrict__ smp_traj,
-                    const float *__restrict__ mean, const float *__restrict__ init_pos,
-                    const float *__restrict__ init_vel, const int64_t *__restrict__ pairs, int grad_mode,
-                    const float *__restrict__ grad_logp, const float *__restrict__ logp_old,
-                    const float *__restrict__ advantage, double grad_scale, double *__restrict__ loss_acc,
-                    float *__restrict__ logp, int32_t *__restrict__ info, float *__restrict__ grad_mean,
-                    double *__restrict__ apart, long long B, int T, int P) {
+uniform_main_kernel(TabDev tb, double *ws, const float *__restrict__ smp_traj, const float *__restrict__ mean,
+                    const float *__restrict__ init_pos, const float *__restrict__ init_vel,
+                    const int64_t *__restrict__ pairs, int grad_mode, const float *__restrict__ grad_logp,
+                    const float *__restrict__ logp_old, const float *__restrict__ advantage, double grad_scale,
+                    double *__restrict__ loss_acc, float *__restrict__ logp, int32_t *__restrict__ info,
+                    float *__restrict__ grad_mean, double *apart, const float *__restrict__ L,
+                    const float *__restrict__ upstream, float *__restrict__ grad_L, double *__restrict__ grad_sigma,
+                    long long B, int T, int P) {
   using UL = UniLayout<D, K1>;
   using SM = UniMainSmem<D, K1, UM_EP>;
   constexpr int Dp = D * K1, N = 2 * D, NT = tri(N), AL = SM::AL, MS = SM::MS;
@@ -1277,127 +1436,26 @@
       }
     }
   }
-  if (want_grad && apart) {
-#pragma unroll
-    for (int u = 0; u < MAXACC; ++u) {
-      const int e = threadIdx.x + u * UM_THREADS;
-      if (e < NE) apart[(size_t)blockIdx.x * NE + e] = racc[u];
-    }
-  }
-  if (grad_mode == 2 && loss_acc) {
-    loss_part = warp_sum(loss_part);
-    ratio_part = warp_sum(ratio_part);
-    if (lane == 0) { s_red[2 * warp] = loss_part; s_red[2 * warp + 1] = ratio_part; }
-    __syncthreads();
-    if (threadIdx.x == 0) {
-      double a = 0.0, rr = 0.0;
-      for (int w = 0; w < nwarps; ++w) { a += s_red[2 * w]; rr += s_red[2 * w + 1]; }
-      if (rr != 0.0) { atomicAdd(loss_acc, a); atomicAdd(loss_acc + 1, rr); }
-    }
-  }
-}
-
-template <int D, int K1>
-__global__ void __launch_bounds__(UT)
-uniform_finish_kernel(double *ws, const double *__restrict__ apart, int nparts, const float *__restrict__ L,
-                      const float *__restrict__ upstream, float *__restrict__ grad_L, double *__restrict__ grad_sigma,
-                      int P) {
-  using FL = FusedLayout<D, K1>;
-  using UL = UniLayout<D, K1>;
-  constexpr int Dp = FL::Dp, NT = FL::NT, NB = FL::NB, NR4 = FL::NR4, LD = FL::LD;
-  static_assert(NT + 1 <= 128, "128 entry slots");
-  const UL ul(P);
-  extern __shared__ __align__(16) unsigned char smem_raw[];
-  float *M = reinterpret_cast<float *>(smem_raw);
-  float *Ls = M + NR4 * LD;
-  double *G = reinterpret_cast<double *>(Ls + NR4 * LD + (NR4 * LD & 1));
-  double *hm = G + (size_t)P * NT;
-  __shared__ double s_part[8][129];
-  __shared__ int s_last;
-  const int NE = P * (NT + 1);
-  const int p = blockIdx.x, t = threadIdx.x & 127, sl = threadIdx.x >> 7;
-  unsigned int *ticket = reinterpret_cast<unsigned int *>(ws + ul.flags + 2);
-  float lreg[(NR4 * NR4 + UT - 1) / UT];
-#pragma unroll
-  for (int u = 0; u < (NR4 * NR4 + UT - 1) / UT; ++u) {
-    const int e = threadIdx.x + u * UT, i = e / NR4, c = e - i * NR4;
-    lreg[u] = (L && e < NR4 * NR4 && i < Dp && c <= i) ? L[(size_t)i * Dp + c] : 0.f;
-  }
-  double a[4] = {0.0, 0.0, 0.0, 0.0};
-  if (t <= NT) {
-    const double *src = apart + (size_t)p * (NT + 1) + t;
-    int k = sl;
-    for (; k + 24 < nparts; k += 32) {
-#pragma unroll
-      for (int u = 0; u < 4; ++u) a[u] += src[(size_t)(k + 8 * u) * NE];
-    }
-    for (; k < nparts; k += 8) a[0] += src[(size_t)k * NE];
-  }
-  s_part[sl][t] = (a[0] + a[1]) + (a[2] + a[3]);
-  __syncthreads();
-  if (threadIdx.x <= NT) {
-    double v = 0.0;
-#pragma unroll
-    for (int u = 0; u < 8; ++u) v += s_part[u][threadIdx.x];
-    s_part[0][threadIdx.x] = v;
-  }
-  __syncthreads();
-  if (threadIdx.x < NT)
-    ws[ul.gbuf + (size_t)p * NT + threadIdx.x] =
-        0.5 * (s_part[0][threadIdx.x] - s_part[0][NT] * ws[ul.cinv + (size_t)p * NT + threadIdx.x]);
-  __threadfence();
-  __syncthreads();
-  if (threadIdx.x == 0) s_last = (atomicAdd(ticket, 1u) == gridDim.x - 1);
-  __syncthreads();
-  if (!s_last) return;
-  __threadfence();
-  const int chained = (int)ws[ul.flags], nq = (int)ws[ul.flags + 1];
-  const float up = upstream ? *upstream : 1.0f;
-  for (int e = threadIdx.x; e < P * NT; e += UT) G[e] = __ldcg(ws + ul.gbuf + e);
-  for (int e = threadIdx.x; e < nq * K1; e += UT) hm[e] = ws[ul.hm + e];
-  for (int e = threadIdx.x; e < NR4 * LD; e += UT) M[e] = 0.f;
-#pragma unroll
-  for (int u = 0; u < (NR4 * NR4 + UT - 1) / UT; ++u) {
-    const int e = threadIdx.x + u * UT, i = e / NR4, c = e - i * NR4;
-    if (e < NR4 * NR4) Ls[i * LD + c] = lreg[u];
-  }
-  __syncthreads();
-  for (int task = threadIdx.x; task < NB * K1; task += UT) {
-    const int blk = task / K1, i = task - blk * K1;
-    int d, dd;
-    tri_decode(blk, d, dd);
-    const int r0 = 2 * d, q0 = 2 * dd;
-    const int e00 = tri_idx(r0, q0), e10 = tri_idx(r0 + 1, q0), e11 = tri_idx(r0 + 1, q0 + 1);
-    const int e01 = (d != dd) ? tri_idx(r0, q0 + 1) : e10;
-    double acc[K1];
-#pragma unroll
-    for (int j = 0; j < K1; ++j) acc[j] = 0.0;
-    for (int q = 0; q < nq; ++q) {
-      const Links lk = links(chained, q, P);
-      double w = 0.0;
-      const double hqi = hm[(size_t)q * K1 + i];
-      if (lk.pf >= 0) {
-        const double *Gp = G + (size_t)lk.pf * NT;
-        w += Gp[e00] * hqi + Gp[e10] * hm[(size_t)lk.nxt * K1 + i];
-      }
-      if (lk.ps >= 0) {
-        const double *Gp = G + (size_t)lk.ps * NT;
-        w += Gp[e11] * hqi + Gp[e01] * hm[(size_t)lk.prv * K1 + i];
-      }
-#pragma unroll
-      for (int j = 0; j < K1; ++j) acc[j] = fma(w, hm[(size_t)q * K1 + j], acc[j]);
-    }
-#pragma unroll
-    for (int j = 0; j < K1; ++j) {
-      const float v = up * (float)acc[j];
-      M[(d * K1 + i) * LD + dd * K1 + j] = v;
-      if (d != dd) M[(dd * K1 + j) * LD + d * K1 + i] = v;
-    }
-  }
-  __syncthreads();
-  if (grad_sigma)
-    for (int e = threadIdx.x; e < Dp * Dp; e += UT) grad_sigma[e] = (double)M[(e / Dp) * LD + (e % Dp)];
-  if (grad_L) dl_from_dsigma<D, K1>(M, Ls, grad_L);
+  if (!apart) return;
+  const int NRec = uni_record(P, NT);
+  double *rec = apart + (size_t)blockIdx.x * NRec;
+#pragma unroll
+  for (int u = 0; u < MAXACC; ++u) {
+    const int e = threadIdx.x + u * UM_THREADS;
+    if (e < NE) rec[e] = racc[u];
+  }
+  loss_part = warp_sum(loss_part);
+  ratio_part = warp_sum(ratio_part);
+  if (lane == 0) { s_red[2 * warp] = loss_part; s_red[2 * warp + 1] = ratio_part; }
+  __syncthreads();
+  if (threadIdx.x == 0) {
+    double a = 0.0, rr = 0.0;
+    for (int w = 0; w < nwarps; ++w) { a += s_red[2 * w]; rr += s_red[2 * w + 1]; }
+    rec[NE] = a;
+    rec[NE + 1] = rr;
+    if (NRec > NE + 2) rec[NE + 2] = 0.0;
+  }
+  uniform_tail<D, K1, UM_EP>(apart, ws, L, upstream, grad_L, grad_sigma, grad_mode == 2 ? loss_acc : nullptr, P);
 }
 
 }
@@ -1586,40 +1644,39 @@
 extern "C" int tce_seglik_uniform_parts(const tce_tables_t *t, int64_t B, int64_t P, int32_t *nparts,
                                         int64_t *apart_doubles) {
   if (!t || P < 1 || B < 0) return TCE_ERR_INVALID_ARGUMENT;
-  const int g = uniform_grid(B);
+  const int g = uniform_grid(B), groups = (g + UNI_GROUP - 1) / UNI_GROUP;
   const int64_t N = 2 * (int64_t)t->D, NT = N * (N + 1) / 2;
-  if (P * (NT + 1) > 12 * UM_THREADS) return TCE_ERR_UNSUPPORTED_SHAPE;
+  if (P * (NT + 1) > 12 * UM_THREADS || 1 + groups > UNI_TICKETS) return TCE_ERR_UNSUPPORTED_SHAPE;
   if (nparts) *nparts = g;
-  if (apart_doubles) *apart_doubles = (int64_t)g * P * (NT + 1);
+  if (apart_doubles) *apart_doubles = (int64_t)(g + groups) * uni_record((int)P, (int)NT);
   return TCE_OK;
 }
 
-extern "C" int tce_seglik_uniform_prep(const tce_tables_t *t, const float *L, const double *Sigma0,
-                                       const double *sigma_scale, const float *times, const float *init_time,
-                                       const int64_t *pred_pairs, double *ws, double *diag_max, double reg_rel,
-                                       int what, int64_t P, void *stream) {
-  if (!t || (!L && !Sigma0) || !times || !init_time || !pred_pairs || !ws || !diag_max || P < 1 || !(what & 3))
+extern "C" int tce_seglik_uniform_factor(const tce_tables_t *t, const float *L, const double *Sigma0,
+                                         const double *sigma_scale, const float *times, const float *init_time,
+                                         const int64_t *pred_pairs, double *ws, double *acc, double reg_rel, int what,
+                                         int64_t P, void *stream) {
+  if (!t || (!L && !Sigma0) || !times || !init_time || !pred_pairs || !ws || !acc || P < 1 || what < 1 || what > 3)
     return TCE_ERR_INVALID_ARGUMENT;
   cudaStream_t st = (cudaStream_t)stream;
+  const unsigned grid = what == 1 ? 1u : (unsigned)P;
 #define X(Dv, Kv)                                                                                                   \
   if (t->D == Dv && t->K1 == Kv) {                                                                                  \
     using FL = FusedLayout<Dv, Kv>;                                                                                 \
     const size_t sb = sizeof(double) * FL::NB * Kv * FL::KP, ls = sizeof(float) * FL::NR4 * FL::LD;                 \
-    const size_t smem = (((sb > ls ? sb : ls) + 15) & ~(size_t)15) + sizeof(double) * (FL::IR + 2 * P * Kv) + 16;   \
+    const size_t smem = (((sb > ls ? sb : ls) + 15) & ~(size_t)15) + sizeof(double) * (FL::IR + 2 * P * Kv + 4 * P); \
     if (smem > SMEM_LIMIT) return TCE_ERR_UNSUPPORTED_SHAPE;                                                        \
-    if ((what & 1) && Sigma0) {                                                                                     \
-      auto kern = uniform_prep_kernel<Dv, Kv, true>;                                                                \
-      TCE_CUDA(cudaFuncSetAttribute(kern, cudaFuncAttributeMaxDynamicSharedMemorySize, (int)smem), "uprep smem");   \
-      kern<<<1, UT, smem, st>>>(tab_dev(t), nullptr, Sigma0, sigma_scale, times, init_time, pred_pairs, ws,         \
-                                diag_max, reg_rel, (int)P, what);                                                   \
-    } else if (what & 1) {                                                                                          \
-      auto kern = uniform_prep_kernel<Dv, Kv, false>;                                                               \
-      TCE_CUDA(cudaFuncSetAttribute(kern, cudaFuncAttributeMaxDynamicSharedMemorySize, (int)smem), "uprep smem");   \
-      kern<<<1, UT, smem, st>>>(tab_dev(t), L, nullptr, nullptr, times, init_time, pred_pairs, ws, diag_max,        \
-                                reg_rel, (int)P, what);                                                             \
+    if (Sigma0) {                                                                                                   \
+      auto kern = uniform_factor_kernel<Dv, Kv, true>;                                                              \
+      TCE_CUDA(cudaFuncSetAttribute(kern, cudaFuncAttributeMaxDynamicSharedMemorySize, (int)smem), "ufac smem");    \
+      kern<<<grid, UF, smem, st>>>(tab_dev(t), nullptr, Sigma0, sigma_scale, times, init_time, pred_pairs, ws, acc, \
+                                   reg_rel, (int)P, what);                                                          \
+    } else {                                                                                                        \
+      auto kern = uniform_factor_kernel<Dv, Kv, false>;                                                             \
+      TCE_CUDA(cudaFuncSetAttribute(kern, cudaFuncAttributeMaxDynamicSharedMemorySize, (int)smem), "ufac smem");    \
+      kern<<<grid, UF, smem, st>>>(tab_dev(t), L, nullptr, nullptr, times, init_time, pred_pairs, ws, acc, reg_rel, \
+                                   (int)P, what);                                                                   \
     }                                                                                                               \
-    if (what & 1) TCE_CHECK_LAUNCH("uniform_prep_kernel");                                                          \
-    if (what & 2) uniform_factor_kernel<Dv, Kv><<<(unsigned)P, 32, 0, st>>>(ws, diag_max, reg_rel, (int)P);         \
     TCE_CHECK_LAUNCH("uniform_factor_kernel");                                                                      \
     return TCE_OK;                                                                                                  \
   }
@@ -1628,19 +1685,23 @@
   return TCE_ERR_UNSUPPORTED_SHAPE;
 }
 
-extern "C" int tce_seglik_uniform_main(const tce_tables_t *t, const double *ws, const float *smp_traj,
-                                       const float *mean, const float *init_pos, const float *init_vel,
-                                       const int64_t *pred_pairs, int grad_mode, const float *grad_logp,
-                                       const float *logp_old, const float *advantage, double grad_scale,
-                                       double *loss_acc, float *logp, int32_t *info, float *grad_mean, double *apart,
-                                       int64_t B, int64_t T, int64_t P, void *stream) {
+extern "C" int tce_seglik_uniform_main(const tce_tables_t *t, double *ws, const float *smp_traj, const float *mean,
+                                       const float *init_pos, const float *init_vel, const int64_t *pred_pairs,
+                                       int grad_mode, const float *grad_logp, const float *logp_old,
+                                       const float *advantage, double grad_scale, double *loss_acc, float *logp,
+                                       int32_t *info, float *grad_mean, double *apart, const float *L,
+                                       const float *upstream, float *grad_L, double *grad_sigma, int64_t B, int64_t T,
+                                       int64_t P, void *stream) {
   if (B == 0) return TCE_OK;
   if (!t || !ws || !smp_traj || !mean || !init_pos || !init_vel || !pred_pairs || B < 0 || T < 1 || P < 1 ||
       grad_mode < 0 || grad_mode > 2)
     return TCE_ERR_INVALID_ARGUMENT;
   if (grad_mode == 1 && !grad_logp) return TCE_ERR_INVALID_ARGUMENT;
-  if (grad_mode == 2 && (!logp_old || !advantage)) return TCE_ERR_INVALID_ARGUMENT;
+  if (grad_mode == 2 && (!logp_old || !advantage || (loss_acc && !apart))) return TCE_ERR_INVALID_ARGUMENT;
+  if ((grad_L || grad_sigma) && (!apart || !grad_mode)) return TCE_ERR_INVALID_ARGUMENT;
+  if ((grad_L && !L) || (apart && !grad_mode)) return TCE_ERR_INVALID_ARGUMENT;
   const unsigned grid = (unsigned)uniform_grid(B);
+  if (1 + (grid + UNI_GROUP - 1) / UNI_GROUP > UNI_TICKETS) return TCE_ERR_UNSUPPORTED_SHAPE;
 #define X(Dv, Kv)                                                                                                  \
   if (t->D == Dv && t->K1 == Kv) {                                                                                 \
     constexpr int N = 2 * Dv, NT = N * (N + 1) / 2;                                                                \
@@ -1652,7 +1713,8 @@
       TCE_CUDA(cudaFuncSetAttribute(kern, cudaFuncAttributeMaxDynamicSharedMemorySize, (int)smem), "umain smem");  \
       kern<<<grid, UM_THREADS, smem, (cudaStream_t)stream>>>(                                                      \
           tab_dev(t), ws, smp_traj, mean, init_pos, init_vel, pred_pairs, grad_mode, grad_logp, logp_old,          \
-          advantage, grad_scale, loss_acc, logp, info, grad_mean, apart, (long long)B, (int)T, (int)P);            \
+          advantage, grad_scale, loss_acc, logp, info, grad_mean, apart, L, upstream, grad_L, grad_sigma,          \
+          (long long)B, (int)T, (int)P);                                                                           \
     } else {                                                                                                       \
       const size_t smem = UniMainSmem<Dv, Kv, 32>((int)P).total;                                                   \
       if (smem > SMEM_LIMIT) return TCE_ERR_UNSUPPORTED_SHAPE;                                                     \
@@ -1660,7 +1722,8 @@
       TCE_CUDA(cudaFuncSetAttribute(kern, cudaFuncAttributeMaxDynamicSharedMemorySize, (int)smem), "umain smem");  \
       kern<<<grid, UM_THREADS, smem, (cudaStream_t)stream>>>(                                                      \
           tab_dev(t), ws, smp_traj, mean, init_pos, init_vel, pred_pairs, grad_mode, grad_logp, logp_old,          \
-          advantage, grad_scale, loss_acc, logp, info, grad_mean, apart, (long long)B, (int)T, (int)P);            \
+          advantage, grad_scale, loss_acc, logp, info, grad_mean, apart, L, upstream, grad_L, grad_sigma,          \
+          (long long)B, (int)T, (int)P);                                                                           \
     }                                                                                                              \
     TCE_CHECK_LAUNCH("uniform_main_kernel");                                                                       \
     return TCE_OK;                                                                                                 \
@@ -1669,26 +1732,3 @@
 #undef X
   return TCE_ERR_UNSUPPORTED_SHAPE;
 }
-
-extern "C" int tce_seglik_uniform_finish(const tce_tables_t *t, double *ws, const double *apart, int nparts,
-                                         const float *L, const float *upstream, float *grad_L, double *grad_sigma,
-                                         int64_t P, void *stream) {
-  if (!t || !ws || !apart || nparts < 1 || (!grad_L && !grad_sigma) || (grad_L && !L) || P < 1)
-    return TCE_ERR_INVALID_ARGUMENT;
-#define X(Dv, Kv)                                                                                          \
-  if (t->D == Dv && t->K1 == Kv) {                                                                         \
-    using FL = FusedLayout<Dv, Kv>;                                                                        \
-    const size_t smem = sizeof(float) * (2 * FL::NR4 * FL::LD + 2) +                                       \
-                        sizeof(double) * ((size_t)P * FL::NT + 2 * P * Kv) + 16;                           \
-    if (smem > SMEM_LIMIT) return TCE_ERR_UNSUPPORTED_SHAPE;                                               \
-    auto kern = uniform_finish_kernel<Dv, Kv>;                                                             \
-    TCE_CUDA(cudaFuncSetAttribute(kern, cudaFuncAttributeMaxDynamicSharedMemorySize, (int)smem), "ufin smem"); \
-    kern<<<(unsigned)P, UT, smem, (cudaStream_t)stream>>>(ws, apart, nparts, L, upstream, grad_L, grad_sigma, \
-                                                          (int)P);                                         \
-    TCE_CHECK_LAUNCH("uniform_finish_kernel");                                                             \
-    return TCE_OK;                                                                                         \
-  }
-  TCE_FOR_SHAPES(X)
-#undef X
-  return TCE_ERR_UNSUPPORTED_SHAPE;
-}
diff --git a/tce_rl_b200/ops_seglik.py b/tce_rl_b200/ops_seglik.py
--- a/tce_rl_b200/ops_seglik.py
+++ b/tce_rl_b200/ops_seglik.py
@@ -181,8 +181,6 @@
         raise TceError("the uniform path needs a shared covariance")
     logp = torch.empty(B, P, device=dev, dtype=torch.float32)
     info = torch.empty(B, P, device=dev, dtype=torch.int32)
-    acc = torch.zeros(3, device=dev, dtype=torch.float64)
-    diag_max, stats = acc[:1], acc[1:]
     want = grad_mode != 0
     g_mean = torch.empty(B, Dp, device=dev, dtype=torch.float32) if want else mean.new_empty(0)
     need_L = want and want_grad_L
@@ -196,7 +194,7 @@
             g_L = torch.zeros(1 if shared else 0, Dp, Dp, device=dev, dtype=torch.float32)
         if need_S:
             g_S = torch.zeros(Dp, Dp, device=dev, dtype=torch.float64)
-        return logp, info, acc, g_mean, g_L, g_S
+        return logp, info, torch.zeros(3, device=dev, dtype=torch.float64), g_mean, g_L, g_S
     if need_L and shared and L is None:
         raise TceError("grad_L of a shared covariance needs its factor L")
     st = _stream()
@@ -205,29 +203,30 @@
     if uniform and cfg["uni_parts"] == 0:
         uniform = False
     if uniform:
+        acc = torch.empty(3, device=dev, dtype=torch.float64)
         ws = torch.empty(cfg["ws_doubles"], device=dev, dtype=torch.float64)
         Lp = None if sigma is not None else _p(L)
+        fac = (tables, Lp, _p(sigma), _p(sigma_scale), _p(times), _p(init_time), _p(pairs), _p(ws), _p(acc),
+               float(reg_rel))
         if _REG_GROUP is None or (_GLOBAL_UNIFORM and shared):
-            _lib.call("tce_seglik_uniform_prep", tables, Lp, _p(sigma), _p(sigma_scale), _p(times), _p(init_time),
-                      _p(pairs), _p(ws), _p(diag_max), float(reg_rel), 3, P, st)
+            _lib.call("tce_seglik_uniform_factor", *fac, 3, P, st)
         else:
-            _lib.call("tce_seglik_uniform_prep", tables, Lp, _p(sigma), _p(sigma_scale), _p(times), _p(init_time),
-                      _p(pairs), _p(ws), _p(diag_max), float(reg_rel), 1, P, st)
-            _reduce_diag_max(diag_max)
-            _lib.call("tce_seglik_uniform_prep", tables, Lp, _p(sigma), _p(sigma_scale), _p(times), _p(init_time),
-                      _p(pairs), _p(ws), _p(diag_max), float(reg_rel), 2, P, st)
-        apart = torch.empty(cfg["apart_doubles"], device=dev, dtype=torch.float64) if (need_L or need_S) else None
+            _lib.call("tce_seglik_uniform_factor", *fac, 1, P, st)
+            _reduce_diag_max(acc[:1])
+            _lib.call("tce_seglik_uniform_factor", *fac, 2, P, st)
+        apart = torch.empty(cfg["apart_doubles"], device=dev, dtype=torch.float64) \
+            if (need_L or need_S or grad_mode == 2) else None
+        if need_L:
+            g_L = torch.empty(1, Dp, Dp, device=dev, dtype=torch.float32)
+        if need_S:
+            g_S = torch.empty(Dp, Dp, device=dev, dtype=torch.float64)
         _lib.call("tce_seglik_uniform_main", tables, _p(ws), _p(smp_traj), _p(mean), _p(init_pos), _p(init_vel),
-                  _p(pairs), int(grad_mode), _p(grad_logp), _p(logp_old), _p(advantage), scale, _p(stats), _p(logp),
-                  _p(info), _p(g_mean) if want else None, _p(apart), B, T, P, st)
-        if need_L or need_S:
-            if need_L:
-                g_L = torch.empty(1, Dp, Dp, device=dev, dtype=torch.float32)
-            if need_S:
-                g_S = torch.empty(Dp, Dp, device=dev, dtype=torch.float64)
-            _lib.call("tce_seglik_uniform_finish", tables, _p(ws), _p(apart), cfg["uni_parts"],
-                      _p(L) if need_L else None, None, _p(g_L) if need_L else None, _p(g_S) if need_S else None, P, st)
+                  _p(pairs), int(grad_mode), _p(grad_logp), _p(logp_old), _p(advantage), scale, _p(acc[1:]), _p(logp),
+                  _p(info), _p(g_mean) if want else None, _p(apart), _p(L) if need_L else None, None,
+                  _p(g_L) if need_L else None, _p(g_S) if need_S else None, B, T, P, st)
         return logp, info, acc, g_mean, g_L, g_S
+    acc = torch.zeros(3, device=dev, dtype=torch.float64)
+    diag_max, stats = acc[:1], acc[1:]
     pre = torch.empty(B * cfg["pre_doubles"], device=dev, dtype=torch.float64)
     _lib.call("tce_seglik_prepass", tables, _p(smp_traj), _p(mean), None if sigma is not None else _p(L), ldb,
               _p(sigma), _p(sigma_scale), _p(times), _p(init_time), _p(init_pos), _p(init_vel), _p(pairs), _p(pre),
```

Measured after the change: 4.748 million (median of 6 runs). -6.1%, worse.
